# kvarq/kvarq

Measured on AMD Instinct MI355X. Metric: fastq_reads_per_sec_scanned, higher is better.
Workload: dtype u8

## Files before the change

include/kvarq_hip.h:

```cpp
#ifndef KVARQ_HIP_H
#define KVARQ_HIP_H

#include <stddef.h>
#include <stdint.h>

#ifdef __cplusplus
extern "C" {
#endif

#define KVQ_MAX_READLENGTH 1024
#define KVQ_SCANBUFSIZE    (1024*1024)
#define KVQ_MUT_CLASSES    6

enum {
    KVQ_OK          = 0,
    KVQ_ERR_FORMAT  = 1,
    KVQ_ERR_IO      = 2,
    KVQ_ERR_MEMORY  = 3,
    KVQ_ERR_RUNTIME = 4,
    KVQ_ERR_TYPE    = 5,
    KVQ_ERR_DEVICE  = 6,
    KVQ_ERR_RESCAN  = 7
};

typedef struct kvq_config {
    int32_t maxerrors;
    int32_t minoverlap;
    int32_t minreadlength;
    int32_t nthreads;
    int8_t  Amin;
    int8_t  Azero;
} kvq_config;

void kvq_config_set(const kvq_config *cfg);
void kvq_config_get(kvq_config *cfg);

int32_t kvq_last_error(char *msg, size_t cap);

typedef struct kvq_table kvq_table;

kvq_table *kvq_table_create(const uint8_t *const *seqs, const int32_t *seqlens, int32_t nseq,
                            const kvq_config *cfg);
void    kvq_table_destroy(kvq_table *t);
int32_t kvq_table_nseq(const kvq_table *t);
int64_t kvq_table_bases(const kvq_table *t);
int32_t kvq_table_seq_is_seeded(const kvq_table *t, int32_t s);
int32_t kvq_table_seed_k(const kvq_table *t);

enum { KVQ_CTR_RECORDS = 0, KVQ_CTR_LONGEST = 1, KVQ_CTR_HITS = 2, KVQ_CTR_READLENGTHS = 4 };
int64_t kvq_counters_len(const kvq_table *t);
int64_t kvq_counters_off_nseqhits(const kvq_table *t);
int64_t kvq_counters_off_nseqbasehits(const kvq_table *t);
int64_t kvq_counters_off_coverage(const kvq_table *t);
int64_t kvq_counters_off_mutations(const kvq_table *t);
int64_t kvq_table_seq_offset(const kvq_table *t, int32_t s);

typedef struct kvq_scan kvq_scan;

kvq_scan *kvq_scan_create(const kvq_table *t, void *d_counters);
void      kvq_scan_destroy(kvq_scan *s);

int64_t kvq_chunk_offsets(const uint8_t *data, int64_t nbytes, int64_t *offsets, int64_t cap);

int32_t kvq_scan_device(kvq_scan *s, const void *d_data, int64_t nbytes,
                        const int64_t *chunk_off, int64_t nchunks, int64_t fpos_base);

int32_t kvq_scan_host(kvq_scan *s, const void *h_data, int64_t nbytes,
                      const int64_t *chunk_off, int64_t nchunks, int64_t fpos_base);

int32_t kvq_scan_host_async(kvq_scan *s, const void *h_data, int64_t nbytes,
                            const int64_t *chunk_off, int64_t nchunks, int64_t fpos_base);
int32_t kvq_scan_host_copied(kvq_scan *s);
int32_t kvq_scan_host_drain(kvq_scan *s);

int32_t kvq_scan_finish(kvq_scan *s);
int32_t kvq_scan_finish_begin(kvq_scan *s);

int64_t        kvq_scan_n_hits(const kvq_scan *s);
const int32_t *kvq_scan_hit_seq_nr(const kvq_scan *s);
const int64_t *kvq_scan_hit_file_pos(const kvq_scan *s);
const int32_t *kvq_scan_hit_seq_pos(const kvq_scan *s);
const int32_t *kvq_scan_hit_length(const kvq_scan *s);
const int32_t *kvq_scan_hit_readlength(const kvq_scan *s);
const uint8_t *kvq_scan_hitseq_blob(const kvq_scan *s);
const int64_t *kvq_scan_hitseq_offsets(const kvq_scan *s);
const int64_t *kvq_scan_counters(const kvq_scan *s);
void          *kvq_scan_device_counters(const kvq_scan *s);
void          *kvq_scan_device_counters_own(const kvq_scan *s);
int64_t        kvq_scan_parsed(const kvq_scan *s);
int64_t        kvq_scan_total(const kvq_scan *s);

int32_t        kvq_scan_set_records(kvq_scan *s, int32_t on);
const uint8_t *kvq_scan_record_blob(const kvq_scan *s);
const int64_t *kvq_scan_hit_record_off(const kvq_scan *s);
const int32_t *kvq_scan_hit_record_len(const kvq_scan *s);
int64_t        kvq_scan_record_bytes(const kvq_scan *s);

double  kvq_scan_kernel_ms(const kvq_scan *s);
double  kvq_scan_main_kernel_ms(const kvq_scan *s);
double  kvq_scan_gap_ms(const kvq_scan *a, const kvq_scan *b);
int64_t kvq_scan_main_kernel_launches(const kvq_scan *s);
int32_t kvq_scan_reset(kvq_scan *s);
int32_t kvq_scan_path(const kvq_scan *s);
void    kvq_scan_force_exhaustive(kvq_scan *s, int32_t on);

#define KVQ_CELL_DENSE  0x1000
#define KVQ_CELL_DIAG   0x2000
#define KVQ_CELL_STAMPS 0x4000
int32_t kvq_scan_kernel_pick(int32_t k, int32_t stride, int32_t dense, uint32_t rec_bytes, uint32_t tile_bytes, uint32_t dbg);
int32_t kvq_scan_kernel(const kvq_scan *s);
uint32_t kvq_tile_for_text(const uint8_t *text, size_t n, uint32_t *rec_bytes_out);

typedef struct kvq_comm kvq_comm;
int32_t   kvq_comm_unique_id(void *id128);
kvq_comm *kvq_comm_create(int32_t nranks, int32_t rank, const void *id128);
void      kvq_comm_destroy(kvq_comm *c);
int32_t   kvq_comm_nranks(const kvq_comm *c);
int32_t   kvq_comm_rank(const kvq_comm *c);
int32_t   kvq_scan_set_comm(kvq_scan *s, kvq_comm *c);
int32_t   kvq_scan_gather_hits(kvq_scan *s, kvq_comm *c);
int32_t   kvq_comm_allreduce_counters(kvq_comm *c, void *d_counters, int64_t ctr_len, void *d_scratch16);
kvq_comm *kvq_comm_create_local(int32_t nranks, int32_t rank, uint64_t world_key);
int32_t   kvq_gather_plan(int32_t nranks, const uint64_t *counts, uint64_t *parts, uint64_t *blob_base, uint64_t *totals);
int32_t   kvq_gather_host(int32_t nranks, const uint64_t *counts, const uint8_t *const *rank_bufs, uint8_t *out);
void      kvq_result_layout_words(uint64_t n, uint64_t blob_bytes, uint64_t *out8);

kvq_scan *kvq_findseqs(const char *const *files, int32_t nfiles,
                       const uint8_t *const *seqs, const int32_t *seqlens, int32_t nseq);

#define KVQ_FIND_DEVICE_INFLATE 1u
#define KVQ_FIND_DEVICE_GZIP 2u
#define KVQ_FIND_RECORDS 4u
kvq_scan *kvq_findseqs_ex(const char *const *files, int32_t nfiles,
                          const uint8_t *const *seqs, const int32_t *seqlens, int32_t nseq, uint32_t flags);

void kvq_findseqs_free(kvq_scan *s);

int64_t kvq_host_chunk_plan(const char *const *files, int32_t nfiles, int64_t *chunk_fpos, int64_t *chunk_len,
                            int64_t cap, int64_t *parsed, int64_t *total, int64_t batch_bytes);

typedef struct kvq_live_stats {
    int64_t records_parsed;
    int64_t parsed;
    int64_t total;
    int64_t rls_longest;
    int32_t nseq;
    int32_t running;
    int32_t sigints;
    int32_t stop_requested;
} kvq_live_stats;

void kvq_poll_stats(kvq_live_stats *out, int64_t *readlengths ,
                    int64_t *nseqhits, int64_t *nseqbasehits, int32_t nseq_cap);
void kvq_request_stop(void);
void kvq_count_sigint(void);
int  kvq_sigint_counter_install(void);
void kvq_sigint_counter_remove(void);

int32_t kvq_device_count(void);
int32_t kvq_set_device(int32_t ordinal);
void   *kvq_device_alloc(int64_t nbytes);
void    kvq_device_free(void *p);
int32_t kvq_memcpy_h2d(void *d, const void *h, int64_t nbytes);
int32_t kvq_memcpy_d2h(void *h, const void *d, int64_t nbytes);
int32_t kvq_memset_d(void *d, int32_t value, int64_t nbytes);
int32_t kvq_device_synchronize(void);
void    kvq_release_cached(void);

int32_t kvq_synth_reads_device(void *d_out, int64_t first, int64_t n, int32_t L,
                               uint64_t seed, const void *d_genome, int64_t genome_size);
void    kvq_synth_reads_host(uint8_t *out, int64_t first, int64_t n, int32_t L,
                             uint64_t seed, const uint8_t *genome, int64_t genome_size);
void    kvq_synth_genome_host(uint8_t *out, int64_t size, uint64_t seed);

int32_t kvq_inflate_raw_host(const uint8_t *in, int64_t n, uint8_t *out, int64_t isize);

int64_t kvq_bgzf_index(const uint8_t *file_bytes, int64_t n, int64_t *block_off, uint32_t *csize, uint32_t *isize, int64_t cap);

typedef struct kvq_bgzf_block {
    int64_t  in_off;
    int64_t  out_off;
    uint32_t in_len;
    uint32_t isize;
} kvq_bgzf_block;

int32_t kvq_inflate_bgzf_device(const void *d_in, int64_t in_bytes, const kvq_bgzf_block *d_blocks, int64_t nblocks,
                                void *d_out, int64_t out_bytes, int32_t *d_status);

int64_t kvq_chunk_offsets_device(const void *d_data, int64_t nbytes, int64_t *offsets, int64_t cap);

typedef struct kvq_gzip_report {
    int64_t runs;
    int64_t chunks;
    int64_t candidates_tested;
    int64_t refuted;
    int64_t redecodes;
    int64_t slot_overflows;
    int64_t marker_symbols;
    int64_t input_retries;
    double  ms_find, ms_decode, ms_resolve, ms_replace;
} kvq_gzip_report;

int64_t kvq_inflate_gzip_host(const uint8_t *file, int64_t n, int64_t chunk_bytes, uint8_t *out, int64_t out_cap,
                              int32_t *status, int64_t *err_fpos, kvq_gzip_report *rep);
int64_t kvq_inflate_gzip_device(const void *d_file, int64_t n, int64_t chunk_bytes, void *d_out, int64_t out_cap,
                                int32_t *status, int64_t *err_fpos, kvq_gzip_report *rep);
void    kvq_gzip_last_report(kvq_gzip_report *rep);
int64_t kvq_gzip_slot_canaries(int32_t pad_symbols);
int64_t kvq_gzip_last_chunks(int64_t *cand, int64_t ncand_cap, int64_t *start_bit, int64_t *end_bit, int64_t *nsym, int64_t cap,
                             int64_t *ncand);

typedef struct kvq_bam_report {
    int64_t runs;
    int64_t segments;
    int64_t refuted;
    int64_t check_passes;
    int64_t records_seen;
    int64_t records_written;
    int64_t records_skipped;
    int64_t records_noqual;
    int64_t bam_bytes;
    int64_t text_bytes;
    double  ms_inflate, ms_find, ms_emit;
} kvq_bam_report;
void    kvq_bam_last_report(kvq_bam_report *rep);
int64_t kvq_bam_header_host(const uint8_t *inflated, int64_t n, int32_t *n_ref);
int64_t kvq_bam_to_fastq_host(const uint8_t *inflated, int64_t n, int32_t n_ref, int64_t first_record, uint8_t *out, int64_t cap,
                              int64_t *consumed);
int64_t kvq_bam_to_fastq_device(const void *d_in, int64_t n, int32_t n_ref, int64_t first_record, void *d_out, int64_t cap,
                                int64_t segment_bytes, kvq_bam_report *report);

const char *kvq_version(void);

#ifdef __cplusplus
}
#endif
#endif
```

kvarq_amd/_lib.py:

```python
import ctypes as C
import os

HERE = os.path.dirname(os.path.abspath(__file__))
PATH = os.path.join(HERE, 'libkvarq_hip.so')

MAX_READLENGTH = 1024
OK, ERR_FORMAT, ERR_IO, ERR_MEMORY, ERR_RUNTIME, ERR_TYPE, ERR_DEVICE, ERR_RESCAN = range(8)
CTR_RECORDS, CTR_LONGEST, CTR_HITS, CTR_READLENGTHS = 0, 1, 2, 4
CELL_DENSE, CELL_DIAG, CELL_STAMPS = 0x1000, 0x2000, 0x4000
FIND_RECORDS = 4


class Config(C.Structure):
    _fields_ = [('maxerrors', C.c_int32), ('minoverlap', C.c_int32), ('minreadlength', C.c_int32),
                ('nthreads', C.c_int32), ('Amin', C.c_int8), ('Azero', C.c_int8)]


class LiveStats(C.Structure):
    _fields_ = [('records_parsed', C.c_int64), ('parsed', C.c_int64), ('total', C.c_int64),
                ('rls_longest', C.c_int64), ('nseq', C.c_int32), ('running', C.c_int32),
                ('sigints', C.c_int32), ('stop_requested', C.c_int32)]


class GzipReport(C.Structure):
    _fields_ = [(n, C.c_int64) for n in ('runs', 'chunks', 'candidates_tested', 'refuted', 'redecodes',
                                         'slot_overflows', 'marker_symbols', 'input_retries')] + \
        [(n, C.c_double) for n in ('ms_find', 'ms_decode', 'ms_resolve', 'ms_replace')]

    def as_dict(self):
        return {n: getattr(self, n) for n, _ in self._fields_}


class BamReport(C.Structure):
    _fields_ = [(n, C.c_int64) for n in ('runs', 'segments', 'refuted', 'check_passes', 'records_seen', 'records_written',
                                         'records_skipped', 'records_noqual', 'bam_bytes', 'text_bytes')] + \
        [(n, C.c_double) for n in ('ms_inflate', 'ms_find', 'ms_emit')]

    def as_dict(self):
        return {n: getattr(self, n) for n, _ in self._fields_}


i32, i64, u64, vp, cp = C.c_int32, C.c_int64, C.c_uint64, C.c_void_p, C.c_char_p
P = C.POINTER

PROTOTYPES = {
    'kvq_config_set': (None, [P(Config)]),
    'kvq_config_get': (None, [P(Config)]),
    'kvq_last_error': (i32, [C.c_char_p, C.c_size_t]),
    'kvq_table_create': (vp, [P(cp), P(i32), i32, P(Config)]),
    'kvq_table_destroy': (None, [vp]),
    'kvq_table_nseq': (i32, [vp]),
    'kvq_table_bases': (i64, [vp]),
    'kvq_table_seq_is_seeded': (i32, [vp, i32]),
    'kvq_table_seed_k': (i32, [vp]),
    'kvq_counters_len': (i64, [vp]),
    'kvq_counters_off_nseqhits': (i64, [vp]),
    'kvq_counters_off_nseqbasehits': (i64, [vp]),
    'kvq_counters_off_coverage': (i64, [vp]),
    'kvq_counters_off_mutations': (i64, [vp]),
    'kvq_table_seq_offset': (i64, [vp, i32]),
    'kvq_scan_create': (vp, [vp, vp]),
    'kvq_scan_destroy': (None, [vp]),
    'kvq_chunk_offsets': (i64, [vp, i64, P(i64), i64]),
    'kvq_scan_device': (i32, [vp, vp, i64, P(i64), i64, i64]),
    'kvq_scan_host': (i32, [vp, vp, i64, P(i64), i64, i64]),
    'kvq_scan_host_async': (i32, [vp, vp, i64, P(i64), i64, i64]),
    'kvq_scan_host_copied': (i32, [vp]),
    'kvq_scan_host_drain': (i32, [vp]),
    'kvq_scan_finish': (i32, [vp]),
    'kvq_scan_finish_begin': (i32, [vp]),
    'kvq_scan_n_hits': (i64, [vp]),
    'kvq_scan_hit_seq_nr': (P(i32), [vp]),
    'kvq_scan_hit_file_pos': (P(i64), [vp]),
    'kvq_scan_hit_seq_pos': (P(i32), [vp]),
    'kvq_scan_hit_length': (P(i32), [vp]),
    'kvq_scan_hit_readlength': (P(i32), [vp]),
    'kvq_scan_hitseq_blob': (vp, [vp]),
    'kvq_scan_hitseq_offsets': (P(i64), [vp]),
    'kvq_scan_counters': (P(i64), [vp]),
    'kvq_scan_device_counters': (vp, [vp]),
    'kvq_scan_device_counters_own': (vp, [vp]),
    'kvq_scan_parsed': (i64, [vp]),
    'kvq_scan_total': (i64, [vp]),
    'kvq_scan_set_records': (i32, [vp, i32]),
    'kvq_scan_record_blob': (vp, [vp]),
    'kvq_scan_hit_record_off': (P(i64), [vp]),
    'kvq_scan_hit_record_len': (P(i32), [vp]),
    'kvq_scan_record_bytes': (i64, [vp]),
    'kvq_scan_kernel_ms': (C.c_double, [vp]),
    'kvq_scan_main_kernel_ms': (C.c_double, [vp]),
    'kvq_scan_gap_ms': (C.c_double, [vp, vp]),
    'kvq_scan_main_kernel_launches': (i64, [vp]),
    'kvq_scan_reset': (i32, [vp]),
    'kvq_scan_path': (i32, [vp]),
    'kvq_scan_force_exhaustive': (None, [vp, i32]),
    'kvq_scan_kernel_pick': (i32, [i32, i32, i32, C.c_uint32, C.c_uint32, C.c_uint32]),
    'kvq_scan_kernel': (i32, [vp]),
    'kvq_tile_for_text': (C.c_uint32, [vp, C.c_size_t, P(C.c_uint32)]),
    'kvq_comm_unique_id': (i32, [vp]),
    'kvq_comm_create': (vp, [i32, i32, vp]),
    'kvq_comm_destroy': (None, [vp]),
    'kvq_comm_nranks': (i32, [vp]),
    'kvq_comm_rank': (i32, [vp]),
    'kvq_scan_set_comm': (i32, [vp, vp]),
    'kvq_scan_gather_hits': (i32, [vp, vp]),
    'kvq_comm_allreduce_counters': (i32, [vp, vp, i64, vp]),
    'kvq_comm_create_local': (vp, [i32, i32, C.c_uint64]),
    'kvq_gather_plan': (i32, [i32, vp, vp, vp, vp]),
    'kvq_gather_host': (i32, [i32, vp, vp, vp]),
    'kvq_result_layout_words': (None, [C.c_uint64, C.c_uint64, vp]),
    'kvq_findseqs': (vp, [P(cp), i32, P(cp), P(i32), i32]),
    'kvq_findseqs_ex': (vp, [P(cp), i32, P(cp), P(i32), i32, C.c_uint32]),
    'kvq_findseqs_free': (None, [vp]),
    'kvq_host_chunk_plan': (i64, [P(cp), i32, P(i64), P(i64), i64, P(i64), P(i64), i64]),
    'kvq_poll_stats': (None, [P(LiveStats), P(i64), P(i64), P(i64), i32]),
    'kvq_request_stop': (None, []),
    'kvq_count_sigint': (None, []),
    'kvq_sigint_counter_install': (C.c_int, []),
    'kvq_sigint_counter_remove': (None, []),
    'kvq_device_count': (i32, []),
    'kvq_set_device': (i32, [i32]),
    'kvq_device_alloc': (vp, [i64]),
    'kvq_device_free': (None, [vp]),
    'kvq_memcpy_h2d': (i32, [vp, vp, i64]),
    'kvq_memcpy_d2h': (i32, [vp, vp, i64]),
    'kvq_memset_d': (i32, [vp, i32, i64]),
    'kvq_device_synchronize': (i32, []),
    'kvq_release_cached': (None, []),
    'kvq_synth_reads_device': (i32, [vp, i64, i64, i32, u64, vp, i64]),
    'kvq_synth_reads_host': (None, [vp, i64, i64, i32, u64, vp, i64]),
    'kvq_synth_genome_host': (None, [vp, i64, u64]),
    'kvq_inflate_raw_host': (i32, [vp, i64, vp, i64]),
    'kvq_bgzf_index': (i64, [vp, i64, P(i64), P(C.c_uint32), P(C.c_uint32), i64]),
    'kvq_chunk_offsets_device': (i64, [vp, i64, P(i64), i64]),
    'kvq_inflate_bgzf_device': (i32, [vp, i64, vp, i64, vp, i64, vp]),
    'kvq_inflate_gzip_host': (i64, [vp, i64, i64, vp, i64, P(i32), P(i64), P(GzipReport)]),
    'kvq_inflate_gzip_device': (i64, [vp, i64, i64, vp, i64, P(i32), P(i64), P(GzipReport)]),
    'kvq_gzip_last_report': (None, [P(GzipReport)]),
    'kvq_gzip_slot_canaries': (i64, [i32]),
    'kvq_gzip_last_chunks': (i64, [P(i64), i64, P(i64), P(i64), P(i64), i64, P(i64)]),
    'kvq_bam_last_report': (None, [P(BamReport)]),
    'kvq_bam_header_host': (i64, [vp, i64, P(i32)]),
    'kvq_bam_to_fastq_host': (i64, [vp, i64, i32, i64, vp, i64, P(i64)]),
    'kvq_bam_to_fastq_device': (i64, [vp, i64, i32, i64, vp, i64, i64, P(BamReport)]),
    'kvq_version': (cp, []),
}

_lib = None


def build():
    import subprocess
    subprocess.check_call(['make', '-s', '-C', os.path.join(HERE, 'csrc')])


def lib():
    global _lib
    if _lib is None:
        if not os.path.exists(PATH):
            raise ImportError('%s is missing: build it with `make -C kvarq_amd/csrc` '
                              '(there is no CPU fallback for the scan)' % PATH)
        L = C.CDLL(PATH)
        for name, (res, args) in PROTOTYPES.items():
            f = getattr(L, name)
            f.restype, f.argtypes = res, args
        _lib = L
    return _lib


def kernel_cell(cell):
    if cell <= 0:
        return None
    return {'k': cell & 15, 'stride': (cell >> 4) & 15, 'lg': ((cell >> 8) & 15) - 1, 'dense': bool(cell & CELL_DENSE)}


def last_error():
    buf = C.create_string_buffer(1024)
    code = lib().kvq_last_error(buf, 1024)
    return code, buf.value.decode('latin-1')
```

kvarq_amd/csrc/kernels_bp.hip:

```cpp
#include "kvq_host.h"

#ifndef KVQ_TEXT_AUX
#define KVQ_TEXT_AUX 0
#endif
#define KVQ_MARK(name) asm volatile("; KVQMARK " name)
#define BP_WIN (ST_BUF + ST_BLK)
#define BP_Q1_KIND 25
#define BP_QW 96
#define BP_Q2W 96
#define BP_NLCAP 1920
#define BP_P2_LATE 0xFFFEu
#define BP_HEAD 2048u
#define BP_QCAP (BP_QW * ST_WAVES)
#define BP_Q2CAP (BP_Q2W * ST_WAVES)

typedef unsigned int u32x4_t __attribute__((ext_vector_type(4)));

struct BpLds {
    uint32_t cdp[BP_WIN / 16 + 8];
    uint32_t gdp[BP_WIN / 32 + 8];
    uint16_t nl[BP_NLCAP];
    uint8_t  bmA[8192];
    uint32_t hist[KVQ_RL_BINS / 2];
    union {
        struct {
            uint32_t q1[BP_QCAP];
            uint32_t q2[BP_Q2CAP];
        };
        uint32_t nlp[BP_WIN / 32 + 8];
    };
    uint32_t rinfo[ST_RCAP];
    __attribute__((aligned(16))) uint8_t head[BP_HEAD];
    __attribute__((aligned(16))) uint32_t wtot[ST_WAVES];
    uint32_t longest_p1, records, fallback, n_owned, next_tile, first_tile, p2_jn;
    uint32_t sv_at[ST_WAVES], sv_end[ST_WAVES];
};
static_assert(sizeof(BpLds) <= 40 * 1024, "four workgroups per CU: at most 40 KB of LDS each");
static_assert(offsetof(BpLds, cdp) == 0, "cdp[] first");
#define BP_LDS_GDP ((uint32_t)offsetof(BpLds, gdp))
#define BP_LDS_BMA ((uint32_t)offsetof(BpLds, bmA))
#define BP_LDS_NLP ((uint32_t)offsetof(BpLds, nlp))
#define BP_LDS_HEAD ((uint32_t)offsetof(BpLds, head))
static_assert(sizeof(uint32_t) * (BP_QCAP + BP_Q2CAP) >= sizeof(uint32_t) * (BP_WIN / 32 + 8), "the newline plane fits the queues it shares LDS with");

__device__ __forceinline__ uint32_t lds_u32_at(uint32_t addr)
{
    return *reinterpret_cast<const __attribute__((address_space(3))) uint32_t *>((uintptr_t)addr);
}
__device__ __forceinline__ uint32_t cdp32(uint32_t pos)
{
    const uint32_t a = (pos >> 2) & ~3u, sh = (pos & 15u) * 2u;
    return __builtin_amdgcn_alignbit(lds_u32_at(a + 4u), lds_u32_at(a), sh);
}
template <int KK> __device__ __forceinline__ uint32_t cdp_code(uint32_t pos) { return cdp32(pos) & ((1u << (2 * KK)) - 1u); }

typedef const __attribute__((address_space(1))) uint32_t *GlbWords;
__device__ __forceinline__ uint32_t tab2_32(GlbWords tab2, uint32_t tpos)
{
    const uint32_t w = tpos >> 4, sh = (tpos & 15u) * 2u;
    return __builtin_amdgcn_alignbit(tab2[w + 1u], tab2[w], sh);
}

__device__ __forceinline__ int diff_codes(uint32_t x, uint32_t y)
{
    const uint32_t v = x ^ y;
    return __popc((v | (v >> 1)) & 0x55555555u);
}

template <int KK>
__device__ __forceinline__ bool seed_live_bp(GlbWords tab2, uint32_t roff, int rl, int rp, uint32_t toff, int seql, int sq)
{
    if (rp < 0 || rp + KK > rl || sq < 0 || sq + KK > seql) return false;
    return cdp_code<KK>(roff + (uint32_t)rp) == (tab2_32(tab2, toff + (uint32_t)sq) & ((1u << (2 * KK)) - 1u));
}

struct BpHot {
    const KvqParams *cold; GlbBytes tab; GlbWords tab2;
    int maxerrors, minoverlap, pitch;
};
template <int KK>
__device__ __forceinline__ void bp_verify_rest(const BpHot &P, GlbBytes text, bool alive, uint32_t roff, int rl, int p, uint32_t kind,
                                               uint32_t en_lo, uint32_t en_hi, int64_t tile_fpos, int stride)
{
    bool hitAB = false, hitC = false;
    int s = 0, lenAB = 0, lenC = 0, sposAB = 0, sposC = 0; uint32_t keyAB = 0, keyC = 0;
    const int64_t fpos = tile_fpos + (int64_t)roff - (int64_t)ST_PRE;
    if (alive) {
        const int q = (int)(en_lo & 4095u);
        s = (int)(en_lo >> 12);
        const uint32_t toff = en_hi & 0xFFFFFu;
        const int seql = (int)(en_hi >> 20);
        const int mo = P.minoverlap, me = P.maxerrors;
        const int d = q - p;
        const int a = d < 0 ? -d : 0;
        const int L = (rl < seql - d ? rl : seql - d) - a;
        bool canAB = false, canC = false;
        const bool guard = rl > mo && seql > mo;
        if (d < 0) {
            const int i = -d;
            if (i <= rl - seql) { canC = true; lenC = seql; sposC = -i; keyC = (2u << 30) | (uint32_t)i; }
            else if (guard && i <= rl - mo) { canAB = true; lenAB = rl - i; sposAB = -i; keyAB = (0u << 30) | (uint32_t)(rl - mo - i); }
        } else if (d == 0) {
            canC = true; lenC = rl > seql ? seql : rl; sposC = 0; keyC = 2u << 30;
        } else {
            const int i = d;
            if (guard && i <= seql - mo && i >= seql - rl) { canAB = true; lenAB = seql - i; sposAB = i; keyAB = (1u << 30) | (uint32_t)(seql - mo - i); }
            if (rl <= seql && i <= seql - rl) { canC = true; lenC = rl; sposC = i; keyC = (2u << 30) | (uint32_t)i; }
        }
        if (canAB || canC) {
            int mism = 0, j = 0;
            const GlbBytes x = text + roff + (uint32_t)a, y = P.tab + toff + (uint32_t)(a + d);
            for (; j + 8 <= L && mism <= me; j += 8) {
                typedef unsigned int u32x2_t __attribute__((ext_vector_type(2)));
                typedef u32x2_t __attribute__((aligned(1))) u32x2_any;
                const u32x2_t xv = *reinterpret_cast<const __attribute__((address_space(1))) u32x2_any *>(x + j);
                const u32x2_t yv = *reinterpret_cast<const __attribute__((address_space(1))) u32x2_any *>(y + j);
                mism += diff_bytes(xv.x, yv.x) + diff_bytes(xv.y, yv.y);
            }
            for (; j + 4 <= L && mism <= me; j += 4) mism += diff_bytes(glb_u32(x + j), glb_u32(y + j));
            for (; j < L && mism <= me; j++) mism += (x[j] != y[j]);
            if (mism <= me) {
                bool earlier = false;
                for (int jj = 0; jj <= me && !earlier; jj++) {
                    const int ph = jj * KK, pt = rl - (jj + 1) * KK;
                    if (ph + KK <= rl && (kind == 0u || ph < p)) earlier = seed_live_bp<KK>(P.tab2, roff, rl, ph, toff, seql, ph + d);
                    if (!earlier && pt >= 0 && (kind == 0u || pt < p)) earlier = seed_live_bp<KK>(P.tab2, roff, rl, pt, toff, seql, pt + d);
                }
                if (kind == 0u) {
                    for (int jj = 0; jj <= me && !earlier; jj++)
                        for (int sft = 0; sft < stride && !earlier; sft++) {
                            const int o = jj * P.pitch + sft;
                            if (o < q && ((o - d) & (stride - 1)) == 0) earlier = seed_live_bp<KK>(P.tab2, roff, rl, o - d, toff, seql, o);
                        }
                }
                if (!earlier) { hitAB = canAB; hitC = canC; }
            }
        }
    }
    emit_cold(P.cold, hitAB, fpos, s, sposAB, lenAB, rl, keyAB);
    emit_cold(P.cold, hitC, fpos, s, sposC, lenC, rl, keyC);
}

__device__ __forceinline__ void bp_vector(const uint4 v, uint32_t addk, uint32_t &nl16, uint32_t &g16, uint32_t &c32)
{
    const uint32_t x[4] = { v.x, v.y, v.z, v.w };
    uint32_t nf[4], gf[4], cc[4];
#pragma unroll
    for (int d = 0; d < 4; d++) {
        nf[d] = kvq_nl_flags(x[d]);
        gf[d] = good_flags(x[d], addk);
        cc[d] = __builtin_amdgcn_udot4(x[d] & 0x06060606u, 0x40100401u, 0u, false);
    }
#ifdef KVQ_ABL_JUNK
    {
        uint32_t junk = x[0];
#pragma unroll
        for (int i = 0; i < KVQ_ABL_JUNK; i++) {
#if KVQ_ABL_SLOW == 2
            { uint32_t sj = 0; asm volatile("s_add_u32 %0, %0, 1" : "+s"(sj)); asm volatile("" :: "s"(sj)); }
#elif KVQ_ABL_SLOW == 3
            { uint32_t lj; asm volatile("ds_read_b32 %0, %1" : "=v"(lj) : "v"(junk & 0x3FCu)); asm volatile("s_waitcnt lgkmcnt(0)" ::: "memory"); asm volatile("" :: "v"(lj)); }
#elif KVQ_ABL_SLOW
            asm volatile("v_lshl_or_b32 %0, %0, 1, %1" : "+v"(junk) : "v"(x[1]));
#else
            asm volatile("v_add_u32 %0, %0, %1" : "+v"(junk) : "v"(x[1]));
#endif
        }
        asm volatile("" :: "v"(junk));
    }
#endif
    nl16 = kvq_flags16(nf[0], nf[1], nf[2], nf[3]);
    g16 = kvq_flags16(gf[0], gf[1], gf[2], gf[3]);
    c32 = ((cc[0] | (cc[1] << 8)) >> 1) | ((cc[2] | (cc[3] << 8)) << 15);
}

struct BpArgs {
    KvqParams P;
    SeedTables X;
    const uint8_t *data; int64_t fpos_base;
    const uint4 *tiles; uint32_t *tile_report; unsigned int *tile_ctr;
    void *redo;
    unsigned int *fail;
    void *surv;
    uint32_t ntiles, tile_bytes, dbg, pad_, redo_cap;
    uint32_t surv_cap;
};
#define BP_SHARDS 64u
#define BP_SHARD_STRIDE 32u
__host__ __device__ static inline uint32_t bp_shard_begin(uint32_t sh, uint32_t ntiles) { return (uint32_t)(((uint64_t)sh * ntiles) / BP_SHARDS); }
__device__ __forceinline__ uint32_t bp_draw(unsigned int *ctr, uint32_t ntiles, uint32_t &sh, uint32_t &left)
{
    while (left) {
        const uint32_t t = atomicAdd(&ctr[sh * BP_SHARD_STRIDE], 1u);
        if (t < bp_shard_begin(sh + 1u, ntiles)) return t;
        sh = sh + 1u == BP_SHARDS ? 0u : sh + 1u; left--;
    }
    return ntiles;
}
static_assert(BP_SHARDS == 64u, "one counter per lane of the drawing wave");
__device__ __forceinline__ uint32_t bp_draw_wave(unsigned int *ctr, uint32_t ntiles, uint32_t &sh, uint32_t lane)
{
    const uint32_t m = (((uint32_t)blockIdx.x >> 6) * 2u + 37u) | 1u;
    for (;;) {
        const uint32_t mine = (sh + m * lane) & (BP_SHARDS - 1u);
        const uint32_t seen = __hip_atomic_load(&ctr[mine * BP_SHARD_STRIDE], __ATOMIC_RELAXED, __HIP_MEMORY_SCOPE_AGENT);
        const uint64_t open = __ballot(seen < bp_shard_begin(mine + 1u, ntiles));
        if (open == 0) return ntiles;
        const uint32_t pick = (sh + m * (uint32_t)(__ffsll((long long)open) - 1)) & (BP_SHARDS - 1u);
        uint32_t t = 0;
        if (lane == 0) t = atomicAdd(&ctr[pick * BP_SHARD_STRIDE], 1u);
        t = (uint32_t)__builtin_amdgcn_readfirstlane((int)t);
        sh = pick;
        if (t < bp_shard_begin(pick + 1u, ntiles)) return t;
    }
}
typedef const __attribute__((address_space(4))) BpArgs *BpArgsPtr;
__device__ __forceinline__ BpArgsPtr bp_args(const BpArgs *A)
{
    BpArgsPtr p = (BpArgsPtr)A;
    asm volatile("" : "+s"(p));
    return p;
}

#ifndef BP_OCC
#define BP_OCC 8
#endif

__device__ __forceinline__ void bp_runs64(uint64_t m, int n, uint32_t dbg, int &pre, int &suf, int &best, int &bstart)
{
    const uint64_t nmask = n < 64 ? (1ull << n) - 1ull : ~0ull;
    uint64_t zz = ~m & nmask;
    const int c = __popc((uint32_t)zz) + __popc((uint32_t)(zz >> 32));
    if (!__any(c > 3) && !(dbg & 4u)) {
        const uint32_t lo = (uint32_t)zz, hi = (uint32_t)(zz >> 32);
        auto ffbl = [](uint32_t x) -> uint32_t { uint32_t r; asm("v_ffbl_b32 %0, %1" : "=v"(r) : "v"(x)); return r; };
        auto ffbh = [](uint32_t x) -> uint32_t { uint32_t r; asm("v_ffbh_u32 %0, %1" : "=v"(r) : "v"(x)); return r; };
        auto ctz64 = [&](uint32_t l, uint32_t h) -> uint32_t {
            const uint32_t pl = ffbl(l), ph = ffbl(h) | 32u;
            const uint32_t r = pl < ph ? pl : ph; return r < (uint32_t)n ? r : (uint32_t)n;
        };
        const uint32_t p1 = ctz64(lo, hi);
        const uint64_t z2 = zz & (zz - 1ull);
        const uint32_t p2 = ctz64((uint32_t)z2, (uint32_t)(z2 >> 32));
        const uint32_t ch = ffbh(hi), cl = ffbh(lo) | 32u;
        uint32_t lz = ch < cl ? ch : cl; lz = lz < 64u ? lz : 64u;
        const uint32_t e = 64u - lz;
        const int g0 = (int)p1, g1 = (int)p2 - (int)p1 - 1, g2 = (int)e - (int)p2 - 2, g3 = n - (int)e;
        int bl = g0, bs = 0;
        if (g1 > bl) { bl = g1; bs = (int)p1 + 1; }
        if (g2 > bl) { bl = g2; bs = (int)p2 + 1; }
        if (g3 > bl) { bl = g3; bs = (int)e; }
        pre = g0; suf = g3; best = bl; bstart = bs;
    } else if (!__any(c > 8) && !(dbg & 4u)) {
        int prev = 0, first = n, p, bl = 0, bs = 0;
        do {
            const uint32_t plo = (uint32_t)(__ffs((int)(uint32_t)zz) - 1), ph = (uint32_t)(__ffs((int)(uint32_t)(zz >> 32)) - 1);
            const uint32_t phi = ph > 0xFFFFFFDFu ? 0xFFFFFFFFu : ph + 32u;
            uint32_t pm = plo < phi ? plo : phi; if (pm > (uint32_t)n) pm = (uint32_t)n;
            p = (int)pm;
            zz &= zz - 1ull;
            first = first < p ? first : p;
            const int gap = p - prev;
            if (gap > bl) { bl = gap; bs = prev; }
            prev = p < n ? p + 1 : prev;
        } while (__any(p < n));
        pre = first; suf = n - prev; best = bl; bstart = bs;
    } else {
        const uint64_t inv = ~m;
        pre = inv ? __ffsll((long long)inv) - 1 : 64; if (pre > n) pre = n;
        const uint64_t top = ~(m << (64 - n));
        suf = top ? __clzll((long long)top) : 64; if (suf > n) suf = n;
        longest_run64(m, n, best, bstart);
    }
}

template <int SS, int LG, bool STAMPS, bool DIAG = STAMPS, int KK = 8, bool DENSE = (KK < 8)>
__global__ void __launch_bounds__(ST_THREADS, DENSE ? 8 : BP_OCC)
kvq_scan_bp(const BpArgs *__restrict__ A_)
{
    __shared__ __align__(16) BpLds S;
    uint8_t *const lds_raw = reinterpret_cast<uint8_t *>(&S);
    int tid = threadIdx.x, lane = tid & 63;
    const uint32_t wave = rfl((uint32_t)tid >> 6);
    if ((uint32_t)(uintptr_t)((__attribute__((address_space(3))) uint8_t *)lds_raw) != 0u) __builtin_trap();
    unsigned long long stamp_acc[8] = { 0, 0, 0, 0, 0, 0, 0, 0 }, stamp_t = 0, wave_p34 = 0;
    unsigned long long rt_in = 0, rt_pro = 0, rt_first = 0;
    uint32_t tally[8] = { 0, 0, 0, 0, 0, 0, 0, 0 };
#ifdef KVQ_TALLY
#define BTALLY(i, cond) do { if constexpr (STAMPS) { if (cond) tally[i]++; } } while (0)
#else
#define BTALLY(i, cond) ((void)0)
#endif
    if constexpr (STAMPS) rt_in = __builtin_amdgcn_s_memrealtime();
#define BSTAMP(i) do { if constexpr (STAMPS) { const unsigned long long now_ = __builtin_amdgcn_s_memtime(); stamp_acc[i] += now_ - stamp_t; stamp_t = now_; } } while (0)

    uint32_t ntiles, tile_bytes, dbg, amin;
    {
        const BpArgsPtr A = bp_args(A_);
        ntiles = A->ntiles; tile_bytes = A->tile_bytes; dbg = DIAG ? A->dbg : 0u; amin = (uint32_t)A->P.amin;
        const GlbWords bm1 = (GlbWords)A->X.bm1;
        for (int i = tid; i < (1 << (2 * KK)) / 32; i += ST_THREADS) reinterpret_cast<uint32_t *>(S.bmA)[i] = bm1[i];
    }
    uint32_t my_shard = blockIdx.x % BP_SHARDS; bool no_more = false;
    if (wave == ST_WAVES - 1u) {
        unsigned int *const ctr = bp_args(A_)->tile_ctr;
        const uint32_t t0 = bp_draw_wave(ctr, ntiles, my_shard, (uint32_t)lane);
        const uint32_t t1 = t0 < ntiles ? bp_draw_wave(ctr, ntiles, my_shard, (uint32_t)lane) : ntiles;
        no_more = t1 >= ntiles;
        if (lane == 0) { S.first_tile = t0; S.next_tile = t1; }
    }
    for (int i = tid; i < KVQ_RL_BINS / 2; i += ST_THREADS) S.hist[i] = 0;
    if (tid == 0) { S.longest_p1 = 0; S.records = 0; S.fallback = 0; }
    if (tid < (int)ST_WAVES) { S.sv_at[tid] = 0; S.sv_end[tid] = 0; }
    if (tid < 8) { S.cdp[BP_WIN / 16 + tid] = 0; S.gdp[BP_WIN / 32 + tid] = 0; }

    static_assert(ST_ROUNDS * 16u == ST_BLK, "one scan block per thread");
    static_assert(ST_WAVES == 8, "eight wave totals");
    __syncthreads();

    if (const uint32_t stg = bp_args(A_)->pad_) { for (uint32_t i = 0; i < (blockIdx.x >> 8) * stg; i++) __builtin_amdgcn_s_sleep(127); }
    if constexpr (STAMPS) rt_pro = __builtin_amdgcn_s_memrealtime();
    unsigned long long *const ctr_stamps = bp_args(A_)->P.ctr + KVQ_CTR_RL_ + 924;
    const uint32_t addk = (0x80u - amin) * 0x01010101u;
    uint32_t tiles_done = 0;
    uint32_t g_done = 0xFFFFFFFFu;
    uint32_t my_longest = 0;
    for (uint32_t g = rfl(S.first_tile); ; ) {
        asm volatile("" : "+v"(tid));
        lane = tid & 63;
        const uint32_t blk = (uint32_t)tid * ST_BLK;
        const uint32_t wv = wave * (ST_BLK * 64u / 16u) + (uint32_t)lane;
        if constexpr (STAMPS) stamp_t = __builtin_amdgcn_s_memtime();
        uint32_t Ja = 0, Jb = 0, Jt = 0, g0 = 0; GlbBytes text = nullptr;
        uint4 pre[ST_ROUNDS];
#pragma unroll
        for (int r = 0; r < (int)ST_ROUNDS; r++) pre[r] = make_uint4(0, 0, 0, 0);
        if (g < ntiles) {
            const BpArgsPtr A = bp_args(A_);
            const u32x4_t q = ((const __attribute__((address_space(4))) u32x4_t *)A->tiles)[(dbg & 64u) ? (g & 63u) : g];
            Ja = q.x; Jb = q.y; Jt = q.z;
            g0 = (Ja & ~15u) + Jt * tile_bytes;
            const uint8_t *const data = A->data;
            text = (GlbBytes)data + g0 - ST_PRE;
            const uint32_t load_hi = g0 + ST_TILE + ST_OV < Jb ? g0 + ST_TILE + ST_OV : Jb;
            const uint32_t vo = 16u * wv - ST_PRE, vo0 = wv >= ST_PRE / 16u ? vo : ST_NO_BLOCK;
            const __amdgpu_buffer_rsrc_t rs = __builtin_amdgcn_make_buffer_rsrc((void *)(data + g0), 0, (int)(((load_hi + 15u) & ~15u) - g0), 0x00020000);
#pragma unroll
            for (int r = 0; r < (int)ST_ROUNDS; r++) {
                const u32x4_t v = __builtin_amdgcn_raw_buffer_load_b128(rs, (int)(r ? vo + 1024u * r : vo0), 0, KVQ_TEXT_AUX);
                pre[r] = make_uint4(v.x, v.y, v.z, v.w);
            }
        }
        __syncthreads();
        unsigned long long sub_t0 = 0, sub_t1 = 0;
        if constexpr (STAMPS) sub_t0 = __builtin_amdgcn_s_memtime();
        if (g_done != 0xFFFFFFFFu) {
            if (tid == 0 && S.fallback) { atomicOr(&bp_args(A_)->tile_report[g_done], TR_FLAG_FALLBACK); S.fallback = 0; }
        }
        if (g >= ntiles) break;
        const uint32_t gn = rfl(S.next_tile);
        const uint32_t own_end = g0 + tile_bytes < Jb ? g0 + tile_bytes : Jb;
        const uint32_t load_hi = g0 + ST_TILE + ST_OV < Jb ? g0 + ST_TILE + ST_OV : Jb;
        const uint32_t own_begin_l = (Jt == 0 ? Ja : g0) - g0 + ST_PRE;
        const uint32_t own_end_l = own_end - g0 + ST_PRE;
        const uint32_t end_l = load_hi - g0 + ST_PRE;

        {
            const uint32_t w_lo = wave * (ST_BLK * 64u), w_hi = w_lo + ST_BLK * 64u;
            const bool cut = ((own_begin_l & 15u) && own_begin_l > w_lo && own_begin_l < w_hi) || ((end_l & 15u) && end_l > w_lo && end_l < w_hi);
            if (cut) {
                uint32_t wv_ = wv;
                asm volatile("" : "+v"(wv_));
#pragma unroll
                for (int r = 0; r < (int)ST_ROUNDS; r++) {
                    const uint32_t o = 16u * (wv_ + 64u * r);
                    uint32_t x[4] = { pre[r].x, pre[r].y, pre[r].z, pre[r].w };
#pragma unroll
                    for (int d = 0; d < 4; d++) x[d] &= (kvq_range_flags(o + 4u * d, own_begin_l, end_l) >> 7) * 0xFFu;
                    pre[r] = make_uint4(x[0], x[1], x[2], x[3]);
                }
            }
        }
        if constexpr (STAMPS) { asm volatile("s_waitcnt vmcnt(0)" ::: "memory"); sub_t1 = __builtin_amdgcn_s_memtime(); }
        KVQ_MARK("P0 vectors");
        {
            const uint32_t pa = 2u * wv, ca = 4u * wv;
#pragma unroll
            for (int r = 0; r < (int)ST_ROUNDS; r++) {
                uint32_t n16, g16, c32;
                bp_vector(pre[r], addk, n16, g16, c32);
                *reinterpret_cast<__attribute__((address_space(3))) uint16_t *>((uintptr_t)(BP_LDS_NLP + pa + 128u * r)) = (uint16_t)n16;
                *reinterpret_cast<__attribute__((address_space(3))) uint16_t *>((uintptr_t)(BP_LDS_GDP + pa + 128u * r)) = (uint16_t)g16;
                *reinterpret_cast<__attribute__((address_space(3))) uint32_t *>((uintptr_t)(ca + 256u * r)) = c32;
            }
            if (wave == 0u) {
#pragma unroll
                for (int r = 0; r < (int)(BP_HEAD / 1024u); r++)
                    *reinterpret_cast<__attribute__((address_space(3))) u32x4_t *>((uintptr_t)(BP_LDS_HEAD + 16u * (uint32_t)lane + 1024u * r)) = u32x4_t{ pre[r].x, pre[r].y, pre[r].z, pre[r].w };
            }
        }
        KVQ_MARK("P0 vectors end");
        uint32_t m0, m1, m2;
        {
            const uint32_t a = BP_LDS_NLP + ((10u * (uint32_t)tid) & ~3u), sh = ((uint32_t)tid & 1u) * 16u;
            const uint32_t d0 = lds_u32_at(a), d1 = lds_u32_at(a + 4u), d2 = lds_u32_at(a + 8u);
            m0 = __builtin_amdgcn_alignbit(d1, d0, sh); m1 = __builtin_amdgcn_alignbit(d2, d1, sh); m2 = (d2 >> sh) & 0xFFFFu;
        }
        static_assert(ST_BLK == 80u, "five vectors per block");
        const uint32_t cnt = (uint32_t)(__popc(m0) + __popc(m1) + __popc(m2));
        const uint32_t incl = kvq_wave_incl_scan(cnt);
        if (lane == 63) S.wtot[wave] = incl;
        KVQ_MARK("P0 scan end");
        if constexpr (STAMPS) { if (tid == 0) { atomicAdd(&ctr_stamps[0], sub_t0 - stamp_t); atomicAdd(&ctr_stamps[1], sub_t1 - sub_t0); } }
        BSTAMP(0);
        __syncthreads();
        KVQ_MARK("P1b");
        BSTAMP(1);
        uint32_t n_all = 0;
        {
            uint32_t run = S.wtot[lane & 7];
            run += (uint32_t)__builtin_amdgcn_update_dpp(0, (int)run, 0x111, 0xf, 0xf, false);
            run += (uint32_t)__builtin_amdgcn_update_dpp(0, (int)run, 0x112, 0xf, 0xf, false);
            run += (uint32_t)__builtin_amdgcn_update_dpp(0, (int)run, 0x114, 0xf, 0xf, false);
            n_all = (uint32_t)__builtin_amdgcn_readlane((int)run, 7);
            const uint32_t upto = (uint32_t)__builtin_amdgcn_readlane((int)run, (int)wave);
            uint32_t n = upto - (uint32_t)__builtin_amdgcn_readlane((int)incl, 63) + incl - cnt;
            if (blk < own_end_l && blk + ST_BLK >= own_end_l) S.n_owned = n + cnt;
            if (__any(cnt != 0u)) {
                if (n_all <= BP_NLCAP && !__any(cnt > 2u)) {
                    auto low80 = [](uint32_t w0, uint32_t w1, uint32_t w2) -> uint32_t {
                        auto ffbl = [](uint32_t x) -> uint32_t { uint32_t r; asm("v_ffbl_b32 %0, %1" : "=v"(r) : "v"(x)); return r; };
                        const uint32_t f0 = ffbl(w0), f1 = ffbl(w1) | 32u, f2 = ffbl(w2) | 64u;
                        const uint32_t f01 = f0 < f1 ? f0 : f1;
                        return f01 < f2 ? f01 : f2;
                    };
                    const uint32_t p1 = low80(m0, m1, m2);
                    const uint32_t k0 = m0 & (m0 - 1u), k1 = m0 ? m1 : m1 & (m1 - 1u), k2 = (m0 | m1) ? m2 : m2 & (m2 - 1u);
                    const uint32_t p2 = low80(k0, k1, k2);
                    if (cnt) {
                        S.nl[n] = (uint16_t)(blk + p1);
                        if (cnt > 1u) S.nl[n + 1u] = (uint16_t)(blk + p2);
                    }
                    m0 = m1 = m2 = 0u;
                }
                while (__any((m0 | m1 | m2) != 0u)) {
                    const bool in0 = m0 != 0u, in1 = m1 != 0u;
                    const uint32_t w = in0 ? m0 : in1 ? m1 : m2;
                    if (w) {
                        const uint32_t pos = blk + (in0 ? 0u : in1 ? 32u : 64u) + (uint32_t)(__ffs((int)w) - 1);
                        if (n < BP_NLCAP) S.nl[n] = (uint16_t)pos;
                        n++;
                        const uint32_t w1 = w & (w - 1u);
                        if (in0) m0 = w1; else if (in1) m1 = w1; else m2 = w1;
                    }
                }
            }
        }
        if (wave == 0u) {
            const uint32_t cnt0 = (uint32_t)__builtin_amdgcn_readlane((int)incl, 63);
            uint32_t early = BP_P2_LATE;
            if (Jt != 0 && cnt0 >= 10u) {
                const uint32_t m = (uint32_t)lane;
                bool ok = false;
                if (m >= 1 && m <= 8) {
                    const uint32_t e0 = S.nl[m - 1], e2 = S.nl[m + 1];
                    const uint32_t ls0 = e0 + 1u, ls2 = e2 + 1u;
                    if (e0 < own_end_l && ls0 < end_l && ls2 < end_l) {
                        const uint32_t c0 = ls0 < BP_HEAD ? lds_byte_at(BP_LDS_HEAD + ls0) : (uint32_t)text[ls0];
                        const uint32_t c2 = ls2 < BP_HEAD ? lds_byte_at(BP_LDS_HEAD + ls2) : (uint32_t)text[ls2];
                        ok = c0 == '@' && c2 == '+';
                    }
                }
                const uint64_t mk = __ballot(ok);
                early = mk ? (uint32_t)(__ffsll((long long)mk) - 1) : TR_NONE;
            }
            if (lane == 0) S.p2_jn = early;
        }
        __syncthreads();
        KVQ_MARK("P1b end / P2");
        BSTAMP(2);

        uint32_t nrec = 0, jn = TR_NONE, drawn;
        {
            const uint32_t n_nl = n_all < BP_NLCAP ? n_all : BP_NLCAP;
            const uint32_t n_owned = rfl(S.n_owned);
            uint32_t fallback = n_all > BP_NLCAP ? 1u : 0u;
            if (Jt == 0) jn = 0;
            else if (const uint32_t early = rfl(S.p2_jn); early != BP_P2_LATE) jn = early;
            else {
                const uint32_t m = (uint32_t)lane;
                bool ok = false;
                if (m >= 1 && m <= 8 && m <= n_owned && m + 2 <= n_nl) {
                    const uint32_t ls0 = (uint32_t)S.nl[m - 1] + 1u;
                    const uint32_t ls2 = (uint32_t)S.nl[m + 1] + 1u;
                    if (ls0 < end_l && ls2 < end_l) {
                        const uint32_t c0 = ls0 < BP_HEAD ? lds_byte_at(BP_LDS_HEAD + ls0) : (uint32_t)text[ls0];
                        const uint32_t c2 = ls2 < BP_HEAD ? lds_byte_at(BP_LDS_HEAD + ls2) : (uint32_t)text[ls2];
                        ok = c0 == '@' && c2 == '+';
                    }
                }
                const uint64_t mk = __ballot(ok);
                if (mk) jn = (uint32_t)(__ffsll((long long)mk) - 1);
            }
            uint32_t left = 0u;
            if (jn != TR_NONE) {
                if (jn <= n_owned) nrec = (n_owned - jn) / 4u + 1u;
                if (nrec > 0 && jn + 4u * nrec > n_nl) {
                    const uint32_t fit = n_nl >= jn ? (n_nl - jn) / 4u : 0u;
                    if (load_hi < Jb) left = 1u;
                    if (n_all > BP_NLCAP) fallback = 1u;
                    nrec = fit;
                }
                if (nrec > ST_RCAP) { nrec = ST_RCAP; fallback = 1u; }
            }
            if (fallback) { nrec = 0; left = 1u; }
            if (tid == 0 || tid == ST_THREADS - 64) {
                const BpArgsPtr A = bp_args(A_);
                if (tid == 0) {
                    A->tile_report[g] = (n_owned & 0xFFFFu) | ((jn & 0xFFu) << 16) | (left ? TR_FLAG_SKIPPED : 0u) | (left && nrec ? TR_FLAG_PARTIAL : 0u);
                    if (left) A->tile_report[ntiles + g] = nrec ? g0 - ST_PRE + (uint32_t)S.nl[jn + 4u * nrec - 1u] + 2u : 0u;
                    S.records += nrec;
                } else if (!no_more) drawn = atomicAdd(&A->tile_ctr[my_shard * BP_SHARD_STRIDE], 1u);
            }
        }

        if (++tiles_done == ST_HIST_TILES) {
            unsigned long long *const ctr = (bp_args(A_)->P.ctr + (size_t)(blockIdx.x % KVQ_STAGE_COPIES) * KVQ_STAGE_SLOTS);
            for (int i = tid; i < KVQ_RL_BINS / 2; i += ST_THREADS) {
                const uint32_t w = atomicExch(&S.hist[i], 0u);
                if (w & 0xFFFFu) atomicAdd(&ctr[KVQ_CTR_RL_ + 2 * i], (unsigned long long)(w & 0xFFFFu));
                if (w >> 16) atomicAdd(&ctr[KVQ_CTR_RL_ + 2 * i + 1], (unsigned long long)(w >> 16));
            }
            tiles_done = 0;
        }
        if (dbg & 32u) nrec = 0;
        KVQ_MARK("P2 end / P3 setup");
        BSTAMP(3);
        if (wave >= 4u) KVQ_SETPRIO(2); else KVQ_SETPRIO(1);
        unsigned long long wave_t3 = 0;
        if constexpr (STAMPS) wave_t3 = __builtin_amdgcn_s_memtime();
        static_assert(ST_THREADS == 512, "lg = 9 - ceil(log2(nrec))");
        uint32_t lg;
        if constexpr (LG >= 0) lg = (uint32_t)LG;
        else {
            const int lg_ = 9 - (nrec > 1u ? 32 - __builtin_clz(nrec - 1u) : 0);
            lg = lg_ < 0 ? 0u : lg_ > 6 ? 6u : (uint32_t)lg_;
        }
        const uint32_t G = 1u << lg, RP = ST_THREADS >> lg;
        const uint32_t gl = (uint32_t)tid & (G - 1u), gr = (uint32_t)tid >> lg;
        for (uint32_t pass0 = 0; pass0 < nrec; pass0 += RP) {
            const uint32_t k = pass0 + gr;
            const bool have = k < nrec;
            uint32_t roff = 0; int rl = 0;
            uint32_t c0, cp;
            if (have) {
                const uint32_t m = jn + 4u * k;
                const uint32_t rstart = m == 0 ? ST_PRE + (Ja & 15u) : (uint32_t)S.nl[m - 1] + 1u;
                const uint32_t n0 = S.nl[m], n1 = S.nl[m + 1], n2 = S.nl[m + 2], n3 = S.nl[m + 3];
                const uint32_t sread = n0 + 1u, plus = n1 + 1u, sscore = n2 + 1u;
        KVQ_MARK("trim");
                if (gl == 0) { if (dbg & 8u) { c0 = '@'; cp = '+'; } else { c0 = text[rstart]; cp = text[plus]; } }
                const int Q = (int)(n3 - sscore);
                const int per = (Q + (int)G - 1) >> lg;
                Seg sg; sg.beg = (int)mul_u24(gl, (uint32_t)per); if (sg.beg > Q) sg.beg = Q;
                int s1 = sg.beg + per; if (s1 > Q) s1 = Q;
                sg.len = 0; sg.pre = 0; sg.suf = 0; sg.best = 0; sg.bstart = sg.beg;
                {
                    auto round = [&](int c0_) -> Seg {
                        const int n = s1 - c0_ < 64 ? s1 - c0_ : 64;
                        const uint32_t bit = sscore + (uint32_t)c0_;
                        const uint32_t a = BP_LDS_GDP + ((bit >> 5) << 2), sh = bit & 31u;
                        const uint32_t d0 = lds_u32_at(a), d1 = lds_u32_at(a + 4u), d2 = lds_u32_at(a + 8u);
                        const uint64_t nmask = n < 64 ? (1ull << n) - 1ull : ~0ull;
                        const uint64_t mm = (((uint64_t)__builtin_amdgcn_alignbit(d2, d1, sh) << 32) | (uint64_t)__builtin_amdgcn_alignbit(d1, d0, sh)) & nmask;
                        Seg sub; sub.beg = c0_; sub.len = n;
                        int bs;
                        bp_runs64(mm, n, dbg, sub.pre, sub.suf, sub.best, bs);
                        sub.bstart = c0_ + bs;
                        return sub;
                    };
                    if (!__any(per > 64)) sg = round(sg.beg);
                    else {
                        for (int cc = sg.beg; cc < s1; cc += 64) {
                            const Seg sub = round(cc);
                            sg = (cc == sg.beg) ? sub : seg_merge(sg, sub);
                        }
                    }
                }
                if (G == 4u) {
#define KVQ_QUAD(v, ctl) __builtin_amdgcn_update_dpp(0, (v), (ctl), 0xf, 0xf, true)
                    {
                        Seg B;
                        B.len = KVQ_QUAD(sg.len, 0xB1); B.pre = KVQ_QUAD(sg.pre, 0xB1); B.suf = KVQ_QUAD(sg.suf, 0xB1);
                        B.best = KVQ_QUAD(sg.best, 0xB1); B.bstart = KVQ_QUAD(sg.bstart, 0xB1); B.beg = 0;
                        sg = seg_merge(sg, B);
                    }
                    {
                        Seg B;
                        B.len = KVQ_QUAD(sg.len, 0x4E); B.pre = KVQ_QUAD(sg.pre, 0x4E); B.suf = KVQ_QUAD(sg.suf, 0x4E);
                        B.best = KVQ_QUAD(sg.best, 0x4E); B.bstart = KVQ_QUAD(sg.bstart, 0x4E); B.beg = 0;
                        sg = seg_merge(sg, B);
                    }
                    rl = KVQ_QUAD(sg.best, 0x00);
                    roff = sread + (uint32_t)KVQ_QUAD(sg.bstart, 0x00);
#undef KVQ_QUAD
                } else {
                    for (uint32_t d = 1; d < G; d <<= 1) {
                        Seg B;
                        B.len = __shfl_xor(sg.len, (int)d, 64); B.pre = __shfl_xor(sg.pre, (int)d, 64); B.suf = __shfl_xor(sg.suf, (int)d, 64);
                        B.best = __shfl_xor(sg.best, (int)d, 64); B.bstart = __shfl_xor(sg.bstart, (int)d, 64); B.beg = 0;
                        if ((gl & d) == 0) sg = seg_merge(sg, B);
                    }
                    rl = __shfl(sg.best, lane & ~(int)(G - 1u), 64);
                    roff = sread + (uint32_t)__shfl(sg.bstart, lane & ~(int)(G - 1u), 64);
                }
                my_longest = my_longest > (uint32_t)(rl + 1) ? my_longest : (uint32_t)(rl + 1);
                if (gl == 0) {
                    if (rl < KVQ_RL_BINS) atomicAdd(&S.hist[rl >> 1], 1u << (16 * (rl & 1)));
                    S.rinfo[k] = roff | ((uint32_t)rl << 16);
                }
            }
        KVQ_MARK("trim end / filter");
            BSTAMP(4);
            KVQ_SETPRIO(2);
            const uint32_t rpw = 64u >> lg, grw = (uint32_t)lane >> lg;
            const uint32_t wfirst = pass0 + wave * rpw;
            const uint32_t npass = wfirst < nrec ? (nrec - wfirst < rpw ? nrec - wfirst : rpw) : 0u;
            uint32_t *const q1 = S.q1 + wave * BP_QW; uint32_t *const q2 = S.q2 + wave * BP_Q2W;
            uint32_t sub = (dbg & 128u) ? npass : 0u, step = rpw;
            while (sub < npass) {
                BTALLY(6, lane == 0);
                asm volatile("" : "+v"(rl), "+v"(roff));
                int minrl, me_; const __attribute__((address_space(1))) uint8_t *bmL;
                {
                    const BpArgsPtr A = bp_args(A_);
                    minrl = A->P.minreadlength; me_ = A->P.maxerrors;
                    bmL = (const __attribute__((address_space(1))) uint8_t *)A->X.bm1 + (1 << (2 * KK)) / 8;
                }
                const bool mine = have && rl >= minrl && !(dbg & 2u) && grw >= sub && grw - sub < step;
                uint32_t qn = 0;
                int e0 = 0, e1 = 0;
                if (mine) {
                    const int NPe = (rl - KK) / SS + 1;
                    const int per = (NPe + (int)G - 1) >> lg;
                    e0 = (int)mul_u24(gl, (uint32_t)per); if (e0 > NPe) e0 = NPe;
                    e1 = e0 + per; if (e1 > NPe) e1 = NPe;
                }
                auto fixed_block = [&](int pp, bool ok) -> bool {
                    const uint32_t code = cdp_code<KK>(roff + (uint32_t)(ok ? pp : 0));
                    const uint32_t bits = bmL[code >> 3];
                    return ok & (bool)((bits >> (code & 7u)) & 1u);
                };
                auto head_ok = [&](int jj) { return mine && jj <= me_ && (jj + 1) * KK <= rl; };
                auto tail_ok = [&](int jj) { const int pp = rl - (jj + 1) * KK; return mine && jj <= me_ && pp >= 0 && !((pp % KK) == 0 && pp <= me_ * KK); };
                const bool hhit = fixed_block((int)gl * KK, head_ok((int)gl));
                const bool thit = fixed_block(rl - ((int)gl + 1) * KK, tail_ok((int)gl));
                constexpr int NR = SS == 8 ? 6 : SS == 4 ? 12 : (LG == 3 || LG == 1) ? 24 : 18;
                bool first = true;
                if constexpr (!DENSE) {
                for (int ee = e0; __any(ee < e1); ee += NR, first = false) {
                    const bool act = ee < e1;
#include "kernels_bp_lookup.inc"
                    const int nv = act ? (e1 - ee < NR ? e1 - ee : NR) : 0;
                    hA &= (1u << nv) - 1u;
                    const bool hh = first && hhit, th = first && thit;
                    const uint32_t c = (uint32_t)__popc(hA) + (hh ? 1u : 0u) + (th ? 1u : 0u);
                    const uint32_t inc = kvq_wave_incl_scan(c);
                    const uint32_t tot = (uint32_t)__builtin_amdgcn_readlane((int)inc, 63);
                    if (tot) {
                        uint32_t idx = qn + inc - c;
                        while (hA) {
                            const int j = __ffs((int)hA) - 1; hA &= hA - 1u;
                            if (idx < BP_QW) q1[idx] = k | ((uint32_t)(SS * (ee + j)) << 9);
                            idx++;
                        }
                        if (hh) { if (idx < BP_QW) q1[idx] = k | ((gl * KK) << 9) | (1u << BP_Q1_KIND); idx++; }
                        if (th && idx < BP_QW) { const uint32_t pt = (uint32_t)(rl - ((int)gl + 1) * KK); q1[idx] = k | (pt << 9) | (1u << BP_Q1_KIND); }
                        qn += tot;
                    }
                }
                for (int t = (int)G; t <= me_; t += (int)G) {
                    const int jj = t + (int)gl;
#pragma unroll
                    for (int side = 0; side < 2; side++) {
                        const int pp = side ? rl - (jj + 1) * KK : jj * KK;
                        const bool hit = fixed_block(pp, side ? tail_ok(jj) : head_ok(jj));
                        const uint64_t mm = __ballot(hit);
                        if (mm) {
                            const uint32_t idx = qn + (uint32_t)__popcll(mm & kvq_lanemask_lt());
                            if (hit && idx < BP_QW) q1[idx] = k | ((uint32_t)pp << 9) | (1u << BP_Q1_KIND);
                            qn += (uint32_t)__popcll(mm);
                        }
                    }
                }
                }
        KVQ_MARK("filter end / P4a");
                BSTAMP(5);
                KVQ_SETPRIO(3);

                if constexpr (!DENSE) {
                const bool over = qn > BP_QW;
                const uint32_t qn_ok = (over || (dbg & 1u)) ? 0u : qn;
                if (over && step > 1u) { step >>= 1; continue; }
                if (over) {
                    if (mine && gl == 0) {
                        const BpArgsPtr A = bp_args(A_);
                        const KvqRedo Rd(A->redo);
                        const uint32_t boff = g0 - ST_PRE + roff;
                        bool put = false;
                        if (A->redo) {
                            if (rl >= KVQ_LONG_READ) {
                                const unsigned int i = atomicAdd(Rd.count + 1, 1u);
                                if (i < KVQ_LONG_CAP) { Rd.read_off[KVQ_REDO_CAP - 1u - i] = boff; Rd.read_len[KVQ_REDO_CAP - 1u - i] = rl; put = true; }
                            }
                            if (!put) {
                                const unsigned int i = atomicAdd(Rd.count, 1u);
                                if (i < A->redo_cap) { Rd.rec_start[i] = KVQ_REDO_TRIMMED; Rd.read_off[i] = boff; Rd.read_len[i] = rl; }
                                put = true;
                            }
                        }
                        if (!put) S.fallback = 1u;
                        else atomicOr(A->fail, 2u);
                    }
                }
#include "kernels_bp_p4.inc"
                } else {
                    uint32_t hA = 0, hpos = 0, tpos = 0; bool hh = false, th = false;
                    int ee = e0, xt = (int)G;
                    int ee_of_hA = e0;
                    bool done = false;
                    while (!done) {
                        bool full = false;
                        while (!full) {
                            if (!__any(hA != 0u || hh || th)) {
                                ee_of_hA = ee;
                                if (__any(ee < e1)) {
                                    const bool act = ee < e1;
                                    uint32_t hA_;
                                    {
#include "kernels_bp_lookup.inc"
                                        hA_ = hA;
                                    }
                                    const int nv = act ? (e1 - ee < NR ? e1 - ee : NR) : 0;
                                    hA = hA_ & ((1u << nv) - 1u);
                                    if (first) { hh = hhit; th = thit; hpos = gl * KK; tpos = (uint32_t)(rl - ((int)gl + 1) * KK); first = false; }
                                    ee += NR;
                                } else if (xt <= me_) {
                                    const int jj = xt + (int)gl;
                                    hpos = (uint32_t)(jj * KK); tpos = (uint32_t)(rl - (jj + 1) * KK);
                                    hh = fixed_block((int)hpos, head_ok(jj)); th = fixed_block((int)tpos, tail_ok(jj));
                                    xt += (int)G;
                                } else { done = true; break; }
                                continue;
                            }
                            const uint32_t c = (uint32_t)__popc(hA) + (hh ? 1u : 0u) + (th ? 1u : 0u);
                            const uint32_t inc = kvq_wave_incl_scan(c);
                            const uint32_t tot = (uint32_t)__builtin_amdgcn_readlane((int)inc, 63);
                            uint32_t idx = qn + inc - c;
                            while (hA && idx < BP_QW) {
                                const int j = __ffs((int)hA) - 1; hA &= hA - 1u;
                                q1[idx++] = k | ((uint32_t)(SS * (ee_of_hA + j)) << 9);
                            }
                            if (hh && idx < BP_QW) { q1[idx++] = k | (hpos << 9) | (1u << BP_Q1_KIND); hh = false; }
                            if (th && idx < BP_QW) { q1[idx++] = k | (tpos << 9) | (1u << BP_Q1_KIND); th = false; }
                            full = qn + tot >= BP_QW;
                            qn = qn + tot < BP_QW ? qn + tot : BP_QW;
                        }
                        {
                            const uint32_t qn_ok = (dbg & 1u) ? 0u : qn;
#include "kernels_bp_p4.inc"
                        }
                        qn = 0;
                    }
                }
                KVQ_SETPRIO(2);
                sub += step;
            }
            KVQ_SETPRIO(0);
            if (have && gl == 0 && (c0 != '@' || cp != '+')) {
                const BpArgsPtr A = bp_args(A_);
                const uint32_t m = jn + 4u * k;
                const uint32_t rstart = m == 0 ? ST_PRE + (Ja & 15u) : (uint32_t)S.nl[m - 1] + 1u, plus = (uint32_t)S.nl[m + 1] + 1u;
                const int64_t tf = A->fpos_base + (int64_t)g0;
                if (c0 != '@') atomicMin(A->P.err, ((unsigned long long)(tf + rstart - ST_PRE) << 16) | (0ull << 8) | c0);
                else atomicMin(A->P.err, ((unsigned long long)(tf + plus - ST_PRE) << 16) | (1ull << 8) | cp);
            }
        KVQ_MARK("P4 end");
            BSTAMP(6);
        }
        if constexpr (STAMPS) wave_p34 += __builtin_amdgcn_s_memtime() - wave_t3;
        if (wave == ST_WAVES - 1u) {
            uint32_t d = no_more ? ntiles : rfl(drawn);
            if (!no_more && d >= bp_shard_begin(my_shard + 1u, ntiles)) {
                d = bp_draw_wave(bp_args(A_)->tile_ctr, ntiles, my_shard, (uint32_t)tid & 63u);
                no_more = d >= ntiles;
            }
            if ((tid & 63) == 0) S.next_tile = d;
        }
        KVQ_MARK("tile end");
        BSTAMP(7);
        if constexpr (STAMPS) { if (rt_first == 0) rt_first = __builtin_amdgcn_s_memrealtime(); }
        g_done = g; g = gn;
    }

    unsigned long long rt_loop = 0;
    if constexpr (STAMPS) rt_loop = __builtin_amdgcn_s_memrealtime();
    {
        const uint32_t at = S.sv_at[wave], end = S.sv_end[wave];
        if (at + (uint32_t)lane < end) KvqSurvivors(bp_args(A_)->surv).item[at + (uint32_t)lane].rl = 0;
    }
    atomicMax(&S.longest_p1, my_longest);
    __syncthreads();
    unsigned long long *const ctr = (bp_args(A_)->P.ctr + (size_t)(blockIdx.x % KVQ_STAGE_COPIES) * KVQ_STAGE_SLOTS);
    if constexpr (STAMPS) {
        if (tid == 0) for (int i = 0; i < 8; i++) atomicAdd(&ctr[KVQ_CTR_RL_ + 900 + i], stamp_acc[i]);
        for (int i = 0; i < 8; i++) if (tally[i]) atomicAdd(&ctr[KVQ_CTR_RL_ + 930 + i], (unsigned long long)tally[i]);
        if (lane == 0) atomicAdd(&ctr[KVQ_CTR_RL_ + 908 + wave], wave_p34);
        if (tid == 0) {
            const unsigned long long rt_out = __builtin_amdgcn_s_memrealtime();
            atomicAdd(&ctr[KVQ_CTR_RL_ + 916], rt_pro - rt_in); atomicAdd(&ctr[KVQ_CTR_RL_ + 917], rt_first ? rt_first - rt_pro : 0ull);
            atomicAdd(&ctr[KVQ_CTR_RL_ + 918], rt_loop - rt_in); atomicAdd(&ctr[KVQ_CTR_RL_ + 919], 1ull);
            atomicMax(&ctr[KVQ_CTR_RL_ + 920], rt_out); atomicMax(&ctr[KVQ_CTR_RL_ + 921], rt_in);
            atomicMax(&ctr[KVQ_CTR_RL_ + 922], ~rt_in);
            atomicAdd(&ctr[KVQ_CTR_RL_ + 923], rt_out - rt_loop);
        }
    }
    for (int i = tid; i < KVQ_RL_BINS / 2; i += ST_THREADS) {
        const uint32_t w = S.hist[i];
        if (w & 0xFFFFu) atomicAdd(&ctr[KVQ_CTR_RL_ + 2 * i], (unsigned long long)(w & 0xFFFFu));
        if (w >> 16) atomicAdd(&ctr[KVQ_CTR_RL_ + 2 * i + 1], (unsigned long long)(w >> 16));
    }
    if (tid == 0) {
        if (S.longest_p1) atomicMax(&ctr[KVQ_CTR_LONGEST_], (unsigned long long)S.longest_p1);
        if (S.records) atomicAdd(&ctr[KVQ_CTR_RECORDS_], (unsigned long long)S.records);
    }
}

__device__ __forceinline__ bool seed_same_text(GlbBytes x, GlbBytes y, int K)
{
    const uint32_t x0 = glb_u32(x), y0 = glb_u32(y), x1 = glb_u32(x + 4), y1 = glb_u32(y + 4);
    const uint32_t m0 = K >= 4 ? 0x06060606u : (0x06060606u & ((1u << (8 * K)) - 1u));
    const uint32_t m1 = K >= 8 ? 0x06060606u : K > 4 ? (0x06060606u & ((1u << (8 * (K - 4))) - 1u)) : 0u;
    return (((x0 ^ y0) & m0) | ((x1 ^ y1) & m1)) == 0u;
}
extern "C" __global__ void __launch_bounds__(1024)
kvq_verify_survivors(KvqParams P, const uint8_t *__restrict__ data, int64_t fpos_base, const void *surv_, const unsigned int *__restrict__ fail,
                     int K, int stride, int pitch)
{
    const KvqSurvivors Sv(const_cast<void *>(surv_));
    if (fail && (*fail & 1u)) return;
    const uint32_t n = Sv.count[0] < Sv.count[1] ? Sv.count[0] : Sv.count[1];
    const int me = P.maxerrors, mo = P.minoverlap;
    const uint32_t step = gridDim.x * blockDim.x;
    __shared__ uint32_t n_round, arena_at;
    const uint32_t lane = threadIdx.x & 63u;
    for (uint32_t base = blockIdx.x * blockDim.x; base < n; base += step) {
        if (threadIdx.x == 0) n_round = 0;
        __syncthreads();
        const uint32_t i = base + threadIdx.x;
        bool hitAB = false, hitC = false;
        int s = 0, rl = 0, lenAB = 0, lenC = 0, sposAB = 0, sposC = 0; uint32_t keyAB = 0, keyC = 0; int64_t fpos = 0;
        if (i < n) {
            const KvqSurvivor v = Sv.item[i];
            rl = (int)v.rl; const int p = (int)v.p; const uint32_t kind = v.kind;
            fpos = fpos_base + (int64_t)v.boff;
            const int q = (int)(v.en & 4095u);
            s = (int)((v.en >> 12) & 0xFFFFFu);
            const uint32_t toff = (uint32_t)((v.en >> 32) & 0xFFFFFu);
            const int seql = (int)(v.en >> 52);
            const GlbBytes read = (GlbBytes)data + v.boff, seq = (GlbBytes)P.tab + toff;
            const int d = q - p;
            const int a = d < 0 ? -d : 0;
            const int L = (rl < seql - d ? rl : seql - d) - a;
            bool canAB = false, canC = false;
            const bool guard = rl > mo && seql > mo;
            if (d < 0) {
                const int ii = -d;
                if (ii <= rl - seql) { canC = true; lenC = seql; sposC = -ii; keyC = (2u << 30) | (uint32_t)ii; }
                else if (guard && ii <= rl - mo) { canAB = true; lenAB = rl - ii; sposAB = -ii; keyAB = (0u << 30) | (uint32_t)(rl - mo - ii); }
            } else if (d == 0) {
                canC = true; lenC = rl > seql ? seql : rl; sposC = 0; keyC = 2u << 30;
            } else {
                const int ii = d;
                if (guard && ii <= seql - mo && ii >= seql - rl) { canAB = true; lenAB = seql - ii; sposAB = ii; keyAB = (1u << 30) | (uint32_t)(seql - mo - ii); }
                if (rl <= seql && ii <= seql - rl) { canC = true; lenC = rl; sposC = ii; keyC = (2u << 30) | (uint32_t)ii; }
            }
            if ((canAB || canC) && L > 0 && rl > 0) {
                bool earlier = false;
                auto live = [&](bool want, int rp, int sq) -> bool {
                    const bool ok = want && rp >= 0 && rp + K <= rl && sq >= 0 && sq + K <= seql;
                    return seed_same_text(read + (ok ? rp : 0), seq + (ok ? sq : 0), K) && ok;
                };
                const int sft = d & (stride - 1);
                constexpr int JJ = 4;
#pragma unroll
                for (int jj = 0; jj < JJ; jj++) {
                    const int ph = jj * K, pt = rl - (jj + 1) * K, o = jj * pitch + sft;
                    const bool in = jj <= me;
                    const bool e0 = live(in && (kind == 0u || ph < p), ph, ph + d);
                    const bool e1 = live(in && (kind == 0u || pt < p), pt, pt + d);
                    const bool e2 = live(in && kind == 0u && o < q, o - d, o);
                    earlier = earlier || e0 || e1 || e2;
                }
                for (int jj = JJ; jj <= me && !earlier; jj++) {
                    const int ph = jj * K, pt = rl - (jj + 1) * K, o = jj * pitch + sft;
                    earlier = live(kind == 0u || ph < p, ph, ph + d) || live(kind == 0u || pt < p, pt, pt + d) || live(kind == 0u && o < q, o - d, o);
                }
                if (!earlier) {
                    int mism = 0, j = 0;
                    const GlbBytes x = read + a, y = seq + (a + d);
                    typedef u32x4_t __attribute__((aligned(1))) u32x4_any;
                    typedef const __attribute__((address_space(1))) u32x4_any *GlbVec;
                    auto diff16 = [](const u32x4_t xv, const u32x4_t yv) { return diff_bytes(xv.x, yv.x) + diff_bytes(xv.y, yv.y) + diff_bytes(xv.z, yv.z) + diff_bytes(xv.w, yv.w); };
                    for (; j + 128 <= L && mism <= me; j += 128) {
                        u32x4_t xv[8], yv[8];
#pragma unroll
                        for (int t = 0; t < 8; t++) { xv[t] = *(GlbVec)(x + j + 16 * t); yv[t] = *(GlbVec)(y + j + 16 * t); }
#pragma unroll
                        for (int t = 0; t < 8; t++) mism += diff16(xv[t], yv[t]);
                    }
                    if (j + 64 <= L && mism <= me) {
                        u32x4_t xv[4], yv[4];
#pragma unroll
                        for (int t = 0; t < 4; t++) { xv[t] = *(GlbVec)(x + j + 16 * t); yv[t] = *(GlbVec)(y + j + 16 * t); }
#pragma unroll
                        for (int t = 0; t < 4; t++) mism += diff16(xv[t], yv[t]);
                        j += 64;
                    }
                    for (; j + 16 <= L && mism <= me; j += 16) mism += diff16(*(GlbVec)(x + j), *(GlbVec)(y + j));
                    if (j < L && mism <= me) {
                        if (L >= 16) {
                            const u32x4_t xv = *(GlbVec)(x + L - 16), yv = *(GlbVec)(y + L - 16);
                            const int keep = L - j;
                            uint32_t dx[4] = { xv.x ^ yv.x, xv.y ^ yv.y, xv.z ^ yv.z, xv.w ^ yv.w };
#pragma unroll
                            for (int t = 0; t < 4; t++) {
                                const int first_new = 16 - keep - 4 * t;
                                const uint32_t m = first_new <= 0 ? 0xFFFFFFFFu : first_new >= 4 ? 0u : 0xFFFFFFFFu << (8 * first_new);
                                mism += diff_bytes(dx[t] & m, 0u);
                            }
                        } else {
                            for (; j + 4 <= L && mism <= me; j += 4) mism += diff_bytes(glb_u32(x + j), glb_u32(y + j));
                            for (; j < L && mism <= me; j++) mism += (x[j] != y[j]);
                        }
                    }
                    if (mism <= me) { hitAB = canAB; hitC = canC; }
                }
            }
        }
        const uint64_t mAB = __ballot(hitAB), mC = __ballot(hitC);
        const uint32_t nAB = (uint32_t)__popcll(mAB), nC = (uint32_t)__popcll(mC);
        uint32_t at = 0;
        if (nAB + nC) {
            if (lane == 0u) at = atomicAdd(&n_round, nAB + nC);
            at = (uint32_t)__builtin_amdgcn_readfirstlane((int)at);
        }
        __syncthreads();
        const uint32_t total = n_round;
        if (total) {
            if (threadIdx.x == 0) arena_at = atomicAdd(P.arena_n, total);
            __syncthreads();
            const uint32_t o = arena_at + at;
            KvqHit h;
            h.fpos = fpos; h.seq_nr = s; h.readlength = rl; h.blob_off = 0;
            if (hitAB) {
                const uint32_t idx = o + (uint32_t)__popcll(mAB & kvq_lanemask_lt());
                h.seq_pos = sposAB; h.length = lenAB; h.key = keyAB;
                if (idx < P.arena_cap) P.arena[idx] = h;
            }
            if (hitC) {
                const uint32_t idx = o + nAB + (uint32_t)__popcll(mC & kvq_lanemask_lt());
                h.seq_pos = sposC; h.length = lenC; h.key = keyC;
                if (idx < P.arena_cap) P.arena[idx] = h;
            }
        }
    }
}

__device__ void kvq_long_line_run(const uint8_t *line, uint32_t Q, int amin, int lane, int &best, uint32_t &best_start)
{
    Seg all; all.beg = 0; all.len = 0; all.pre = 0; all.suf = 0; all.best = 0; all.bstart = 0;
    for (uint32_t r0 = 0; r0 < Q; r0 += 4096u) {
        uint32_t w[4][4];
#pragma unroll
        for (int r = 0; r < 4; r++) {
            const uint32_t o = r0 + 1024u * (uint32_t)r + 16u * (uint32_t)lane;
            const uint32_t oo = o + 16u <= Q + 1u ? o : (Q + 1u >= 16u ? Q + 1u - 16u : 0u);
#pragma unroll
            for (int d = 0; d < 4; d++) __builtin_memcpy(&w[r][d], line + oo + 4u * d, 4);
        }
#pragma unroll
        for (int r = 0; r < 4; r++) {
            const uint32_t row = r0 + 1024u * (uint32_t)r;
            if (row >= Q) break;
            const uint32_t o = row + 16u * (uint32_t)lane;
            const uint32_t oo = o + 16u <= Q + 1u ? o : (Q + 1u >= 16u ? Q + 1u - 16u : 0u);
            const int n = o < Q ? (Q - o < 16u ? (int)(Q - o) : 16) : 0;
            uint32_t m = 0;
#pragma unroll
            for (int d = 0; d < 4; d++)
#pragma unroll
                for (int b = 0; b < 4; b++) m |= (uint32_t)((int)(int8_t)(w[r][d] >> (8 * b)) >= amin) << (4 * d + b);
            const uint32_t shift = o - oo;
            m = shift < 16u ? m >> shift : 0u;
            m &= n > 0 ? (1u << n) - 1u : 0u;
            Seg sg; sg.beg = (int)o; sg.len = n;
            int bs;
            bp_runs64((uint64_t)m, n, 0u, sg.pre, sg.suf, sg.best, bs);
            sg.bstart = (int)o + bs;
            for (uint32_t d = 1; d < 64u; d <<= 1) {
                Seg B;
                B.len = __shfl_xor(sg.len, (int)d, 64); B.pre = __shfl_xor(sg.pre, (int)d, 64); B.suf = __shfl_xor(sg.suf, (int)d, 64);
                B.best = __shfl_xor(sg.best, (int)d, 64); B.bstart = __shfl_xor(sg.bstart, (int)d, 64); B.beg = 0;
                if (((uint32_t)lane & d) == 0) sg = seg_merge(sg, B);
            }
            Seg R;
            R.beg = (int)row; R.len = __shfl(sg.len, 0, 64); R.pre = __shfl(sg.pre, 0, 64); R.suf = __shfl(sg.suf, 0, 64);
            R.best = __shfl(sg.best, 0, 64); R.bstart = __shfl(sg.bstart, 0, 64);
            all = (row == 0u) ? R : seg_merge(all, R);
        }
    }
    best = all.best; best_start = (uint32_t)all.bstart;
}
```

kvarq_amd/csrc/kernels_bp_p4.inc:

```
                if (qn_ok) {
                    typedef const __attribute__((address_space(1))) u32x4_t *GlbEntries;
                    typedef unsigned int u32x2_t __attribute__((ext_vector_type(2)));
                    typedef const __attribute__((address_space(1))) u32x2_t __attribute__((aligned(4))) *GlbPairs;
                    GlbWords start; GlbEntries ent; int need;
                    {
                        const BpArgsPtr A = bp_args(A_);
                        start = (GlbWords)A->X.start; ent = (GlbEntries)A->X.ent;
                        need = (me_ + 1) * KK;
                    }
                    BTALLY(5, lane == 0);
                    for (uint32_t w0 = 0; ; w0 += BP_Q2W) {
                        uint32_t run = 0;
                        for (uint32_t q0 = 0; q0 < qn_ok; q0 += 64u) {
                            const uint32_t qi = q0 + lane;
                            uint32_t en0 = 0, ne = 0;
                            if (qi < qn_ok) {
                                const uint32_t cd = q1[qi];
                                BTALLY(0, w0 == 0u && (cd >> BP_Q1_KIND) == 0u); BTALLY(1, w0 == 0u && (cd >> BP_Q1_KIND) != 0u);
                                const uint32_t code = cdp_code<KK>((S.rinfo[cd & 511u] & 0xFFFFu) + ((cd >> 9) & 0xFFFFu));
                                const u32x2_t st = *(GlbPairs)(start + (code | ((cd >> BP_Q1_KIND) << (2 * KK))));
                                en0 = st.x; ne = st.y - st.x;
                            }
                            const uint32_t inc = kvq_wave_incl_scan(ne);
                            const uint32_t base = run + inc - ne - w0;
                            for (uint32_t j = 0; j < ne; j++)
                                if (base + j < BP_Q2W) q2[base + j] = (qi << 22) | (en0 + j);
                            run += (uint32_t)__builtin_amdgcn_readlane((int)inc, 63);
                        }
        KVQ_MARK("P4b");
                        const uint32_t n_items = run - w0 < BP_Q2W ? run - w0 : BP_Q2W;
                        for (uint32_t i0 = 0; i0 < n_items; i0 += 64u) {
                            BTALLY(4, lane == 0);
                            const uint32_t ii = i0 + lane;
                            bool alive = false;
                            uint32_t kind = 0, croff = 0, en_lo = 0, en_hi = 0; int p = 0, crl = 0;
                            BTALLY(2, ii < n_items);
                            if (ii < n_items) {
                                const uint32_t it = q2[ii];
                                const u32x4_t E = ent[it & 0x3FFFFFu];
                                const uint32_t cd = q1[it >> 22];
                                p = (int)((cd >> 9) & 0xFFFFu); kind = cd >> BP_Q1_KIND;
                                const uint32_t ri = S.rinfo[cd & 511u];
                                croff = ri & 0xFFFFu; crl = (int)(ri >> 16);
                                en_lo = E.x; en_hi = E.y;
                                const int q = (int)(E.x & 4095u), seql = (int)(E.y >> 20);
                                const int d = q - p;
                                const int a = d < 0 ? -d : 0;
                                const int L = (crl < seql - d ? crl : seql - d) - a;
                                if (L >= need) {
                                    const int wn = L < 16 ? L : 16;
                                    const int w = p < a + L - wn ? p : a + L - wn;
                                    const uint32_t sh = 2u * (uint32_t)(w - p + 16);
                                    const uint32_t seqw = (uint32_t)((((uint64_t)E.w << 32) | E.z) >> sh);
                                    const uint32_t v = cdp32(croff + (uint32_t)w) ^ seqw;
                                    uint32_t dm = (v | (v >> 1)) & 0x55555555u;
                                    if (wn < 16) dm &= (1u << (2 * wn)) - 1u;
                                    alive = __popc(dm) <= me_;
                                }
                            }
                            const bool any_alive = __any(alive);
                            BTALLY(3, alive); BTALLY(7, lane == 0 && any_alive);
                            if (any_alive) {
                                const KvqSurvivors Sv(bp_args(A_)->surv);
                                if (Sv.count) {
                                    const uint64_t am = __ballot(alive);
                                    const uint32_t na = (uint32_t)__popcll(am);
                                    uint32_t at = rfl(S.sv_at[wave]), end = rfl(S.sv_end[wave]);
                                    if (at + na > end) {
                                        if (at + lane < end) Sv.item[at + lane].rl = 0;
                                        const uint32_t want = na > KVQ_SURV_CHUNK ? na : KVQ_SURV_CHUNK;
                                        uint32_t base = 0;
                                        if (lane == 0) base = atomicAdd(Sv.count, want);
                                        base = rfl(base);
                                        const uint32_t cap = bp_args(A_)->surv_cap;
                                        if (base + want <= cap) { at = base; end = base + want; }
                                        else {
                                            if (lane < want && base + lane < cap) Sv.item[base + lane].rl = 0;
                                            at = end = 0;
                                        }
                                    }
                                    if (at + na <= end && end != 0u) {
                                        if (alive) {
                                            KvqSurvivor v;
                                            v.boff = g0 - ST_PRE + croff; v.rl = (uint16_t)crl; v.p = (uint16_t)p; v.en = ((uint64_t)en_hi << 32) | en_lo; v.kind = kind; v.pad = 0;
                                            Sv.item[at + (uint32_t)__popcll(am & kvq_lanemask_lt())] = v;
                                            alive = false;
                                        }
                                        at += na;
                                    }
                                    if (lane == 0) { S.sv_at[wave] = at; S.sv_end[wave] = end; }
                                }
                                if (__any(alive)) {
                                    BpHot H; int64_t tile_fpos;
                                    {
                                        const BpArgsPtr A = bp_args(A_);
                                        H.cold = &A_->P; H.tab = (GlbBytes)A->P.tab; H.tab2 = (GlbWords)A->X.tab2; H.maxerrors = me_; H.minoverlap = A->P.minoverlap; H.pitch = A->X.pitch;
                                        tile_fpos = A->fpos_base + (int64_t)g0;
                                    }
                                    bp_verify_rest<KK>(H, text, alive, croff, crl, p, kind, en_lo, en_hi, tile_fpos, SS);
                                }
                            }
                        }
                        if (run <= w0 + BP_Q2W) break;
                    }
                }
```

kvarq_amd/csrc/kernels_seeded.hip:

```cpp
#include "kvq_host.h"

#include <algorithm>
#include <string.h>

#ifdef KVQ_NO_PRIO
#define KVQ_SETPRIO(n) ((void)0)
#else
#define KVQ_SETPRIO(n) __builtin_amdgcn_s_setprio(n)
#endif
#define KVQ_K_MAX 8
#define ST_TILE 36640u
#define ST_TILE_MIN 30960u
#define ST_OV 4160u
#define ST_PRE 80u
#define ST_THREADS 512
#define ST_WAVES (ST_THREADS / 64)
#define ST_ROUNDS ((ST_TILE + ST_OV) / 16u / ST_THREADS + 1)
#define ST_NLCAP 2048
#define ST_RCAP 512
#define ST_QCAP 896
#define ST_Q2CAP 2048
#define ST_QW (ST_QCAP / ST_WAVES)
#define ST_Q2W (ST_Q2CAP / ST_WAVES)
#define ST_BLK 80u
#define ST_BUF (ST_PRE + ST_TILE + ST_OV)
#define ST_HIST_TILES 100u

#define TR_NONE 0xFFu
#define TR_FLAG_FALLBACK 0x2000000u
#define TR_FLAG_SKIPPED 0x4000000u
#define TR_FLAG_PARTIAL 0x8000000u
#define KVQ_SKIP_CAP 1024u

struct SeedEntry { uint64_t en, ctx; };
struct SeedTables {
    const uint32_t *bm1;
    const uint32_t *start;
    const SeedEntry *ent;
    const uint32_t *tab2;
    int32_t stride;
    int32_t pitch;
};

struct SeedIndex {
    int stride = 2;
    int k = 8;
    int pitch = 8;
    bool dense = false;
    DevBuf d_bm1, d_start, d_ent, d_tab2;
    SeedTables dev;
};

__host__ __device__ static inline uint32_t code2_of(uint8_t c) { return (c >> 1) & 3u; }

static uint32_t host_code(const uint8_t *p, int K)
{
    uint32_t c = 0;
    for (int i = 0; i < K; i++) c |= code2_of(p[i]) << (2 * i);
    return c;
}

int kvq_seed_k(const kvq_config &cfg)
{
    const int e = cfg.maxerrors;
    if (e < 0 || e > 6) return 0;
    if (cfg.Amin <= 13) return 0;
    int K = std::min(cfg.minoverlap, cfg.minreadlength) / (e + 1);
    if (K > KVQ_K_MAX) K = KVQ_K_MAX;
    if (const char *kv = getenv("KVQ_K")) { const int w = atoi(kv); if (w >= 5 && w < K) K = w; }
    return K >= 5 ? K : 0;
}

SeedIndex *kvq_seed_index_build(kvq_table *t)
{
    const kvq_config &cfg = t->cfg;
    t->seed_k = 0;
    const int e = cfg.maxerrors;
    const int K = kvq_seed_k(cfg);
    if (!K) return nullptr;
    auto pitch_of = [&](int stride) { return (K + stride - 1) / stride * stride; };
    auto span_of = [&](int stride) { return pitch_of(stride) * e + K + stride - 1; };
    int minlen = 1 << 30;
    for (int s = 0; s < t->nseq; s++) {
        const int len = t->h_off[s + 1] - t->h_off[s];
        bool ok = len >= span_of(2) && len <= 4095 && t->h_off[s] < (1 << 20) && s < (1 << 20);
        for (int i = 0; ok && i < len; i++) {
            const uint8_t c = t->h_tab[t->h_off[s] + i];
            ok = (c == 'A' || c == 'C' || c == 'G' || c == 'T');
        }
        if (ok) { t->seeded.push_back(s); t->is_seeded[s] = 1; minlen = std::min(minlen, len); }
    }
    if (t->seeded.empty()) return nullptr;
    t->seed_k = K;
    int stride = minlen >= span_of(8) ? 8 : minlen >= span_of(4) ? 4 : 2;
    if (const char *sv = getenv("KVQ_STRIDE")) { const int w = atoi(sv); if ((w == 2 || w == 4 || w == 8) && w <= stride) stride = w; }

    const int pitch = pitch_of(stride);
    struct Ent { uint32_t key; SeedEntry e; };
    std::vector<Ent> v;
    for (int s : t->seeded) {
        const uint8_t *q = &t->h_tab[t->h_off[s]];
        const int len = t->h_off[s + 1] - t->h_off[s];
        const uint64_t hi = ((uint64_t)(uint32_t)t->h_off[s] << 32) | ((uint64_t)(uint32_t)len << 52) | ((uint64_t)(uint32_t)s << 12);
        auto entry = [&](int pos, uint32_t all) -> Ent {
            uint64_t ctx = 0;
            for (int i = 0; i < 32; i++) { const int sp = pos - 16 + i; if (sp >= 0 && sp < len) ctx |= (uint64_t)code2_of(q[sp]) << (2 * i); }
            return Ent{ host_code(q + pos, K) + (all << (2 * K)), SeedEntry{ hi | (uint64_t)pos, ctx } };
        };
        for (int j = 0; j <= e; j++)
            for (int sft = 0; sft < stride; sft++) v.push_back(entry(j * pitch + sft, 0u));
        for (int p = 0; p + K <= len; p++) v.push_back(entry(p, 1u));
    }
    if (v.size() >= (1u << 22)) {
        t->seeded.clear(); std::fill(t->is_seeded.begin(), t->is_seeded.end(), 0); t->seed_k = 0;
        return nullptr;
    }
    SeedIndex *ix = new SeedIndex();
    ix->stride = stride; ix->k = K; ix->pitch = pitch;
    const uint32_t NC = 1u << (2 * K);
    std::vector<uint8_t> bm1(2 * NC / 8 < 64 ? 64 : 2 * NC / 8, 0);
    std::stable_sort(v.begin(), v.end(), [](const Ent &a, const Ent &b) { return a.key < b.key; });
    std::vector<uint32_t> start(2 * (size_t)NC + 2, 0); std::vector<SeedEntry> ent(v.size() + 1, SeedEntry{ 0, 0 });
    for (size_t i = 0; i < v.size(); i++) {
        bm1[v[i].key >> 3] |= (uint8_t)(1u << (v[i].key & 7));
        start[v[i].key + 1]++; ent[i] = v[i].e;
    }
    {
        size_t occ_anc = 0, occ_all = 0;
        for (uint32_t c = 0; c < NC; c++) { occ_anc += start[c + 1] != 0; occ_all += start[NC + c + 1] != 0; }
        const double expect = (double)occ_anc / NC * (150.0 / stride) + (double)occ_all / NC * 2 * (e + 1);
        ix->dense = expect > 5.0;
    }
    for (uint32_t c = 0; c < 2 * NC; c++) start[c + 1] += start[c];
    start[2 * (size_t)NC + 1] = start[2 * (size_t)NC];
    if (ix->d_start.ensure(start.size() * 4) != KVQ_OK || ix->d_ent.ensure(ent.size() * sizeof(SeedEntry)) != KVQ_OK ||
        hipMemcpy(ix->d_start.p, start.data(), start.size() * 4, hipMemcpyHostToDevice) != hipSuccess ||
        hipMemcpy(ix->d_ent.p, ent.data(), ent.size() * sizeof(SeedEntry), hipMemcpyHostToDevice) != hipSuccess ||
        ix->d_bm1.ensure(bm1.size()) != KVQ_OK || hipMemcpy(ix->d_bm1.p, bm1.data(), bm1.size(), hipMemcpyHostToDevice) != hipSuccess) {
        if (!kvq_error_code()) kvq_set_error(KVQ_ERR_DEVICE, "uploading the seed index failed");
        kvq_seed_index_destroy(ix);
        return nullptr;
    }
    ix->dev.bm1 = ix->d_bm1.as<uint32_t>();
    {
        const size_t nb = t->h_tab.size();
        std::vector<uint32_t> t2(nb / 16 + 3, 0);
        for (size_t i = 0; i < nb; i++) t2[i >> 4] |= code2_of(t->h_tab[i]) << (2 * (i & 15));
        if (ix->d_tab2.ensure(t2.size() * 4) != KVQ_OK || hipMemcpy(ix->d_tab2.p, t2.data(), t2.size() * 4, hipMemcpyHostToDevice) != hipSuccess) {
            if (!kvq_error_code()) kvq_set_error(KVQ_ERR_DEVICE, "uploading the seed index failed");
            kvq_seed_index_destroy(ix);
            return nullptr;
        }
        ix->dev.tab2 = ix->d_tab2.as<uint32_t>();
    }
    ix->dev.start = ix->d_start.as<uint32_t>(); ix->dev.ent = ix->d_ent.as<SeedEntry>();
    ix->dev.stride = stride; ix->dev.pitch = pitch;
    return ix;
}

void kvq_seed_index_destroy(SeedIndex *ix)
{
    if (!ix) return;
    DevBuf *b[] = { &ix->d_tab2, &ix->d_bm1, &ix->d_start, &ix->d_ent };
    for (DevBuf *x : b) x->release();
    delete ix;
}


__device__ __forceinline__ uint32_t lds_byte_at(uint32_t addr)
{
    return *reinterpret_cast<const __attribute__((address_space(3))) uint8_t *>((uintptr_t)addr);
}
__device__ __forceinline__ uint32_t rfl(uint32_t v) { return (uint32_t)__builtin_amdgcn_readfirstlane((int)v); }

typedef const __attribute__((address_space(1))) uint8_t *GlbBytes;
__device__ __forceinline__ uint32_t glb_u32(GlbBytes p)
{
    typedef uint32_t __attribute__((aligned(1))) u32_any;
    return *reinterpret_cast<const __attribute__((address_space(1))) u32_any *>(p);
}

__device__ __forceinline__ uint32_t good_flags(uint32_t x, uint32_t addk)
{
    return __builtin_amdgcn_bitop3_b32((x & 0x7F7F7F7Fu) + addk, 0x80808080u, x, 0x40);
}

__device__ __forceinline__ uint32_t mul_u24(uint32_t a, uint32_t b)
{
    uint32_t r;
    asm("v_mul_u32_u24 %0, %1, %2" : "=v"(r) : "v"(a), "v"(b));
    return r;
}

__device__ __forceinline__ void longest_run64(uint64_t m, int n, int &len, int &start)
{
    const uint64_t r1 = m & (m << 1), r2 = r1 & (r1 << 2), r3 = r2 & (r2 << 4), r4 = r3 & (r3 << 8), r5 = r4 & (r4 << 16);
    uint64_t E = n >= 64 ? ~0ull : ((1ull << n) - 1ull);
    int L = 0; uint64_t T;
    T = E & r5;        if (T) { E = T; L = 32; }
    T = E & (r4 << L); if (T) { E = T; L += 16; }
    T = E & (r3 << L); if (T) { E = T; L += 8; }
    T = E & (r2 << L); if (T) { E = T; L += 4; }
    T = E & (r1 << L); if (T) { E = T; L += 2; }
    T = E & (m << L);  if (T) { E = T; L += 1; }
    len = L;
    start = L ? (__ffsll((long long)E) - 1) - L + 1 : 0;
    if (m == ~0ull) { len = 64; start = 0; }
}

struct Seg { int len, pre, suf, best, bstart, beg; };

__device__ __forceinline__ Seg seg_merge(const Seg &A, const Seg &B)
{
    Seg R;
    R.beg = A.beg; R.len = A.len + B.len;
    R.pre = (A.pre == A.len) ? A.len + B.pre : A.pre;
    R.suf = (B.suf == B.len) ? B.len + A.suf : B.suf;
    R.best = A.best; R.bstart = A.bstart;
    const int cross = A.suf + B.pre;
    if (cross > R.best) { R.best = cross; R.bstart = A.beg + A.len - A.suf; }
    if (B.best > R.best) { R.best = B.best; R.bstart = B.bstart; }
    return R;
}

__device__ __forceinline__ int diff_bytes(uint32_t x, uint32_t y)
{
    const uint32_t v = x ^ y;
    return __popc(__builtin_amdgcn_bitop3_b32((v & 0x7F7F7F7Fu) + 0x7F7F7F7Fu, 0x80808080u, v, 0xC8));
}

__device__ __forceinline__ void emit_cold(const KvqParams *__restrict__ P, bool hit, int64_t fpos, int seq_nr,
                                          int seq_pos, int length, int rl, uint32_t key)
{
    const uint64_t m = __ballot(hit);
    if (m == 0) return;
    KvqHit *const arena = P->arena; const uint32_t cap = P->arena_cap; unsigned int *const arena_n = P->arena_n;
    const int leader = __ffsll((long long)m) - 1;
    uint32_t base = 0;
    if (kvq_lane() == leader) base = atomicAdd(arena_n, (unsigned int)__popcll(m));
    base = __shfl(base, leader, 64);
    if (hit) {
        const uint32_t idx = base + (uint32_t)__popcll(m & kvq_lanemask_lt());
        if (idx < cap) {
            KvqHit h;
            h.fpos = fpos; h.seq_nr = seq_nr; h.seq_pos = seq_pos; h.length = length;
            h.readlength = rl; h.key = key; h.blob_off = 0;
            arena[idx] = h;
        }
    }
}

#define ST_NO_BLOCK 0x7FFFFF00u
__host__ __device__ static inline bool kvq_tile_report_bad(uint32_t rep, bool first_tile, uint32_t seen, uint32_t total)
{
    const uint32_t n_owned = rep & 0xFFFFu, jn = (rep >> 16) & 0xFFu;
    if (rep & TR_FLAG_FALLBACK) return true;
    if ((rep & TR_FLAG_SKIPPED) && !(rep & TR_FLAG_PARTIAL)) return false;
    const uint32_t want = first_tile ? 0u : 4u - (seen & 3u);
    const bool expect = want <= n_owned && (first_tile || want + 2u <= total - seen);
    return expect ? jn != want : jn != TR_NONE;
}

extern "C" __global__ void __launch_bounds__(256)
kvq_validate_tiles(uint32_t nchunks, const uint32_t *__restrict__ tile_first, const uint32_t *__restrict__ tile_report,
                   unsigned int *__restrict__ spec_fail, KvqSkippedTile *__restrict__ skip_list,
                   const uint32_t *__restrict__ chunk_off, uint32_t tile_bytes)
{
    KVQ_BESIDE_SCAN();
    const uint32_t c = blockIdx.x * blockDim.x + threadIdx.x;
    if (c >= nchunks) return;
    uint32_t total = 0;
    for (uint32_t g = tile_first[c]; g < tile_first[c + 1]; g++) total += tile_report[g] & 0xFFFFu;
    uint32_t seen = 0;
    bool bad = false;
    for (uint32_t g = tile_first[c]; g < tile_first[c + 1]; g++) {
        const uint32_t rep = tile_report[g];
        if (kvq_tile_report_bad(rep, g == tile_first[c], seen, total)) bad = true;
        if ((rep & TR_FLAG_SKIPPED) && skip_list) {
            const unsigned int k = atomicAdd(spec_fail, 0x100u) >> 8;
            if (k < KVQ_SKIP_CAP) {
                const uint32_t a = chunk_off[c], e = chunk_off[c + 1], tn = g - tile_first[c];
                const uint32_t g0 = (a & ~15u) + tn * tile_bytes;
                KvqSkippedTile T;
                T.a = a; T.b = e; T.own_begin = tn == 0 ? a : g0; T.own_end = (uint64_t)g0 + tile_bytes < e ? g0 + tile_bytes : e;
                T.seen = seen; T.first = tn == 0 ? 1u : 0u;
                const uint32_t z = tile_report[tile_first[nchunks] + g];
                if (z) { T.a = T.own_begin = z - 1u; T.seen = 0; T.first = 1u; }
                skip_list[k] = T;
            } else bad = true;
        }
        seen += rep & 0xFFFFu;
    }
    if (bad) atomicOr(spec_fail, 1u);
}


extern "C" __global__ void __launch_bounds__(256)
kvq_expand_tiles(uint32_t nchunks, const uint32_t *__restrict__ chunk_off, const uint32_t *__restrict__ tile_first, uint4 *__restrict__ tile_tab, unsigned int *__restrict__ redo_count,
                 unsigned int *__restrict__ surv_count)
{
    KVQ_BESIDE_SCAN();
    const uint32_t c = blockIdx.x * blockDim.x + threadIdx.x;
    if (c == 0 && redo_count) { redo_count[0] = 0; redo_count[1] = 0; }
    if (c == 0 && surv_count) surv_count[0] = 0;
    if (c >= nchunks) return;
    const uint32_t a = chunk_off[c], b = chunk_off[c + 1], g0 = tile_first[c];
    for (uint32_t g = g0; g < tile_first[c + 1]; g++) tile_tab[g] = make_uint4(a, b, g - g0, c);
}

uint32_t kvq_choose_tile(uint32_t maxline, uint32_t rec_bytes)
{
    if (const char *e = getenv("KVQ_TILE")) { const int v = atoi(e); if (v >= 4000 && v <= (int)(ST_TILE + ST_OV - 1040u)) return (uint32_t)v / ST_BLK * ST_BLK; }
    if (maxline == 0) return ST_TILE;
    uint32_t ov = (4u * (maxline + 2u) + 160u + ST_BLK - 1u) / ST_BLK * ST_BLK;
    ov = std::max<uint32_t>(1040u, std::min<uint32_t>(ov, ST_OV));
    uint32_t tile = ST_TILE + ST_OV - ov;
    if (rec_bytes >= 40u) {
        const uint32_t n_full = tile / rec_bytes + 1u;
        uint32_t p = 1; while (2u * p <= n_full) p *= 2u;
        if (p >= 16u && p <= (uint32_t)ST_THREADS && n_full > p) {
            const uint32_t cut = (p - 1u) * rec_bytes / ST_BLK * ST_BLK;
            if (cut >= ST_TILE_MIN && (uint64_t)cut * 100u >= (uint64_t)tile * 78u) tile = cut;
        }
    }
    return tile;
}
uint32_t kvq_min_tile()
{
    if (getenv("KVQ_TILE")) return std::min<uint32_t>(ST_TILE_MIN, kvq_choose_tile(1u << 20, 0));
    return ST_TILE_MIN;
}

void kvq_probe_text(const uint8_t *text, size_t n, uint32_t &maxline, uint32_t &rec_bytes)
{
    uint32_t best = 0; size_t start = 0, lines = 0;
    for (size_t i = 0; i < n; i++)
        if (text[i] == '\n') { best = std::max<uint32_t>(best, (uint32_t)(i + 1 - start)); start = i + 1; lines++; }
    maxline = std::max<uint32_t>(best, (uint32_t)(n - start));
    rec_bytes = lines >= 16 ? (uint32_t)(start * 4 / lines) : 0u;
}
extern "C" uint32_t kvq_tile_for_text(const uint8_t *text, size_t n, uint32_t *rec_bytes_out)
{
    uint32_t maxline, rec_bytes;
    kvq_probe_text(text, n, maxline, rec_bytes);
    if (rec_bytes_out) *rec_bytes_out = rec_bytes;
    return kvq_choose_tile(maxline, rec_bytes);
}
```

kvarq_amd/csrc/kvq_launch.hip:

```cpp
#include "kvq_host.h"


int32_t kvq_scan_pick(int k, int stride, bool ix_dense, uint32_t rec_bytes, uint32_t tile_bytes, uint32_t dbg, int lg_env, int dense_env)
{
    if (k < 5 || k > 8 || (stride != 2 && stride != 4 && stride != 8)) return -1;
    const bool st = (dbg & 16u) != 0;
    int lg = -1;
    if (rec_bytes >= 40u) {
        const uint32_t n_full = tile_bytes / rec_bytes + 1u;
        if (n_full <= 128u && n_full > 64u) lg = 2;
        else if (n_full <= 64u && n_full > 32u) lg = 3;
        else if (n_full <= 256u && n_full > 128u) lg = 1;
    }
    if (lg_env >= -1) lg = lg_env >= 1 && lg_env <= 3 ? lg_env : -1;
    if ((lg == 3 || lg == 1) && st) lg = -1;
    const bool dense = k == 8 && !st && (dense_env >= 0 ? dense_env != 0 : ix_dense);
    const bool diag = ((dbg & ~16u) && !st) || k != 8 || dense;
    if (diag && lg != 2) lg = -1;
    return (int32_t)k | (int32_t)stride << 4 | (int32_t)(lg + 1) << 8 | (k < 8 || dense ? KVQ_CELL_DENSE : 0) |
           (diag ? KVQ_CELL_DIAG : 0) | (st && !diag ? KVQ_CELL_STAMPS : 0);
}

extern "C" int32_t kvq_scan_kernel_pick(int32_t k, int32_t stride, int32_t dense, uint32_t rec_bytes, uint32_t tile_bytes, uint32_t dbg)
{
    return kvq_scan_pick(k, stride, dense != 0, rec_bytes, tile_bytes, dbg, -2, -1);
}

extern "C" int32_t kvq_scan_kernel(const kvq_scan *s) { return s->kernel_cell; }

int kvq_seeded_launch(kvq_scan *s, const KvqParams &P, const uint8_t *d_data, int64_t nbytes,
                      const uint32_t *d_chunk_off, int64_t nchunks, int64_t fpos_base, uint32_t max_chunk_bytes)
{
    (void)nbytes; (void)max_chunk_bytes;
    SeedIndex *ix = s->t->index;
    const std::vector<int64_t> &co = s->cur_chunk_off;
    if (s->tile_bytes == 0) {
        const size_t n = (size_t)std::min<int64_t>(nbytes, 128 << 10);
        std::vector<uint8_t> head(n);
        KVQ_HIP(hipStreamSynchronize(s->stream));
        KVQ_HIP(hipMemcpy(head.data(), d_data, n, hipMemcpyDeviceToHost));
        s->tile_bytes = kvq_tile_for_text(head.data(), n, &s->rec_bytes);
    }
    const uint32_t TILE = s->tile_bytes;
    uint64_t nt = 0;
    for (int64_t c = 0; c < nchunks; c++) {
        const uint32_t a = (uint32_t)co[c], b = (uint32_t)co[c + 1];
        nt += b > a ? (uint32_t)(((uint64_t)b - (a & ~15u) + TILE - 1) / TILE) : 0u;
    }
    s->cur_ntiles = 0;
    if (nt == 0) {
        if (!s->ev_main.empty()) { KVQ_HIP(hipEventRecord(s->ev_main.back().first, s->stream)); KVQ_HIP(hipEventRecord(s->ev_main.back().second, s->stream)); }
        return KVQ_OK;
    }
    static const uint32_t grid_env = (uint32_t)(getenv("KVQ_GRID") ? atoi(getenv("KVQ_GRID")) : 0);
    const uint32_t cus = s->cus ? s->cus : (s->cus = kvq_device_cu_count());
    const uint32_t per_cu = 4u;
    const uint32_t grid_full = cus * per_cu, grid_shared = grid_full - cus / 4u;
    const uint32_t grid_cap = grid_env ? grid_env : (kvq_live_scans() > 1 && kvq_chain_busy(s)) ? grid_shared : grid_full;
    if (s->pool.used + ((size_t)nchunks + 1) * 4 + (size_t)nt * 24 + 24576 + KVQ_SKIP_CAP * sizeof(KvqSkippedTile) > s->pool.cap) {
        kvq_set_error(KVQ_ERR_RUNTIME, "batch tables outgrew their reservation"); return KVQ_ERR_RUNTIME;
    }
    const size_t first_b = (((size_t)nchunks + 1) * 4 + 255) & ~(size_t)255;
    const size_t ctr_b = 256 + 4 * BP_SHARDS * BP_SHARD_STRIDE;
    const size_t first_at = s->pool.take(first_b + sizeof(BpArgs) + ctr_b);
    const size_t chunk_at = s->pool.take((size_t)nt * 16), report_at = s->pool.take((size_t)nt * 8), skip_at = s->pool.take(KVQ_SKIP_CAP * sizeof(KvqSkippedTile));
    s->cur_skip_at = skip_at; s->cur_first_at = first_at; s->cur_ntiles = (uint32_t)nt;
    uint32_t *first = reinterpret_cast<uint32_t *>(s->pool.h + first_at);
    uint64_t acc = 0;
    for (int64_t c = 0; c < nchunks; c++) {
        const uint32_t a = (uint32_t)co[c], b = (uint32_t)co[c + 1];
        first[c] = (uint32_t)acc;
        acc += b > a ? (uint32_t)(((uint64_t)b - (a & ~15u) + TILE - 1) / TILE) : 0u;
    }
    first[nchunks] = (uint32_t)acc;
    static const uint32_t dbg = (uint32_t)(getenv("KVQ_DBG") ? atoi(getenv("KVQ_DBG")) : 0);
    const uint32_t grid_seeded = (uint32_t)std::min<uint64_t>(nt, grid_cap);
    uint32_t *d_first = reinterpret_cast<uint32_t *>(s->pool.d + first_at);
    const BpArgs *d_args = reinterpret_cast<const BpArgs *>(s->pool.d + first_at + first_b);
    uint32_t *d_tchunk = reinterpret_cast<uint32_t *>(s->pool.d + chunk_at);
    uint32_t *d_report = reinterpret_cast<uint32_t *>(s->pool.d + report_at);
    const size_t ctr_at = first_at + first_b + ((sizeof(BpArgs) + 127) & ~(size_t)127);
    unsigned int *d_tile_ctr = reinterpret_cast<unsigned int *>(s->pool.d + ctr_at);
    {
        BpArgs a;
        memset(&a, 0, sizeof(a));
        a.P = P; a.X = ix->dev; a.data = d_data; a.fpos_base = fpos_base;
        a.tiles = reinterpret_cast<const uint4 *>(d_tchunk); a.tile_report = d_report; a.tile_ctr = d_tile_ctr;
        static const uint32_t stagger = (uint32_t)(getenv("KVQ_STAGGER") ? atoi(getenv("KVQ_STAGGER")) : 0);
        a.ntiles = (uint32_t)nt; a.tile_bytes = TILE; a.dbg = dbg; a.pad_ = stagger;
        a.redo = s->d_redo.p; a.redo_cap = KVQ_REDO_CAP - KVQ_LONG_CAP; a.fail = s->cur_fail;
        static const bool surv_off = getenv("KVQ_SURVIVORS") && getenv("KVQ_SURVIVORS")[0] == '0';
        a.surv = surv_off ? nullptr : s->d_surv.p; a.surv_cap = s->surv_cap;
        memcpy(s->pool.h + first_at + first_b, &a, sizeof(a));
    }
    {
        unsigned int *hc = reinterpret_cast<unsigned int *>(s->pool.h + ctr_at);
        memset(hc, 0, 4 * BP_SHARDS * BP_SHARD_STRIDE);
        for (uint32_t sh = 0; sh < BP_SHARDS; sh++) hc[sh * BP_SHARD_STRIDE] = bp_shard_begin(sh, (uint32_t)nt);
    }
    KVQ_HIP(hipMemcpyAsync(s->pool.d + s->cur_co_at, s->pool.h + s->cur_co_at, ctr_at + 4 * BP_SHARDS * BP_SHARD_STRIDE - s->cur_co_at,
                           hipMemcpyHostToDevice, s->stream));
    hipLaunchKernelGGL(kvq_expand_tiles, dim3((uint32_t)((nchunks + 255) / 256)), dim3(256), 0, s->stream, (uint32_t)nchunks, d_chunk_off, d_first, reinterpret_cast<uint4 *>(d_tchunk),
                       s->d_redo.p ? KvqRedo(s->d_redo.p).count : (unsigned int *)nullptr, s->d_surv.p ? KvqSurvivors(s->d_surv.p).count : (unsigned int *)nullptr);

    bool pipelined = false;
    { const int rcw = kvq_chain_wait(s, &pipelined); if (rcw) return rcw; }
    const bool timed = !s->ev_main.empty();
    if (timed) KVQ_HIP(hipEventRecord(s->ev_main.back().first, s->stream));
    typedef void (*BpKernel)(const BpArgs *);
    {
        static const BpKernel kernels_diag[6] = { kvq_scan_bp<2, -1, false, true>, kvq_scan_bp<4, -1, false, true>, kvq_scan_bp<8, -1, false, true>,
                                                  kvq_scan_bp<2, 2, false, true>, kvq_scan_bp<4, 2, false, true>, kvq_scan_bp<8, 2, false, true> };
        static const BpKernel kernels_bp[18] = { kvq_scan_bp<2, -1, false>, kvq_scan_bp<4, -1, false>, kvq_scan_bp<8, -1, false>,
                                                 kvq_scan_bp<2, -1, true>, kvq_scan_bp<4, -1, true>, kvq_scan_bp<8, -1, true>,
                                                 kvq_scan_bp<2, 2, false>, kvq_scan_bp<4, 2, false>, kvq_scan_bp<8, 2, false>,
                                                 kvq_scan_bp<2, 2, true>, kvq_scan_bp<4, 2, true>, kvq_scan_bp<8, 2, true>,
                                                 kvq_scan_bp<2, 3, false>, kvq_scan_bp<4, 3, false>, kvq_scan_bp<8, 3, false>,
                                                 kvq_scan_bp<2, 1, false>, kvq_scan_bp<4, 1, false>, kvq_scan_bp<8, 1, false> };
        static const BpKernel kernels_k5[6] = { kvq_scan_bp<2, -1, false, true, 5>, kvq_scan_bp<4, -1, false, true, 5>, kvq_scan_bp<8, -1, false, true, 5>,
                                                kvq_scan_bp<2, 2, false, true, 5>, kvq_scan_bp<4, 2, false, true, 5>, kvq_scan_bp<8, 2, false, true, 5> };
        static const BpKernel kernels_k6[6] = { kvq_scan_bp<2, -1, false, true, 6>, kvq_scan_bp<4, -1, false, true, 6>, kvq_scan_bp<8, -1, false, true, 6>,
                                                kvq_scan_bp<2, 2, false, true, 6>, kvq_scan_bp<4, 2, false, true, 6>, kvq_scan_bp<8, 2, false, true, 6> };
        static const BpKernel kernels_k7[6] = { kvq_scan_bp<2, -1, false, true, 7>, kvq_scan_bp<4, -1, false, true, 7>, kvq_scan_bp<8, -1, false, true, 7>,
                                                kvq_scan_bp<2, 2, false, true, 7>, kvq_scan_bp<4, 2, false, true, 7>, kvq_scan_bp<8, 2, false, true, 7> };
        static const BpKernel kernels_dense[6] = { kvq_scan_bp<2, -1, false, true, 8, true>, kvq_scan_bp<4, -1, false, true, 8, true>, kvq_scan_bp<8, -1, false, true, 8, true>,
                                                   kvq_scan_bp<2, 2, false, true, 8, true>, kvq_scan_bp<4, 2, false, true, 8, true>, kvq_scan_bp<8, 2, false, true, 8, true> };
        static const int lg_env = getenv("KVQ_LG") ? atoi(getenv("KVQ_LG")) : -2;
        static const int dense_env = getenv("KVQ_DENSE") ? atoi(getenv("KVQ_DENSE")) : -1;
        const int32_t cell = kvq_scan_pick(ix->k, ix->stride, ix->dense, s->rec_bytes, TILE, dbg, lg_env, dense_env);
        if (cell < 0) { kvq_set_error(KVQ_ERR_RUNTIME, "no scan kernel for seeds of %d bases at stride %d", ix->k, ix->stride); return KVQ_ERR_RUNTIME; }
        const int si = ix->stride == 8 ? 2 : ix->stride == 4 ? 1 : 0, lg = ((cell >> 8) & 15) - 1;
        const int k = cell & 15;
        const bool dense = (cell & KVQ_CELL_DENSE) != 0, diag = (cell & KVQ_CELL_DIAG) != 0, stamps = (cell & KVQ_CELL_STAMPS) != 0;
        const BpKernel *const dk = k == 5 ? kernels_k5 : k == 6 ? kernels_k6 : k == 7 ? kernels_k7 : dense ? kernels_dense : kernels_diag;
        const BpKernel kern = diag ? dk[(lg == 2 ? 3 : 0) + si] : kernels_bp[lg == 3 ? 12 + si : lg == 1 ? 15 + si : (lg == 2 ? 6 : 0) + si + (stamps ? 3 : 0)];
        s->kernel_cell = cell;
        hipLaunchKernelGGL(kern, dim3(grid_seeded), dim3(ST_THREADS), 0, s->stream, d_args);
    }
    if (timed) KVQ_HIP(hipEventRecord(s->ev_main.back().second, s->stream));
    static const int sv_env = getenv("KVQ_SV_MODE") ? atoi(getenv("KVQ_SV_MODE")) : -1;
    const bool beside = sv_env >= 0 ? sv_env != 0 : pipelined;
    if (beside) { const int rcp = kvq_chain_publish(s); if (rcp) return rcp; }
    static const int sv_grid = getenv("KVQ_SV_GRID") ? atoi(getenv("KVQ_SV_GRID")) : 64;
    if (s->d_surv.p)
        hipLaunchKernelGGL(kvq_verify_survivors, dim3(beside ? sv_grid : 256), dim3(beside ? 256 : 1024), 0, s->stream, P, d_data, fpos_base, (const void *)s->d_surv.p,
                           (const unsigned int *)s->cur_fail, ix->k, ix->stride, ix->pitch);
    if (!beside) { const int rcp = kvq_chain_publish(s); if (rcp) return rcp; }
    if (!(dbg & 64u))
    hipLaunchKernelGGL(kvq_validate_tiles, dim3((uint32_t)((nchunks + 255) / 256)), dim3(256), 0, s->stream, (uint32_t)nchunks,
                       d_first, d_report, s->cur_fail, reinterpret_cast<KvqSkippedTile *>(s->pool.d + skip_at), d_chunk_off, TILE);
    KVQ_HIP(hipGetLastError());
    if (getenv("KVQ_DBG_REPORT")) {
        KVQ_HIP(hipStreamSynchronize(s->stream));
        std::vector<uint32_t> rep((size_t)nt);
        KVQ_HIP(hipMemcpy(rep.data(), d_report, (size_t)nt * 4, hipMemcpyDeviceToHost));
        for (int64_t c = 0; c < nchunks; c++) {
            uint32_t seen = 0, total = 0;
            for (uint32_t g = first[c]; g < first[c + 1]; g++) total += rep[g] & 0xFFFFu;
            for (uint32_t g = first[c]; g < first[c + 1]; g++) {
                if (kvq_tile_report_bad(rep[g], g == first[c], seen, total))
                    fprintf(stderr, "tile %u (chunk %lld [%lld, %lld), tile %u of it): report %08x n_owned %u jn %u seen %u of %u\n",
                            g, (long long)c, (long long)co[c], (long long)co[c + 1], g - first[c], rep[g], rep[g] & 0xFFFFu, (rep[g] >> 16) & 0xFFu, seen, total);
                seen += rep[g] & 0xFFFFu;
            }
        }
    }
    return KVQ_OK;
}
```

kvarq_amd/csrc/kvq_runtime.hip:

```cpp
#include "kvq_host.h"

#include <algorithm>
#include <atomic>
#include <mutex>
#include <stdarg.h>
#include <string.h>
#include <chrono>

static double now_ms() { return std::chrono::duration<double, std::milli>(std::chrono::steady_clock::now().time_since_epoch()).count(); }
static const bool g_timing = getenv("KVQ_TIMING") != nullptr;

#define KVQ_NEED_RESCAN (-2)


static thread_local int  tl_err_code = 0;
static thread_local char tl_err_msg[1024] = "";

void kvq_set_error(int code, const char *fmt, ...)
{
    tl_err_code = code;
    va_list ap; va_start(ap, fmt);
    vsnprintf(tl_err_msg, sizeof(tl_err_msg), fmt, ap);
    va_end(ap);
}
// ... 146 lines not shown
    for (int i = 0; i < nseq; i++) {
        if (seqlens[i] < 0) { kvq_set_error(KVQ_ERR_TYPE, "seqlist must be list of strings"); delete t; return nullptr; }
        t->h_off[i] = (int32_t)tot; tot += seqlens[i];
        if (tot > 0x7FFFFFFF) { kvq_set_error(KVQ_ERR_MEMORY, "sequence table too large"); delete t; return nullptr; }
    }
    t->h_off[nseq] = (int32_t)tot;
    t->bases = tot;
    t->h_tab.resize((size_t)tot + 64, 0);
    for (int i = 0; i < nseq; i++) if (seqlens[i]) memcpy(&t->h_tab[t->h_off[i]], seqs[i], (size_t)seqlens[i]);
    t->off_nseqhits = KVQ_CTR_RL_ + KVQ_RL_BINS;
    t->off_nseqbasehits = t->off_nseqhits + nseq;
    t->off_cov = t->off_nseqbasehits + nseq;
    t->off_mut = t->off_cov + tot;
    t->ctr_len = t->off_mut + 6 * tot;

    (void)hipGetDevice(&t->device);
    t->is_seeded.assign((size_t)nseq, 0);
    t->index = kvq_seed_index_build(t);
    if (kvq_error_code()) { kvq_table_destroy(t); return nullptr; }
    for (int i = 0; i < nseq; i++) if (!t->is_seeded[i]) t->exhaustive.push_back(i);

    std::vector<int32_t> all((size_t)nseq);
    for (int i = 0; i < nseq; i++) all[i] = i;
    bool ok = t->d_tab.ensure(t->h_tab.size()) == KVQ_OK && t->d_off.ensure((size_t)(nseq + 1) * 4) == KVQ_OK &&
              t->d_exh.ensure((size_t)(nseq + 1) * 4) == KVQ_OK && t->d_all.ensure((size_t)(nseq + 1) * 4) == KVQ_OK &&
              t->d_seeded.ensure((size_t)(nseq + 1) * 4) == KVQ_OK;
    if (ok) {
        ok = hipMemcpy(t->d_tab.p, t->h_tab.data(), t->h_tab.size(), hipMemcpyHostToDevice) == hipSuccess &&
             hipMemcpy(t->d_off.p, t->h_off.data(), (size_t)(nseq + 1) * 4, hipMemcpyHostToDevice) == hipSuccess &&
             (t->exhaustive.empty() || hipMemcpy(t->d_exh.p, t->exhaustive.data(), t->exhaustive.size() * 4, hipMemcpyHostToDevice) == hipSuccess) &&
             (t->seeded.empty() || hipMemcpy(t->d_seeded.p, t->seeded.data(), t->seeded.size() * 4, hipMemcpyHostToDevice) == hipSuccess) &&
             (nseq == 0 || hipMemcpy(t->d_all.p, all.data(), (size_t)nseq * 4, hipMemcpyHostToDevice) == hipSuccess);
        if (!ok) kvq_set_error(KVQ_ERR_DEVICE, "uploading the sequence table failed");
    }
    if (!ok) { kvq_table_destroy(t); return nullptr; }
    return t;
}

extern "C" void kvq_table_destroy(kvq_table *t)
{
    if (!t) return;
    {
        int cur = 0; (void)hipGetDevice(&cur);
        if (t->device != cur) (void)hipSetDevice(t->device);
        (void)hipDeviceSynchronize();
        if (t->device != cur) (void)hipSetDevice(cur);
    }
    if (t->index) kvq_seed_index_destroy(t->index);
    t->d_tab.release(); t->d_off.release(); t->d_exh.release(); t->d_all.release(); t->d_seeded.release();
    delete t;
}
extern "C" int32_t kvq_table_nseq(const kvq_table *t) { return t->nseq; }
extern "C" int64_t kvq_table_bases(const kvq_table *t) { return t->bases; }
extern "C" int32_t kvq_table_seq_is_seeded(const kvq_table *t, int32_t s) { return (s >= 0 && s < t->nseq) ? t->is_seeded[s] : 0; }
extern "C" int32_t kvq_table_seed_k(const kvq_table *t) { return t->seed_k; }
extern "C" int64_t kvq_counters_len(const kvq_table *t) { return t->ctr_len; }
extern "C" int64_t kvq_counters_off_nseqhits(const kvq_table *t) { return t->off_nseqhits; }
extern "C" int64_t kvq_counters_off_nseqbasehits(const kvq_table *t) { return t->off_nseqbasehits; }
extern "C" int64_t kvq_counters_off_coverage(const kvq_table *t) { return t->off_cov; }
extern "C" int64_t kvq_counters_off_mutations(const kvq_table *t) { return t->off_mut; }
extern "C" int64_t kvq_table_seq_offset(const kvq_table *t, int32_t s) { return (s >= 0 && s <= t->nseq) ? t->h_off[s] : -1; }


#define KVQ_MAX_BATCHES 65536
static const size_t SMALL_RANGE = 64, SMALL_FAIL = SMALL_RANGE + 4 * (KVQ_MAX_BATCHES + 1),
                    SMALL_STAGE = (SMALL_FAIL + 4 * KVQ_MAX_BATCHES + 255) & ~(size_t)255,
                    SMALL_BYTES = SMALL_STAGE + 8 * KVQ_STAGE_SLOTS * KVQ_STAGE_COPIES;

extern "C" __global__ void __launch_bounds__(256)
kvq_commit_batch(unsigned long long *stage, unsigned long long *ctr, unsigned long long *err_stage, unsigned long long *err,
                 const unsigned int *fail, unsigned int *arena_n, unsigned int *range)
{
    KVQ_BESIDE_SCAN();
    const bool bad = (*fail & 1u) != 0u;
    for (int i = threadIdx.x; i < KVQ_STAGE_SLOTS; i += blockDim.x) {
        unsigned long long v = 0;
        for (int c = 0; c < KVQ_STAGE_COPIES; c++) {
            const unsigned long long w = stage[(size_t)c * KVQ_STAGE_SLOTS + i];
            v = i == KVQ_CTR_LONGEST_ ? (v > w ? v : w) : v + w;
            stage[(size_t)c * KVQ_STAGE_SLOTS + i] = 0;
        }
        if (v && !bad) { if (i == KVQ_CTR_LONGEST_) atomicMax(&ctr[i], v); else atomicAdd(&ctr[i], v); }
    }
    if (threadIdx.x == 0) {
        if (bad) *arena_n = range[0];
        else if (*err_stage != ~0ull) atomicMin(err, *err_stage);
        *err_stage = ~0ull;
        range[1] = *arena_n;
    }
}

extern "C" __global__ void __launch_bounds__(256)
kvq_reset_state(unsigned long long *small, size_t small_words, unsigned long long *ctr, size_t ctr_words,
                unsigned long long *cov, size_t cov_words)
{
    KVQ_BESIDE_SCAN();
    const size_t i0 = (size_t)blockIdx.x * blockDim.x + threadIdx.x, step = (size_t)gridDim.x * blockDim.x;
    for (size_t i = i0; i < small_words; i += step) small[i] = (i == 2 || i == 3) ? ~0ull : 0ull;
    for (size_t i = i0; i < ctr_words; i += step) ctr[i] = 0ull;
    for (size_t i = i0; i < cov_words; i += step) cov[i] = 0ull;
}

extern "C" __global__ void __launch_bounds__(256)
kvq_publish_small(const unsigned int *__restrict__ small, const unsigned int *__restrict__ fail, unsigned int nbatches,
                  const unsigned int *__restrict__ state, unsigned int state_words,
                  unsigned int *host_small, unsigned int *host_fail, unsigned int *host_state)
{
    KVQ_BESIDE_SCAN();
    if (threadIdx.x < 8) host_small[threadIdx.x] = small[threadIdx.x];
    for (unsigned int i = threadIdx.x; i < nbatches; i += blockDim.x) host_fail[i] = fail[i];
    for (unsigned int i = threadIdx.x; i < state_words; i += blockDim.x) host_state[i] = state[i];
    __threadfence_system();
}

static KvqRecTable rec_table(const kvq_scan *s)
{
    KvqRecTable T;
    T.key = s->d_rkey.as<unsigned long long>(); T.off = s->d_roff.as<unsigned long long>(); T.len = s->d_rlen.as<unsigned int>();
    T.dir = s->d_rdir.as<unsigned int>(); T.ctr = s->d_rsmall.as<unsigned long long>();
    T.store = s->d_rstore.as<uint8_t>(); T.store_cap = s->rstore_cap; T.mask = s->rslots - 1u;
    return T;
}

static int records_prepare(kvq_scan *s)
{
    int rc;
    uint64_t slots = 1024; while (slots < 2ull * s->arena_cap) slots <<= 1;
    if (s->rstore_cap == 0) {
        unsigned long long cap = 32ull << 20;
        if (const char *e = getenv("KVQ_RECORD_CAP")) { const long long v = atoll(e); if (v >= 0 && (unsigned long long)v < cap) cap = (unsigned long long)v; }
        if ((rc = s->d_rstore.ensure((size_t)std::max<unsigned long long>(cap, 256) + 64))) return rc;
        s->rstore_cap = cap;
    }
    if ((rc = s->d_rsmall.ensure(256))) return rc;
    if (slots > s->rslots) {
        if ((rc = s->d_rkey.ensure((size_t)slots * 8)) || (rc = s->d_roff.ensure((size_t)slots * 8)) ||
            (rc = s->d_rlen.ensure((size_t)slots * 4)) || (rc = s->d_rdir.ensure((size_t)slots * 4))) return rc;
        KVQ_HIP(hipMemsetAsync(s->d_rkey.p, 0, (size_t)slots * 8, s->stream));
        s->rslots = (uint32_t)slots;
    } else {
        hipLaunchKernelGGL(kvq_records_clear, dim3(256), dim3(256), 0, s->stream, rec_table(s));
    }
    KVQ_HIP(hipMemsetAsync(s->d_rsmall.p, 0, 256, s->stream));
    KVQ_HIP(hipGetLastError());
    return KVQ_OK;
}

static int reset_device_state(kvq_scan *s)
{
    static_assert(SMALL_BYTES % 8 == 0, "kvq_reset_state writes 8-byte words");
    hipLaunchKernelGGL(kvq_reset_state, dim3(256), dim3(256), 0, s->stream, (unsigned long long *)s->d_small.p, SMALL_BYTES / 8,
                       s->d_ctr, (size_t)s->t->ctr_len, s->d_covdiff.as<unsigned long long>(), (size_t)s->t->bases + (size_t)s->t->nseq + 1);
    KVQ_HIP(hipGetLastError());
    if (s->records_on) return records_prepare(s);
    return KVQ_OK;
}

static int ensure_arena(kvq_scan *s, uint64_t hits, uint64_t blob)
{
    if (hits > 0xFFFFFFF0ull) { kvq_set_error(KVQ_ERR_MEMORY, "cannot allocate memory for results"); return KVQ_ERR_MEMORY; }
    if (hits > s->arena_cap) {
        int rc = s->d_arena.ensure((size_t)hits * sizeof(KvqHit)); if (rc) return rc;
        s->arena_cap = (uint32_t)hits;
    }
    if (blob > s->blob_cap) {
        if (blob > 0xFFFFFFF0ull) { kvq_set_error(KVQ_ERR_MEMORY, "cannot allocate memory for results"); return KVQ_ERR_MEMORY; }
        int rc = s->d_blob.ensure((size_t)blob); if (rc) return rc;
        s->blob_cap = blob;
    }
    return KVQ_OK;
}

static std::atomic<int> g_live_scans{0};
int kvq_live_scans() { return g_live_scans.load(); }
uint32_t kvq_device_cu_count()
{
    int dev = 0; hipDeviceProp_t pr;
    if (hipGetDevice(&dev) != hipSuccess || hipGetDeviceProperties(&pr, dev) != hipSuccess || pr.multiProcessorCount <= 0) return 256u;
    return (uint32_t)pr.multiProcessorCount;
}

extern "C" kvq_scan *kvq_scan_create(const kvq_table *t, void *d_counters)
{
    kvq_clear_error();
    kvq_scan *s = new kvq_scan();
    g_live_scans++;
    s->t = t;
    if (hipStreamCreateWithFlags(&s->stream, hipStreamNonBlocking) != hipSuccess) {
        kvq_set_error(KVQ_ERR_DEVICE, "hipStreamCreate failed"); delete s; return nullptr;
    }
    if (d_counters) { s->d_ctr = (unsigned long long *)d_counters; s->own_ctr = false; }
    else {
        if (s->d_ctr_own.ensure((size_t)t->ctr_len * 8) != KVQ_OK) { kvq_scan_destroy(s); return nullptr; }
        s->d_ctr = s->d_ctr_own.as<unsigned long long>(); s->own_ctr = true;
    }
    if (s->d_small.ensure(SMALL_BYTES) != KVQ_OK) { kvq_scan_destroy(s); return nullptr; }
    if (s->d_covdiff.ensure(((size_t)t->bases + (size_t)t->nseq + 1) * 8) != KVQ_OK) { kvq_scan_destroy(s); return nullptr; }
    s->d_arena_n = (unsigned int *)s->d_small.p;
    s->d_blob_n = (unsigned long long *)((char *)s->d_small.p + 8);
    s->d_err = (unsigned long long *)((char *)s->d_small.p + 16);
    s->d_err_stage = (unsigned long long *)((char *)s->d_small.p + 24);
    s->d_range = (unsigned int *)((char *)s->d_small.p + SMALL_RANGE);
    s->d_fail = (unsigned int *)((char *)s->d_small.p + SMALL_FAIL);
    s->d_stage_ctr = (unsigned long long *)((char *)s->d_small.p + SMALL_STAGE);
    if (ensure_arena(s, 1u << 20, 64ull << 20) != KVQ_OK) { kvq_scan_destroy(s); return nullptr; }
    if (s->d_surv.ensure(KvqSurvivors::bytes()) != KVQ_OK) { kvq_scan_destroy(s); return nullptr; }
    {
        unsigned int hdr[64] = { 0 };
        hdr[1] = KVQ_SURV_CAP;
        if (const char *e = getenv("KVQ_SURV_CAP")) { const long v = atol(e); if (v >= 0 && v < (long)KVQ_SURV_CAP) hdr[1] = (unsigned int)v; }
        s->surv_cap = hdr[1];
        if (hipMemcpyAsync(s->d_surv.p, hdr, 256, hipMemcpyHostToDevice, s->stream) != hipSuccess || hipStreamSynchronize(s->stream) != hipSuccess) { kvq_scan_destroy(s); return nullptr; }
    }
    if (s->d_redo.ensure(KvqRedo::bytes()) != KVQ_OK) { kvq_scan_destroy(s); return nullptr; }
    if (hipMemsetAsync(s->d_redo.p, 0, 256, s->stream) != hipSuccess) { kvq_scan_destroy(s); return nullptr; }
    s->pin_cap = (size_t)t->ctr_len * 8 + (4u << 20);
    {
        const size_t small_b = 64 + 4 * (size_t)KVQ_MAX_BATCHES + 512;
        size_t c = 0;
        s->pin_small = (uint8_t *)pinned_take(small_b, &c); s->pin_small_cap = c;
        s->pin = (uint8_t *)pinned_take(s->pin_cap, &c);
        if (s->pin) s->pin_cap = c;
        if (!s->pin_small || !s->pin) { kvq_set_error(KVQ_ERR_MEMORY, "cannot allocate memory for results"); kvq_scan_destroy(s); return nullptr; }
        memset(s->pin_small, 0, small_b);
    }
    memset(s->pin, 0, s->pin_cap < (1u << 20) ? s->pin_cap : (1u << 20));
    s->res = kvq_result_layout(0, 0);
    s->pin_res = s->pin + ((((size_t)t->ctr_len * 8) + 255) & ~(size_t)255);
    if (reset_device_state(s) != KVQ_OK) { kvq_scan_destroy(s); return nullptr; }
    s->h_ctr.assign((size_t)t->ctr_len, 0);
    return s;
}

static std::mutex g_chain_lock;
static hipEvent_t g_chain_done = nullptr;
static const kvq_scan *g_chain_owner = nullptr;

bool kvq_chain_busy(const kvq_scan *s)
{
    std::lock_guard<std::mutex> l(g_chain_lock);
    if (!g_chain_done || g_chain_owner == s) return false;
    const bool busy = hipEventQuery(g_chain_done) == hipErrorNotReady;
    (void)hipGetLastError();
    return busy;
}
int kvq_chain_wait(kvq_scan *s, bool *behind_a_running_scan)
{
    std::lock_guard<std::mutex> l(g_chain_lock);
    if (behind_a_running_scan) *behind_a_running_scan = false;
    if (g_chain_done && g_chain_owner != s) {
        if (behind_a_running_scan) { *behind_a_running_scan = hipEventQuery(g_chain_done) == hipErrorNotReady; (void)hipGetLastError(); }
        KVQ_HIP(hipStreamWaitEvent(s->stream, g_chain_done, 0));
    }
    return KVQ_OK;
}
int kvq_chain_publish(kvq_scan *s)
{
    if (!s->ev_chain) KVQ_HIP(hipEventCreateWithFlags(&s->ev_chain, hipEventDisableTiming));
    KVQ_HIP(hipEventRecord(s->ev_chain, s->stream));
    std::lock_guard<std::mutex> l(g_chain_lock);
    g_chain_done = s->ev_chain; g_chain_owner = s;
    return KVQ_OK;
}
static void chain_forget(const kvq_scan *s)
{
    std::lock_guard<std::mutex> l(g_chain_lock);
    if (g_chain_owner == s) { g_chain_done = nullptr; g_chain_owner = nullptr; }
}

static void drop_events(kvq_scan *s, bool destroy = false)
{
    for (auto *v : { &s->ev_all, &s->ev_main }) { s->ev_free.insert(s->ev_free.end(), v->begin(), v->end()); v->clear(); }
    if (destroy) {
        chain_forget(s);
        for (auto &e : s->ev_free) { (void)hipEventDestroy(e.first); (void)hipEventDestroy(e.second); }
        s->ev_free.clear();
    }
}

extern "C" void kvq_scan_destroy(kvq_scan *s)
{
    if (!s) return;
    g_live_scans--;
    if (s->stream) (void)hipStreamSynchronize(s->stream);
    drop_events(s, true);
    s->d_ctr_own.release();
    if (s->copy_stream) (void)hipStreamSynchronize(s->copy_stream);
    if (s->pin) pinned_give(s->pin, s->pin_cap);
    if (s->pin_small) pinned_give(s->pin_small, s->pin_small_cap);
    for (int i = 0; i < 2; i++) if (s->ev_copy[i]) (void)hipEventDestroy(s->ev_copy[i]);
    if (s->copy_stream) (void)hipStreamDestroy(s->copy_stream);
    if (s->ev_chain) (void)hipEventDestroy(s->ev_chain);
    if (s->pin_rec) pinned_give(s->pin_rec, s->pin_rec_cap);
    DevBuf *bufs[] = { &s->d_rkey, &s->d_roff, &s->d_rlen, &s->d_rdir, &s->d_rstore, &s->d_rsmall, &s->d_rres, &s->d_surv, &s->d_redo, &s->d_ctr_all, &s->d_gather_cnt, &s->d_gather_res, &s->d_sort_tmp, &s->d_sorted, &s->d_result, &s->d_order, &s->d_finish, &s->d_covdiff, &s->d_skipped, &s->d_chunk_off, &s->d_seg_base, &s->d_seg_cnt, &s->d_chunk_nrec, &s->d_rec_base, &s->d_nl4,
                       &s->d_rec_start, &s->d_read_off, &s->d_read_len, &s->d_arena, &s->d_blob, &s->d_small, &s->d_stage, &s->d_stage_b };
    for (DevBuf *b : bufs) b->release();
    s->pool.release();
    if (s->stream) (void)hipStreamDestroy(s->stream);
    delete s;
}

extern "C" int32_t kvq_scan_path(const kvq_scan *s) { return s->path_bits; }
extern "C" void kvq_scan_force_exhaustive(kvq_scan *s, int32_t on) { s->force_exhaustive = on != 0; }

extern "C" int32_t kvq_scan_set_records(kvq_scan *s, int32_t on)
{
    kvq_clear_error();
    if (!s->batches.empty() || s->copied_pending || s->host_pending >= 0) {
        kvq_set_error(KVQ_ERR_RUNTIME, "kvq_scan_set_records: only before the first batch or after kvq_scan_reset");
        return KVQ_ERR_RUNTIME;
    }
    if (on && s->comm) {
        kvq_set_error(KVQ_ERR_RUNTIME, "records are not gathered across ranks: a scan with a communicator cannot keep them");
        return KVQ_ERR_RUNTIME;
    }
    const bool was = s->records_on;
    s->records_on = on != 0;
    s->rec_store_bytes = 0;
    return s->records_on && !was ? records_prepare(s) : KVQ_OK;
}
extern "C" const uint8_t *kvq_scan_record_blob(const kvq_scan *s)
{
    return s->records_on && s->finished ? s->pin_rec + 256 + ((s->rec_hcap * 8 + 255) & ~255ull) + ((s->rec_hcap * 4 + 255) & ~255ull) : nullptr;
}
extern "C" const int64_t *kvq_scan_hit_record_off(const kvq_scan *s) { return s->records_on && s->finished ? reinterpret_cast<const int64_t *>(s->pin_rec + 256) : nullptr; }
extern "C" const int32_t *kvq_scan_hit_record_len(const kvq_scan *s)
{
    return s->records_on && s->finished ? reinterpret_cast<const int32_t *>(s->pin_rec + 256 + ((s->rec_hcap * 8 + 255) & ~255ull)) : nullptr;
}
extern "C" int64_t kvq_scan_record_bytes(const kvq_scan *s) { return s->records_on && s->finished ? s->rec_store_bytes : 0; }

extern "C" int32_t kvq_scan_reset(kvq_scan *s)
{
    kvq_clear_error();
    const double tr0 = now_ms();
    KVQ_HIP(hipStreamSynchronize(s->stream));
    drop_events(s);
    if (s->copy_stream) (void)hipStreamSynchronize(s->copy_stream);
    s->batches.clear(); s->host_batches = false; s->host_pending = -1; s->copied_pending = false; s->records = 0; s->parsed = 0; s->total = 0;
    s->ms_all = s->ms_main = 0; s->main_launches = 0; s->finished = false; s->reduced = false; s->gathered = false; s->path_bits = 0; s->kernel_cell = 0; s->n_hits = 0;
    s->tail_pending = false;
    s->pool.used = 0;
    const int rr = reset_device_state(s);
    if (g_timing) fprintf(stderr, "reset host %.3f ms\n", now_ms() - tr0);
    return rr;
}

static KvqParams make_params(const kvq_scan *s)
{
    const kvq_table *t = s->t;
    KvqParams P;
    P.maxerrors = t->cfg.maxerrors; P.minoverlap = t->cfg.minoverlap; P.minreadlength = t->cfg.minreadlength;
    P.amin = (int32_t)t->cfg.Amin; P.nseq = t->nseq;
    P.tab = t->d_tab.as<uint8_t>(); P.tab_off = t->d_off.as<int32_t>();
    P.ctr = s->d_ctr; P.covdiff = s->d_covdiff.as<unsigned long long>();
    P.off_nseqhits = t->off_nseqhits; P.off_nseqbasehits = t->off_nseqbasehits; P.off_cov = t->off_cov; P.off_mut = t->off_mut;
    P.arena = s->d_arena.as<KvqHit>(); P.arena_cap = s->arena_cap; P.arena_n = s->d_arena_n;
    P.blob = s->d_blob.as<uint8_t>(); P.blob_cap = s->blob_cap; P.blob_n = s->d_blob_n;
    P.err = s->d_err;
    return P;
}

static int new_event_pair(kvq_scan *s, std::vector<std::pair<hipEvent_t, hipEvent_t>> &v)
{
    if (!s->ev_free.empty()) { v.push_back(s->ev_free.back()); s->ev_free.pop_back(); return KVQ_OK; }
    hipEvent_t a, b;
    KVQ_HIP(hipEventCreate(&a)); KVQ_HIP(hipEventCreate(&b));
    v.emplace_back(a, b);
    return KVQ_OK;
}

static int run_batch(kvq_scan *s, const uint8_t *d_data, int64_t nbytes, const int64_t *chunk_off, int64_t nchunks,
                     int64_t fpos_base, size_t batch_no, bool exhaustive_only)
{
    const kvq_table *t = s->t;
    const double tb0 = now_ms();
    if (nbytes <= 0 || nchunks <= 0) return KVQ_OK;
    if (nbytes > 0xFFF00000ll) { kvq_set_error(KVQ_ERR_RUNTIME, "batch of %lld bytes is too large (< 4 GiB - 1 MiB)", (long long)nbytes); return KVQ_ERR_RUNTIME; }
    if (batch_no >= KVQ_MAX_BATCHES) { kvq_set_error(KVQ_ERR_RUNTIME, "too many batches in one scan"); return KVQ_ERR_RUNTIME; }
    if (((uintptr_t)d_data & 15u) != 0) { kvq_set_error(KVQ_ERR_RUNTIME, "device buffer must be 16-byte aligned"); return KVQ_ERR_RUNTIME; }

    KvqParams P = make_params(s);
    const bool use_seeded = t->index && !t->seeded.empty() && !s->force_exhaustive && !exhaustive_only;
    s->cur_chunk_off.assign(chunk_off, chunk_off + nchunks + 1);
    const std::vector<int32_t> *exh = &t->exhaustive;
    const int32_t *d_exh = t->d_exh.as<int32_t>();
    std::vector<int32_t> all;
    if (!use_seeded) { d_exh = t->d_all.as<int32_t>(); }
    const int32_t n_exh = use_seeded ? (int32_t)exh->size() : t->nseq;

    int rc;
    const size_t tiles_bound = (size_t)(nbytes / kvq_min_tile()) + (size_t)nchunks + 2;
    if ((rc = s->pool.reserve(((size_t)nchunks + 1) * 8 + tiles_bound * 24 + 65536, s->stream))) return rc;
    const size_t co_at = s->pool.take(((size_t)nchunks + 1) * 4);
    s->cur_co_at = co_at;
    uint32_t *co = reinterpret_cast<uint32_t *>(s->pool.h + co_at);
    const uint32_t *d_co = reinterpret_cast<const uint32_t *>(s->pool.d + co_at);
    std::vector<uint32_t> sb((size_t)nchunks + 1);
    uint32_t maxseg = 0, maxchunk = 0; uint64_t segs = 0;
    for (int64_t c = 0; c <= nchunks; c++) {
        if (chunk_off[c] < 0 || chunk_off[c] > nbytes || (c && chunk_off[c] < chunk_off[c - 1])) {
            kvq_set_error(KVQ_ERR_RUNTIME, "bad chunk offsets"); return KVQ_ERR_RUNTIME;
        }
        co[c] = (uint32_t)chunk_off[c];
    }
    for (int64_t c = 0; c < nchunks; c++) {
        const uint32_t a = co[c], b = co[c + 1];
        const uint32_t n = b > a ? (uint32_t)(((uint64_t)b - (a & ~15u) + KVQ_SEG_BYTES - 1) / KVQ_SEG_BYTES) : 0u;
        sb[c] = (uint32_t)segs; segs += n;
        maxseg = std::max(maxseg, n); maxchunk = std::max(maxchunk, b - a);
    }
    sb[nchunks] = (uint32_t)segs;
    if (!use_seeded) KVQ_HIP(hipMemcpyAsync(s->pool.d + co_at, co, ((size_t)nchunks + 1) * 4, hipMemcpyHostToDevice, s->stream));

    if ((rc = new_event_pair(s, s->ev_all))) return rc;
    KVQ_HIP(hipEventRecord(s->ev_all.back().first, s->stream));

    bool hist_done = false;
    if (use_seeded) {
        if ((rc = new_event_pair(s, s->ev_main))) return rc;
        KvqParams PS = P;
        PS.ctr = s->d_stage_ctr; PS.err = s->d_err_stage;
        s->cur_fail = s->d_fail + batch_no;
        if ((rc = kvq_seeded_launch(s, PS, d_data, nbytes, d_co, nchunks, fpos_base, maxchunk))) return rc;
        s->batches[batch_no].skip_at = s->cur_skip_at; s->batches[batch_no].tile_bytes = s->tile_bytes;
        s->main_launches++; s->path_bits |= 1;
        hist_done = true;
    }

    if (!hist_done || n_exh > 0) {
        if (n_exh > 0) s->path_bits |= 2;
        if ((rc = s->d_seg_base.ensure(sb.size() * 4))) return rc;
        if ((rc = s->d_seg_cnt.ensure((size_t)(segs + 1) * 4))) return rc;
        if ((rc = s->d_chunk_nrec.ensure((size_t)(nchunks + 1) * 4))) return rc;
        if ((rc = s->d_rec_base.ensure((size_t)(nchunks + 1) * 4))) return rc;
        KVQ_HIP(hipMemcpyAsync(s->d_seg_base.p, sb.data(), sb.size() * 4, hipMemcpyHostToDevice, s->stream));
        const uint32_t gx = std::max(1u, std::min(65u, (maxseg + 3) / 4));
        for (int64_t c0 = 0; c0 < nchunks; c0 += 32768) {
            const uint32_t ny = (uint32_t)std::min<int64_t>(32768, nchunks - c0);
            hipLaunchKernelGGL(kvq_count_lines, dim3(gx, ny), dim3(256), 0, s->stream, d_data,
                               d_co + c0, s->d_seg_base.as<uint32_t>() + c0, s->d_seg_cnt.as<uint32_t>());
        }
        hipLaunchKernelGGL(kvq_scan_segments, dim3((uint32_t)((nchunks + 3) / 4)), dim3(256), 0, s->stream, (uint32_t)nchunks,
                           s->d_seg_base.as<uint32_t>(), s->d_seg_cnt.as<uint32_t>(), s->d_chunk_nrec.as<uint32_t>());
        std::vector<uint32_t> nrec((size_t)nchunks), rbase((size_t)nchunks + 1);
        KVQ_HIP(hipMemcpyAsync(nrec.data(), s->d_chunk_nrec.p, (size_t)nchunks * 4, hipMemcpyDeviceToHost, s->stream));
        KVQ_HIP(hipStreamSynchronize(s->stream));
        uint64_t R = 0;
        for (int64_t c = 0; c < nchunks; c++) { rbase[c] = (uint32_t)R; R += nrec[c]; }
        rbase[nchunks] = (uint32_t)R;
        if (R > 0) {
            if ((rc = s->d_nl4.ensure((size_t)R * 16))) return rc;
            if ((rc = s->d_rec_start.ensure((size_t)R * 4))) return rc;
            if ((rc = s->d_read_off.ensure((size_t)R * 4))) return rc;
            if ((rc = s->d_read_len.ensure((size_t)R * 4))) return rc;
            KVQ_HIP(hipMemcpyAsync(s->d_rec_base.p, rbase.data(), rbase.size() * 4, hipMemcpyHostToDevice, s->stream));
            KVQ_HIP(hipStreamSynchronize(s->stream));
            for (int64_t c0 = 0; c0 < nchunks; c0 += 32768) {
                const uint32_t ny = (uint32_t)std::min<int64_t>(32768, nchunks - c0);
                hipLaunchKernelGGL(kvq_index_records, dim3(gx, ny), dim3(256), 0, s->stream, d_data,
                                   d_co + c0, s->d_seg_base.as<uint32_t>() + c0, s->d_seg_cnt.as<uint32_t>(),
                                   s->d_chunk_nrec.as<uint32_t>() + c0, s->d_rec_base.as<uint32_t>() + c0,
                                   s->d_nl4.as<uint32_t>(), s->d_rec_start.as<uint32_t>());
            }
            const uint32_t per_block = 4 * 16;
            hipLaunchKernelGGL(kvq_trim_records, dim3((uint32_t)((R + per_block - 1) / per_block)), dim3(256), 0, s->stream, P, d_data,
                               fpos_base, (uint32_t)R, KvqDevCount{ nullptr, 0, 0, nullptr }, s->d_nl4.as<uint32_t>(), s->d_rec_start.as<uint32_t>(),
                               s->d_read_off.as<uint32_t>(), s->d_read_len.as<int32_t>(), hist_done ? 0 : 1, 16u, (unsigned int *)nullptr, 0u);
            if (n_exh > 0) {
                const bool main_here = !use_seeded;
                if (main_here) { if ((rc = new_event_pair(s, s->ev_main))) return rc; KVQ_HIP(hipEventRecord(s->ev_main.back().first, s->stream)); }
                hipLaunchKernelGGL(kvq_match_all, dim3((uint32_t)((R + 3) / 4)), dim3(256), 0, s->stream, P, d_data, fpos_base, (uint32_t)R, KvqDevCount{ nullptr, 0, 0, nullptr },
                                   s->d_read_off.as<uint32_t>(), s->d_read_len.as<int32_t>(), d_exh, n_exh);
                if (main_here) { KVQ_HIP(hipEventRecord(s->ev_main.back().second, s->stream)); s->main_launches++; }
            }
        }
    }
    if (use_seeded && s->cur_ntiles) {
        const KvqRedo Rd(s->d_redo.p);
        unsigned int *const failw = s->d_fail + batch_no;
        const KvqSkippedTile *tiles = reinterpret_cast<const KvqSkippedTile *>(s->pool.d + s->cur_skip_at);
        const KvqDevCount ntile{ failw, 8, KVQ_SKIP_CAP, failw }, nrec{ Rd.count, 0, KVQ_REDO_CAP - KVQ_LONG_CAP, failw }, nlong{ Rd.count + 1, 0, 0xFFFFFFFFu, failw };
        hipLaunchKernelGGL(kvq_collect_skipped, dim3(16), dim3(256), 0, s->stream, d_data, tiles, 0u, ntile, Rd.nl4, Rd.rec_start, Rd.count, KVQ_REDO_CAP - KVQ_LONG_CAP);
        hipLaunchKernelGGL(kvq_trim_records, dim3(32), dim3(256), 0, s->stream, P, d_data, fpos_base, 0u, nrec, Rd.nl4, Rd.rec_start, Rd.read_off, Rd.read_len, 1, 1u, Rd.count + 1, KVQ_REDO_CAP - 1u);
        static const char *mg = getenv("KVQ_MGRID");
        const uint32_t lgrid = mg && atoi(mg) > 0 ? (uint32_t)atoi(mg) : 1536u;
        const dim3 ogrid = s->seen_skips ? dim3(128, (uint32_t)std::min<size_t>(s->t->seeded.size(), 4), 1) : dim3(16, (uint32_t)std::min<size_t>(s->t->seeded.size(), 4), 1);
        if (!s->t->seeded.empty()) {
            hipLaunchKernelGGL(kvq_match_all, ogrid, dim3(256), 0, s->stream, P, d_data, fpos_base, 0u, nrec,
                               Rd.read_off, Rd.read_len, s->t->d_seeded.as<int32_t>(), (int32_t)s->t->seeded.size());
            hipLaunchKernelGGL(kvq_match_long, dim3(s->seen_skips ? lgrid : 256u), dim3(256), 0, s->stream, P, d_data, fpos_base, nlong,
                               Rd.read_off, Rd.read_len, s->t->d_seeded.as<int32_t>(), (int32_t)s->t->seeded.size(), KVQ_REDO_CAP - 1u);
        }
    }
    if (use_seeded)
        hipLaunchKernelGGL(kvq_commit_batch, dim3(1), dim3(256), 0, s->stream, s->d_stage_ctr, s->d_ctr, s->d_err_stage, s->d_err,
                           (const unsigned int *)(s->d_fail + batch_no), s->d_arena_n, s->d_range + batch_no);
    else
        KVQ_HIP(hipMemcpyAsync(s->d_range + batch_no + 1, s->d_arena_n, 4, hipMemcpyDeviceToDevice, s->stream));
    hipLaunchKernelGGL(kvq_fold_batch, dim3(512), dim3(256), 0, s->stream, P, d_data, fpos_base,
                       (const unsigned int *)(s->d_range + batch_no), (const unsigned int *)(s->d_range + batch_no + 1));
    if (s->records_on)
        hipLaunchKernelGGL(kvq_gather_records, dim3(512), dim3(256), 0, s->stream, rec_table(s), (const KvqHit *)P.arena, P.arena_cap, d_data,
                           nbytes, fpos_base, d_co, (uint32_t)nchunks, (const unsigned int *)(s->d_range + batch_no), (const unsigned int *)(s->d_range + batch_no + 1));
    KVQ_HIP(hipEventRecord(s->ev_all.back().second, s->stream));
    KVQ_HIP(hipGetLastError());
    if (g_timing) fprintf(stderr, "run_batch host %.3f ms\n", now_ms() - tb0);
    return KVQ_OK;
}

static int check_batch(const void *data, int64_t nbytes, const int64_t *chunk_off, int64_t nchunks, size_t batch_no, bool device)
{
    if (nbytes > 0xFFF00000ll) { kvq_set_error(KVQ_ERR_RUNTIME, "batch of %lld bytes is too large (< 4 GiB - 1 MiB)", (long long)nbytes); return KVQ_ERR_RUNTIME; }
    if (batch_no >= KVQ_MAX_BATCHES) { kvq_set_error(KVQ_ERR_RUNTIME, "too many batches in one scan"); return KVQ_ERR_RUNTIME; }
    if (device && ((uintptr_t)data & 15u) != 0) { kvq_set_error(KVQ_ERR_RUNTIME, "device buffer must be 16-byte aligned"); return KVQ_ERR_RUNTIME; }
    for (int64_t c = 0; c <= nchunks; c++)
        if (chunk_off[c] < 0 || chunk_off[c] > nbytes || (c && chunk_off[c] < chunk_off[c - 1])) {
            kvq_set_error(KVQ_ERR_RUNTIME, "bad chunk offsets"); return KVQ_ERR_RUNTIME;
        }
    return KVQ_OK;
}

extern "C" int32_t kvq_scan_device(kvq_scan *s, const void *d_data, int64_t nbytes, const int64_t *chunk_off, int64_t nchunks, int64_t fpos_base)
{
    kvq_clear_error();
    if (nbytes <= 0 || nchunks <= 0) return KVQ_OK;
    int rc = check_batch(d_data, nbytes, chunk_off, nchunks, s->batches.size(), true); if (rc) return rc;
    Batch b; b.d_data = (const uint8_t *)d_data; b.nbytes = nbytes; b.fpos_base = fpos_base;
    b.chunk_off.assign(chunk_off, chunk_off + nchunks + 1);
    s->batches.push_back(b);
    s->parsed += nbytes; s->total += nbytes;
    return run_batch(s, (const uint8_t *)d_data, nbytes, chunk_off, nchunks, fpos_base, s->batches.size() - 1, false);
}

static DevBuf &stage_of(kvq_scan *s, int slot) { return slot == 0 ? s->d_stage : s->d_stage_b; }

static int settle_in_flight(kvq_scan *s)
{
    KVQ_HIP(hipStreamSynchronize(s->stream));
    if (s->host_pending < 0) return KVQ_OK;
    const size_t b = (size_t)s->host_pending;
    s->host_pending = -1;
    if (!(s->path_bits & 1)) return KVQ_OK;
    const unsigned int fail = *reinterpret_cast<const unsigned int *>(s->pin_small + 40);
    if (!fail) return KVQ_OK;
    if (!(fail & 1u)) { s->path_bits |= 8 | 2; s->seen_skips = true; return KVQ_OK; }
    s->batches[b].redone = true;
    s->tile_bytes = kvq_choose_tile(1u << 20, 0); s->rec_bytes = 0;
    Batch again = s->batches[b]; again.is_redo = true;
    s->batches.push_back(again);
    s->path_bits |= 4;
    int rc = run_batch(s, again.staged ? again.staged : stage_of(s, s->run_slot).as<uint8_t>(), again.nbytes, again.chunk_off.data(), (int64_t)again.chunk_off.size() - 1,
                       again.fpos_base, s->batches.size() - 1, true);
    if (rc) return rc;
    KVQ_HIP(hipStreamSynchronize(s->stream));
    return KVQ_OK;
}

static int launch_copied(kvq_scan *s)
{
    if (!s->copied_pending) return KVQ_OK;
    s->copied_pending = false;
    const int slot = s->copied_slot;
    DevBuf &stage = stage_of(s, slot);
    s->pool.used = 0;
    *reinterpret_cast<unsigned int *>(s->pin_small + 40) = 0;
    KVQ_HIP(hipStreamWaitEvent(s->stream, s->ev_copy[slot], 0));
    s->batches.push_back(s->copied);
    const Batch &b = s->batches.back();
    s->run_slot = slot;
    int rc = run_batch(s, stage.as<uint8_t>(), b.nbytes, b.chunk_off.data(), (int64_t)b.chunk_off.size() - 1, b.fpos_base, s->batches.size() - 1, false);
    if (rc) return rc;
    if (s->path_bits & 1)
        KVQ_HIP(hipMemcpyAsync(s->pin_small + 40, s->d_fail + (s->batches.size() - 1), 4, hipMemcpyDeviceToHost, s->stream));
    s->host_pending = (int64_t)s->batches.size() - 1;
    return KVQ_OK;
}

extern "C" int32_t kvq_scan_host_drain(kvq_scan *s)
{
    int rc;
    if ((rc = settle_in_flight(s))) return rc;
    if ((rc = launch_copied(s))) return rc;
    return settle_in_flight(s);
}

extern "C" int32_t kvq_scan_host_async(kvq_scan *s, const void *h_data, int64_t nbytes, const int64_t *chunk_off, int64_t nchunks, int64_t fpos_base)
{
    kvq_clear_error();
    if (nbytes <= 0 || nchunks <= 0) return KVQ_OK;
    int rc;
    if ((rc = check_batch(h_data, nbytes, chunk_off, nchunks, s->batches.size() + (s->copied_pending ? 1u : 0u), false))) return rc;
    if ((rc = settle_in_flight(s))) return rc;
    if ((rc = launch_copied(s))) return rc;
    const int slot = s->run_slot == 0 ? 1 : 0;
    DevBuf &stage = stage_of(s, slot);
    if ((rc = stage.ensure((size_t)nbytes + 64))) return rc;
    if (!s->copy_stream) KVQ_HIP(hipStreamCreateWithFlags(&s->copy_stream, hipStreamNonBlocking));
    for (int i = 0; i < 2; i++) if (!s->ev_copy[i]) KVQ_HIP(hipEventCreateWithFlags(&s->ev_copy[i], hipEventDisableTiming));
    if (s->tile_bytes == 0)
        s->tile_bytes = kvq_tile_for_text((const uint8_t *)h_data, (size_t)std::min<int64_t>(nbytes, 128 << 10), &s->rec_bytes);
    KVQ_HIP(hipMemcpyAsync(stage.p, h_data, (size_t)nbytes, hipMemcpyHostToDevice, s->copy_stream));
    KVQ_HIP(hipEventRecord(s->ev_copy[slot], s->copy_stream));
    s->copied = Batch(); s->copied.d_data = nullptr; s->copied.nbytes = nbytes; s->copied.fpos_base = fpos_base;
    s->copied.chunk_off.assign(chunk_off, chunk_off + nchunks + 1);
    s->copied_pending = true; s->copied_slot = slot;
    s->host_batches = true;
    s->parsed += nbytes; s->total += nbytes;
    if (s->host_pending >= 0) KVQ_HIP(hipEventSynchronize(s->ev_copy[s->run_slot]));
    return KVQ_OK;
}

int kvq_scan_staged(kvq_scan *s, const uint8_t *d_text, int64_t nbytes, const int64_t *chunk_off, int64_t nchunks, int64_t fpos_base)
{
    kvq_clear_error();
    if (nbytes <= 0 || nchunks <= 0) return KVQ_OK;
    int rc;
    if ((rc = check_batch(d_text, nbytes, chunk_off, nchunks, s->batches.size() + (s->copied_pending ? 1u : 0u), true))) return rc;
    if ((rc = settle_in_flight(s))) return rc;
    if ((rc = launch_copied(s))) return rc;
    if (s->tile_bytes == 0) {
        std::vector<uint8_t> head((size_t)std::min<int64_t>(nbytes, 128 << 10));
        KVQ_HIP(hipMemcpyAsync(head.data(), d_text, head.size(), hipMemcpyDeviceToHost, s->stream));
        KVQ_HIP(hipStreamSynchronize(s->stream));
        s->tile_bytes = kvq_tile_for_text(head.data(), head.size(), &s->rec_bytes);
    }
    s->pool.used = 0;
    *reinterpret_cast<unsigned int *>(s->pin_small + 40) = 0;
    Batch b; b.d_data = nullptr; b.staged = d_text; b.nbytes = nbytes; b.fpos_base = fpos_base;
    b.chunk_off.assign(chunk_off, chunk_off + nchunks + 1);
    s->batches.push_back(b);
    s->host_batches = true;
    s->parsed += nbytes; s->total += nbytes;
    rc = run_batch(s, d_text, nbytes, chunk_off, nchunks, fpos_base, s->batches.size() - 1, false);
    if (rc) return rc;
    if (s->path_bits & 1)
        KVQ_HIP(hipMemcpyAsync(s->pin_small + 40, s->d_fail + (s->batches.size() - 1), 4, hipMemcpyDeviceToHost, s->stream));
    s->host_pending = (int64_t)s->batches.size() - 1;
    return KVQ_OK;
}

extern "C" int32_t kvq_scan_host_copied(kvq_scan *s)
{
    if (s->copied_pending && s->ev_copy[s->copied_slot]) KVQ_HIP(hipEventSynchronize(s->ev_copy[s->copied_slot]));
    return KVQ_OK;
}

extern "C" int32_t kvq_scan_host(kvq_scan *s, const void *h_data, int64_t nbytes, const int64_t *chunk_off, int64_t nchunks, int64_t fpos_base)
{
    const int rc = kvq_scan_host_async(s, h_data, nbytes, chunk_off, nchunks, fpos_base);
    return rc ? rc : kvq_scan_host_copied(s);
}

static int records_tail(kvq_scan *s, const KvqFinishState *d_st)
{
    int rc;
    const size_t hoff = ((size_t)s->arena_cap * 8 + 255) & ~(size_t)255;
    if ((rc = s->d_rres.ensure(hoff + (size_t)s->arena_cap * 4 + 256))) return rc;
    long long *d_off = s->d_rres.as<long long>();
    int32_t *d_len = reinterpret_cast<int32_t *>(s->d_rres.as<uint8_t>() + hoff);
    hipLaunchKernelGGL(kvq_record_lookup, dim3(256), dim3(256), 0, s->stream, rec_table(s), d_st, (const uint8_t *)s->d_result.p, d_off, d_len);
    KVQ_HIP(hipGetLastError());
    s->rec_tail_n = s->rec_tail_b = 0;
    if (!s->pin_rec) return KVQ_OK;
    const uint64_t n = std::min<uint64_t>(std::min<uint64_t>(s->rec_spec_n, s->rec_hcap), s->arena_cap);
    const uint64_t b = std::min<uint64_t>(std::min<uint64_t>(s->rec_spec_b, s->rec_scap), s->rstore_cap);
    uint8_t *h_len = s->pin_rec + 256 + ((s->rec_hcap * 8 + 255) & ~255ull), *h_blob = h_len + ((s->rec_hcap * 4 + 255) & ~255ull);
    if (n) {
        KVQ_HIP(hipMemcpyAsync(s->pin_rec + 256, d_off, n * 8, hipMemcpyDeviceToHost, s->stream));
        KVQ_HIP(hipMemcpyAsync(h_len, d_len, n * 4, hipMemcpyDeviceToHost, s->stream));
    }
    if (b) KVQ_HIP(hipMemcpyAsync(h_blob, s->d_rstore.p, b, hipMemcpyDeviceToHost, s->stream));
    s->rec_tail_n = n; s->rec_tail_b = b;
    return KVQ_OK;
}

static int records_check(kvq_scan *s, uint64_t n_hits, unsigned long long *used, bool *grow)
{
    *grow = false;
    unsigned long long w[4] = { 0, 0, 0, 0 };
    KVQ_HIP(hipMemcpyAsync(w, s->d_rsmall.p, 32, hipMemcpyDeviceToHost, s->stream));
    KVQ_HIP(hipStreamSynchronize(s->stream));
    *used = w[0];
    if (w[0] <= s->rstore_cap && !w[2]) return KVQ_OK;
    unsigned long long want = w[0];
    if (n_hits > s->arena_cap && s->arena_cap) want = (unsigned long long)((double)w[0] * ((double)n_hits / s->arena_cap) * 1.25) + (1 << 20);
    want = std::max<unsigned long long>(want + want / 8, s->rstore_cap);
    if (want > 0xFFFFFFF0ull) { kvq_set_error(KVQ_ERR_MEMORY, "cannot allocate memory for results"); return KVQ_ERR_MEMORY; }
    int rc; if ((rc = s->d_rstore.ensure((size_t)want + 64))) return rc;
    s->rstore_cap = want;
    *grow = true;
    return KVQ_OK;
}

static int records_fetch(kvq_scan *s, uint64_t n_hits, unsigned long long used)
{
// ... 303 lines not shown
```

Measured before the change: 9.563 billion.

## Precompute per-tile geometry into 32-byte records and reload instead of keeping in registers

The tile table grows from a 16-byte (a,b,tn,chunk) entry to a 32-byte record that also holds g0, load_hi and packed local own/end bounds plus first/cut flags, computed once in the expand kernel. The scan kernel stops carrying Ja/Jb/Jt/g0/text/ntiles/amin and similar values across phases. It re-reads them from the constant-address tile record where needed and uses opaque asm to keep the wave index scalar. The aim is to reduce live register pressure and per-tile arithmetic, at the cost of extra scalar loads and doubled tile-table memory. A survivors query API and a host-side tile-record helper are added as well.

```diff
diff --git a/include/kvarq_hip.h b/include/kvarq_hip.h
--- a/include/kvarq_hip.h
+++ b/include/kvarq_hip.h
@@ -103,6 +103,7 @@
 int32_t kvq_scan_reset(kvq_scan *s);
 int32_t kvq_scan_path(const kvq_scan *s);
 void    kvq_scan_force_exhaustive(kvq_scan *s, int32_t on);
+int32_t kvq_scan_survivors(kvq_scan *s, uint32_t *asked, uint32_t *cap);
 
 #define KVQ_CELL_DENSE  0x1000
 #define KVQ_CELL_DIAG   0x2000
@@ -110,6 +111,7 @@
 int32_t kvq_scan_kernel_pick(int32_t k, int32_t stride, int32_t dense, uint32_t rec_bytes, uint32_t tile_bytes, uint32_t dbg);
 int32_t kvq_scan_kernel(const kvq_scan *s);
 uint32_t kvq_tile_for_text(const uint8_t *text, size_t n, uint32_t *rec_bytes_out);
+void    kvq_tile_record(uint32_t a, uint32_t b, uint32_t tn, uint32_t chunk, uint32_t tile_bytes, uint32_t *out);
 
 typedef struct kvq_comm kvq_comm;
 int32_t   kvq_comm_unique_id(void *id128);
diff --git a/kvarq_amd/_lib.py b/kvarq_amd/_lib.py
--- a/kvarq_amd/_lib.py
+++ b/kvarq_amd/_lib.py
@@ -94,9 +94,11 @@
     'kvq_scan_reset': (i32, [vp]),
     'kvq_scan_path': (i32, [vp]),
     'kvq_scan_force_exhaustive': (None, [vp, i32]),
+    'kvq_scan_survivors': (i32, [vp, P(C.c_uint32), P(C.c_uint32)]),
     'kvq_scan_kernel_pick': (i32, [i32, i32, i32, C.c_uint32, C.c_uint32, C.c_uint32]),
     'kvq_scan_kernel': (i32, [vp]),
     'kvq_tile_for_text': (C.c_uint32, [vp, C.c_size_t, P(C.c_uint32)]),
+    'kvq_tile_record': (None, [C.c_uint32, C.c_uint32, C.c_uint32, C.c_uint32, C.c_uint32, P(C.c_uint32)]),
     'kvq_comm_unique_id': (i32, [vp]),
     'kvq_comm_create': (vp, [i32, i32, vp]),
     'kvq_comm_destroy': (None, [vp]),
diff --git a/kvarq_amd/csrc/kernels_bp.hip b/kvarq_amd/csrc/kernels_bp.hip
--- a/kvarq_amd/csrc/kernels_bp.hip
+++ b/kvarq_amd/csrc/kernels_bp.hip
@@ -33,6 +33,7 @@
     __attribute__((aligned(16))) uint8_t head[BP_HEAD];
     __attribute__((aligned(16))) uint32_t wtot[ST_WAVES];
     uint32_t longest_p1, records, fallback, n_owned, next_tile, first_tile, p2_jn;
+    uint32_t wjn[ST_WAVES];
     uint32_t sv_at[ST_WAVES], sv_end[ST_WAVES];
 };
 static_assert(sizeof(BpLds) <= 40 * 1024, "four workgroups per CU: at most 40 KB of LDS each");
@@ -178,7 +179,7 @@
     KvqParams P;
     SeedTables X;
     const uint8_t *data; int64_t fpos_base;
-    const uint4 *tiles; uint32_t *tile_report; unsigned int *tile_ctr;
+    const KvqTileRec *tiles; uint32_t *tile_report; unsigned int *tile_ctr;
     void *redo;
     unsigned int *fail;
     void *surv;
@@ -214,6 +215,7 @@
         if (t < bp_shard_begin(pick + 1u, ntiles)) return t;
     }
 }
+__device__ __forceinline__ uint32_t bp_opaque(uint32_t v) { asm volatile("" : "+s"(v)); return v; }
 typedef const __attribute__((address_space(4))) BpArgs *BpArgsPtr;
 __device__ __forceinline__ BpArgsPtr bp_args(const BpArgs *A)
 {
@@ -221,6 +223,19 @@
     asm volatile("" : "+s"(p));
     return p;
 }
+typedef const __attribute__((address_space(4))) uint32_t *BpTilePtr;
+#define BP_T_G0 4
+#define BP_T_LOAD_HI 5
+#define BP_T_OWN 6
+#define BP_T_END 7
+__device__ __forceinline__ BpTilePtr bp_tile(BpArgsPtr A, uint32_t g)
+{
+    asm volatile("" : "+s"(g));
+    return (BpTilePtr)A->tiles + (size_t)g * (sizeof(KvqTileRec) / 4u);
+}
+__device__ __forceinline__ GlbBytes bp_text(BpArgsPtr A, BpTilePtr T) { return (GlbBytes)A->data + T[BP_T_G0] - ST_PRE; }
+static_assert(offsetof(KvqTileRec, g0) == 4 * BP_T_G0 && offsetof(KvqTileRec, load_hi) == 4 * BP_T_LOAD_HI && offsetof(KvqTileRec, own) == 4 * BP_T_OWN &&
+              offsetof(KvqTileRec, end) == 4 * BP_T_END, "the words of a tile's record");
 
 #ifndef BP_OCC
 #define BP_OCC 8
@@ -281,7 +296,7 @@
     __shared__ __align__(16) BpLds S;
     uint8_t *const lds_raw = reinterpret_cast<uint8_t *>(&S);
     int tid = threadIdx.x, lane = tid & 63;
-    const uint32_t wave = rfl((uint32_t)tid >> 6);
+    const uint32_t wave_k = rfl((uint32_t)tid >> 6);
     if ((uint32_t)(uintptr_t)((__attribute__((address_space(3))) uint8_t *)lds_raw) != 0u) __builtin_trap();
     unsigned long long stamp_acc[8] = { 0, 0, 0, 0, 0, 0, 0, 0 }, stamp_t = 0, wave_p34 = 0;
     unsigned long long rt_in = 0, rt_pro = 0, rt_first = 0;
@@ -294,20 +309,23 @@
     if constexpr (STAMPS) rt_in = __builtin_amdgcn_s_memrealtime();
 #define BSTAMP(i) do { if constexpr (STAMPS) { const unsigned long long now_ = __builtin_amdgcn_s_memtime(); stamp_acc[i] += now_ - stamp_t; stamp_t = now_; } } while (0)
 
-    uint32_t ntiles, tile_bytes, dbg, amin;
+    uint32_t dbg;
     {
         const BpArgsPtr A = bp_args(A_);
-        ntiles = A->ntiles; tile_bytes = A->tile_bytes; dbg = DIAG ? A->dbg : 0u; amin = (uint32_t)A->P.amin;
+        dbg = DIAG ? A->dbg : 0u;
         const GlbWords bm1 = (GlbWords)A->X.bm1;
         for (int i = tid; i < (1 << (2 * KK)) / 32; i += ST_THREADS) reinterpret_cast<uint32_t *>(S.bmA)[i] = bm1[i];
     }
-    uint32_t my_shard = blockIdx.x % BP_SHARDS; bool no_more = false;
-    if (wave == ST_WAVES - 1u) {
-        unsigned int *const ctr = bp_args(A_)->tile_ctr;
+#define BP_NO_MORE 0x80000000u
+    uint32_t my_shard = blockIdx.x % BP_SHARDS;
+    if (wave_k == ST_WAVES - 1u) {
+        const BpArgsPtr A = bp_args(A_);
+        unsigned int *const ctr = A->tile_ctr;
+        const uint32_t ntiles = A->ntiles;
         const uint32_t t0 = bp_draw_wave(ctr, ntiles, my_shard, (uint32_t)lane);
         const uint32_t t1 = t0 < ntiles ? bp_draw_wave(ctr, ntiles, my_shard, (uint32_t)lane) : ntiles;
-        no_more = t1 >= ntiles;
         if (lane == 0) { S.first_tile = t0; S.next_tile = t1; }
+        if (t1 >= ntiles) my_shard |= BP_NO_MORE;
     }
     for (int i = tid; i < KVQ_RL_BINS / 2; i += ST_THREADS) S.hist[i] = 0;
     if (tid == 0) { S.longest_p1 = 0; S.records = 0; S.fallback = 0; }
@@ -321,7 +339,6 @@
     if (const uint32_t stg = bp_args(A_)->pad_) { for (uint32_t i = 0; i < (blockIdx.x >> 8) * stg; i++) __builtin_amdgcn_s_sleep(127); }
     if constexpr (STAMPS) rt_pro = __builtin_amdgcn_s_memrealtime();
     unsigned long long *const ctr_stamps = bp_args(A_)->P.ctr + KVQ_CTR_RL_ + 924;
-    const uint32_t addk = (0x80u - amin) * 0x01010101u;
     uint32_t tiles_done = 0;
     uint32_t g_done = 0xFFFFFFFFu;
     uint32_t my_longest = 0;
@@ -329,27 +346,31 @@
         asm volatile("" : "+v"(tid));
         lane = tid & 63;
         const uint32_t blk = (uint32_t)tid * ST_BLK;
+        uint32_t wave = bp_opaque(wave_k);
         const uint32_t wv = wave * (ST_BLK * 64u / 16u) + (uint32_t)lane;
         if constexpr (STAMPS) stamp_t = __builtin_amdgcn_s_memtime();
-        uint32_t Ja = 0, Jb = 0, Jt = 0, g0 = 0; GlbBytes text = nullptr;
+#define BP_TILE(A, g, dbg) bp_tile((A), ((dbg) & 64u) ? ((g) & 63u) : (g))
+#define BP_TEXT(A_, g, dbg) bp_text(bp_args(A_), BP_TILE(bp_args(A_), g, dbg))
+        bool live; uint32_t own_w = 0, end_w = 0;
         uint4 pre[ST_ROUNDS];
 #pragma unroll
         for (int r = 0; r < (int)ST_ROUNDS; r++) pre[r] = make_uint4(0, 0, 0, 0);
-        if (g < ntiles) {
-            const BpArgsPtr A = bp_args(A_);
-            const u32x4_t q = ((const __attribute__((address_space(4))) u32x4_t *)A->tiles)[(dbg & 64u) ? (g & 63u) : g];
-            Ja = q.x; Jb = q.y; Jt = q.z;
-            g0 = (Ja & ~15u) + Jt * tile_bytes;
+        {
+        const BpArgsPtr A = bp_args(A_);
+        live = g < A->ntiles;
+        if (live) {
+            const BpTilePtr T = BP_TILE(A, g, dbg);
+            const uint32_t g0 = T[BP_T_G0], load_hi = T[BP_T_LOAD_HI];
+            own_w = T[BP_T_OWN]; end_w = T[BP_T_END];
             const uint8_t *const data = A->data;
-            text = (GlbBytes)data + g0 - ST_PRE;
-            const uint32_t load_hi = g0 + ST_TILE + ST_OV < Jb ? g0 + ST_TILE + ST_OV : Jb;
             const uint32_t vo = 16u * wv - ST_PRE, vo0 = wv >= ST_PRE / 16u ? vo : ST_NO_BLOCK;
-            const __amdgpu_buffer_rsrc_t rs = __builtin_amdgcn_make_buffer_rsrc((void *)(data + g0), 0, (int)(((load_hi + 15u) & ~15u) - g0), 0x00020000);
+            const __amdgpu_buffer_rsrc_t rs = __builtin_amdgcn_make_buffer_rsrc((void *)(data + g0), 0, (int)(((load_hi + 15u) & ~15u) - g0), (int)bp_opaque(0x00020000u));
 #pragma unroll
             for (int r = 0; r < (int)ST_ROUNDS; r++) {
                 const u32x4_t v = __builtin_amdgcn_raw_buffer_load_b128(rs, (int)(r ? vo + 1024u * r : vo0), 0, KVQ_TEXT_AUX);
                 pre[r] = make_uint4(v.x, v.y, v.z, v.w);
             }
+        }
         }
         __syncthreads();
         unsigned long long sub_t0 = 0, sub_t1 = 0;
@@ -357,17 +378,16 @@
         if (g_done != 0xFFFFFFFFu) {
             if (tid == 0 && S.fallback) { atomicOr(&bp_args(A_)->tile_report[g_done], TR_FLAG_FALLBACK); S.fallback = 0; }
         }
-        if (g >= ntiles) break;
+        if (!live) break;
         const uint32_t gn = rfl(S.next_tile);
-        const uint32_t own_end = g0 + tile_bytes < Jb ? g0 + tile_bytes : Jb;
-        const uint32_t load_hi = g0 + ST_TILE + ST_OV < Jb ? g0 + ST_TILE + ST_OV : Jb;
-        const uint32_t own_begin_l = (Jt == 0 ? Ja : g0) - g0 + ST_PRE;
-        const uint32_t own_end_l = own_end - g0 + ST_PRE;
-        const uint32_t end_l = load_hi - g0 + ST_PRE;
 
         {
-            const uint32_t w_lo = wave * (ST_BLK * 64u), w_hi = w_lo + ST_BLK * 64u;
-            const bool cut = ((own_begin_l & 15u) && own_begin_l > w_lo && own_begin_l < w_hi) || ((end_l & 15u) && end_l > w_lo && end_l < w_hi);
+            const uint32_t own_begin_l = own_w & 0xFFFFu, end_l = end_w & 0xFFFFu;
+            bool cut = false;
+            if ((own_begin_l | end_l) & 15u) {
+                const uint32_t w_lo = bp_opaque(wave_k) * (ST_BLK * 64u), w_hi = w_lo + ST_BLK * 64u;
+                cut = ((own_begin_l & 15u) && own_begin_l > w_lo && own_begin_l < w_hi) || ((end_l & 15u) && end_l > w_lo && end_l < w_hi);
+            }
             if (cut) {
                 uint32_t wv_ = wv;
                 asm volatile("" : "+v"(wv_));
@@ -385,6 +405,7 @@
         KVQ_MARK("P0 vectors");
         {
             const uint32_t pa = 2u * wv, ca = 4u * wv;
+            const uint32_t addk = (0x80u - (uint32_t)bp_args(A_)->P.amin) * 0x01010101u;
 #pragma unroll
             for (int r = 0; r < (int)ST_ROUNDS; r++) {
                 uint32_t n16, g16, c32;
@@ -393,7 +414,7 @@
                 *reinterpret_cast<__attribute__((address_space(3))) uint16_t *>((uintptr_t)(BP_LDS_GDP + pa + 128u * r)) = (uint16_t)g16;
                 *reinterpret_cast<__attribute__((address_space(3))) uint32_t *>((uintptr_t)(ca + 256u * r)) = c32;
             }
-            if (wave == 0u) {
+            if (bp_opaque(wave_k) == 0u) {
 #pragma unroll
                 for (int r = 0; r < (int)(BP_HEAD / 1024u); r++)
                     *reinterpret_cast<__attribute__((address_space(3))) u32x4_t *>((uintptr_t)(BP_LDS_HEAD + 16u * (uint32_t)lane + 1024u * r)) = u32x4_t{ pre[r].x, pre[r].y, pre[r].z, pre[r].w };
@@ -409,6 +430,7 @@
         static_assert(ST_BLK == 80u, "five vectors per block");
         const uint32_t cnt = (uint32_t)(__popc(m0) + __popc(m1) + __popc(m2));
         const uint32_t incl = kvq_wave_incl_scan(cnt);
+        wave = bp_opaque(wave_k);
         if (lane == 63) S.wtot[wave] = incl;
         KVQ_MARK("P0 scan end");
         if constexpr (STAMPS) { if (tid == 0) { atomicAdd(&ctr_stamps[0], sub_t0 - stamp_t); atomicAdd(&ctr_stamps[1], sub_t1 - sub_t0); } }
@@ -417,6 +439,7 @@
         KVQ_MARK("P1b");
         BSTAMP(1);
         uint32_t n_all = 0;
+        wave = bp_opaque(wave_k);
         {
             uint32_t run = S.wtot[lane & 7];
             run += (uint32_t)__builtin_amdgcn_update_dpp(0, (int)run, 0x111, 0xf, 0xf, false);
@@ -425,7 +448,10 @@
             n_all = (uint32_t)__builtin_amdgcn_readlane((int)run, 7);
             const uint32_t upto = (uint32_t)__builtin_amdgcn_readlane((int)run, (int)wave);
             uint32_t n = upto - (uint32_t)__builtin_amdgcn_readlane((int)incl, 63) + incl - cnt;
-            if (blk < own_end_l && blk + ST_BLK >= own_end_l) S.n_owned = n + cnt;
+            {
+                const uint32_t own_end_l = BP_TILE(bp_args(A_), g, dbg)[BP_T_OWN] >> 16;
+                if (blk < own_end_l && blk + ST_BLK >= own_end_l) S.n_owned = n + cnt;
+            }
             if (__any(cnt != 0u)) {
                 if (n_all <= BP_NLCAP && !__any(cnt > 2u)) {
                     auto low80 = [](uint32_t w0, uint32_t w1, uint32_t w2) -> uint32_t {
@@ -459,15 +485,18 @@
         if (wave == 0u) {
             const uint32_t cnt0 = (uint32_t)__builtin_amdgcn_readlane((int)incl, 63);
             uint32_t early = BP_P2_LATE;
-            if (Jt != 0 && cnt0 >= 10u) {
+            const BpTilePtr T = BP_TILE(bp_args(A_), g, dbg);
+            const uint32_t end_w1 = T[BP_T_END];
+            if (!(end_w1 & KVQ_TILE_FIRST) && cnt0 >= 10u) {
                 const uint32_t m = (uint32_t)lane;
                 bool ok = false;
                 if (m >= 1 && m <= 8) {
                     const uint32_t e0 = S.nl[m - 1], e2 = S.nl[m + 1];
                     const uint32_t ls0 = e0 + 1u, ls2 = e2 + 1u;
+                    const uint32_t own_end_l = T[BP_T_OWN] >> 16, end_l = end_w1 & 0xFFFFu;
                     if (e0 < own_end_l && ls0 < end_l && ls2 < end_l) {
-                        const uint32_t c0 = ls0 < BP_HEAD ? lds_byte_at(BP_LDS_HEAD + ls0) : (uint32_t)text[ls0];
-                        const uint32_t c2 = ls2 < BP_HEAD ? lds_byte_at(BP_LDS_HEAD + ls2) : (uint32_t)text[ls2];
+                        const uint32_t c0 = ls0 < BP_HEAD ? lds_byte_at(BP_LDS_HEAD + ls0) : (uint32_t)BP_TEXT(A_, g, dbg)[ls0];
+                        const uint32_t c2 = ls2 < BP_HEAD ? lds_byte_at(BP_LDS_HEAD + ls2) : (uint32_t)BP_TEXT(A_, g, dbg)[ls2];
                         ok = c0 == '@' && c2 == '+';
                     }
                 }
@@ -485,7 +514,9 @@
             const uint32_t n_nl = n_all < BP_NLCAP ? n_all : BP_NLCAP;
             const uint32_t n_owned = rfl(S.n_owned);
             uint32_t fallback = n_all > BP_NLCAP ? 1u : 0u;
-            if (Jt == 0) jn = 0;
+            const BpTilePtr T = BP_TILE(bp_args(A_), g, dbg);
+            const uint32_t end_w2 = T[BP_T_END];
+            if (end_w2 & KVQ_TILE_FIRST) jn = 0;
             else if (const uint32_t early = rfl(S.p2_jn); early != BP_P2_LATE) jn = early;
             else {
                 const uint32_t m = (uint32_t)lane;
@@ -493,9 +524,10 @@
                 if (m >= 1 && m <= 8 && m <= n_owned && m + 2 <= n_nl) {
                     const uint32_t ls0 = (uint32_t)S.nl[m - 1] + 1u;
                     const uint32_t ls2 = (uint32_t)S.nl[m + 1] + 1u;
+                    const uint32_t end_l = end_w2 & 0xFFFFu;
                     if (ls0 < end_l && ls2 < end_l) {
-                        const uint32_t c0 = ls0 < BP_HEAD ? lds_byte_at(BP_LDS_HEAD + ls0) : (uint32_t)text[ls0];
-                        const uint32_t c2 = ls2 < BP_HEAD ? lds_byte_at(BP_LDS_HEAD + ls2) : (uint32_t)text[ls2];
+                        const uint32_t c0 = ls0 < BP_HEAD ? lds_byte_at(BP_LDS_HEAD + ls0) : (uint32_t)BP_TEXT(A_, g, dbg)[ls0];
+                        const uint32_t c2 = ls2 < BP_HEAD ? lds_byte_at(BP_LDS_HEAD + ls2) : (uint32_t)BP_TEXT(A_, g, dbg)[ls2];
                         ok = c0 == '@' && c2 == '+';
                     }
                 }
@@ -507,20 +539,21 @@
                 if (jn <= n_owned) nrec = (n_owned - jn) / 4u + 1u;
                 if (nrec > 0 && jn + 4u * nrec > n_nl) {
                     const uint32_t fit = n_nl >= jn ? (n_nl - jn) / 4u : 0u;
-                    if (load_hi < Jb) left = 1u;
+                    if (end_w2 & KVQ_TILE_CUT) left = 1u;
                     if (n_all > BP_NLCAP) fallback = 1u;
                     nrec = fit;
                 }
                 if (nrec > ST_RCAP) { nrec = ST_RCAP; fallback = 1u; }
             }
             if (fallback) { nrec = 0; left = 1u; }
+            S.wjn[wave] = jn;
             if (tid == 0 || tid == ST_THREADS - 64) {
                 const BpArgsPtr A = bp_args(A_);
                 if (tid == 0) {
                     A->tile_report[g] = (n_owned & 0xFFFFu) | ((jn & 0xFFu) << 16) | (left ? TR_FLAG_SKIPPED : 0u) | (left && nrec ? TR_FLAG_PARTIAL : 0u);
-                    if (left) A->tile_report[ntiles + g] = nrec ? g0 - ST_PRE + (uint32_t)S.nl[jn + 4u * nrec - 1u] + 2u : 0u;
+                    if (left) A->tile_report[A->ntiles + g] = nrec ? BP_TILE(A, g, dbg)[BP_T_G0] - ST_PRE + (uint32_t)S.nl[jn + 4u * nrec - 1u] + 2u : 0u;
                     S.records += nrec;
-                } else if (!no_more) drawn = atomicAdd(&A->tile_ctr[my_shard * BP_SHARD_STRIDE], 1u);
+                } else if (!(my_shard & BP_NO_MORE)) drawn = atomicAdd(&A->tile_ctr[my_shard * BP_SHARD_STRIDE], 1u);
             }
         }
 
@@ -536,6 +569,7 @@
         if (dbg & 32u) nrec = 0;
         KVQ_MARK("P2 end / P3 setup");
         BSTAMP(3);
+        wave = bp_opaque(wave_k);
         if (wave >= 4u) KVQ_SETPRIO(2); else KVQ_SETPRIO(1);
         unsigned long long wave_t3 = 0;
         if constexpr (STAMPS) wave_t3 = __builtin_amdgcn_s_memtime();
@@ -549,17 +583,17 @@
         const uint32_t G = 1u << lg, RP = ST_THREADS >> lg;
         const uint32_t gl = (uint32_t)tid & (G - 1u), gr = (uint32_t)tid >> lg;
         for (uint32_t pass0 = 0; pass0 < nrec; pass0 += RP) {
-            const uint32_t k = pass0 + gr;
-            const bool have = k < nrec;
+#define BP_GL0(tid, G) ({ asm volatile("" : "+v"(tid)); ((uint32_t)(tid) & ((G) - 1u)) == 0u; })
+            uint32_t k = pass0 + gr;
             uint32_t roff = 0; int rl = 0;
-            uint32_t c0, cp;
-            if (have) {
-                const uint32_t m = jn + 4u * k;
-                const uint32_t rstart = m == 0 ? ST_PRE + (Ja & 15u) : (uint32_t)S.nl[m - 1] + 1u;
+            uint32_t c0 = '@', cp = '+';
+            if (k < nrec) {
+                const uint32_t m = S.wjn[wave] + 4u * k;
+                const uint32_t rstart = m == 0 ? ST_PRE + ((BP_TILE(bp_args(A_), g, dbg)[BP_T_END] >> 16) & 15u) : (uint32_t)S.nl[m - 1] + 1u;
                 const uint32_t n0 = S.nl[m], n1 = S.nl[m + 1], n2 = S.nl[m + 2], n3 = S.nl[m + 3];
                 const uint32_t sread = n0 + 1u, plus = n1 + 1u, sscore = n2 + 1u;
         KVQ_MARK("trim");
-                if (gl == 0) { if (dbg & 8u) { c0 = '@'; cp = '+'; } else { c0 = text[rstart]; cp = text[plus]; } }
+                if (BP_GL0(tid, G)) { if (dbg & 8u) { c0 = '@'; cp = '+'; } else { const GlbBytes text = BP_TEXT(A_, g, dbg); c0 = text[rstart]; cp = text[plus]; } }
                 const int Q = (int)(n3 - sscore);
                 const int per = (Q + (int)G - 1) >> lg;
                 Seg sg; sg.beg = (int)mul_u24(gl, (uint32_t)per); if (sg.beg > Q) sg.beg = Q;
@@ -615,7 +649,7 @@
                     roff = sread + (uint32_t)__shfl(sg.bstart, lane & ~(int)(G - 1u), 64);
                 }
                 my_longest = my_longest > (uint32_t)(rl + 1) ? my_longest : (uint32_t)(rl + 1);
-                if (gl == 0) {
+                if (BP_GL0(tid, G)) {
                     if (rl < KVQ_RL_BINS) atomicAdd(&S.hist[rl >> 1], 1u << (16 * (rl & 1)));
                     S.rinfo[k] = roff | ((uint32_t)rl << 16);
                 }
@@ -624,13 +658,15 @@
             BSTAMP(4);
             KVQ_SETPRIO(2);
             const uint32_t rpw = 64u >> lg, grw = (uint32_t)lane >> lg;
+            wave = bp_opaque(wave_k);
             const uint32_t wfirst = pass0 + wave * rpw;
             const uint32_t npass = wfirst < nrec ? (nrec - wfirst < rpw ? nrec - wfirst : rpw) : 0u;
             uint32_t *const q1 = S.q1 + wave * BP_QW; uint32_t *const q2 = S.q2 + wave * BP_Q2W;
             uint32_t sub = (dbg & 128u) ? npass : 0u, step = rpw;
             while (sub < npass) {
                 BTALLY(6, lane == 0);
-                asm volatile("" : "+v"(rl), "+v"(roff));
+                asm volatile("" : "+v"(rl), "+v"(roff), "+v"(k));
+                const bool have = k < nrec;
                 int minrl, me_; const __attribute__((address_space(1))) uint8_t *bmL;
                 {
                     const BpArgsPtr A = bp_args(A_);
@@ -698,15 +734,16 @@
                 BSTAMP(5);
                 KVQ_SETPRIO(3);
 
+                if (!DENSE && qn > BP_QW && step > 1u) step >>= 1;
+                else {
                 if constexpr (!DENSE) {
                 const bool over = qn > BP_QW;
                 const uint32_t qn_ok = (over || (dbg & 1u)) ? 0u : qn;
-                if (over && step > 1u) { step >>= 1; continue; }
                 if (over) {
-                    if (mine && gl == 0) {
+                    if (mine && BP_GL0(tid, G)) {
                         const BpArgsPtr A = bp_args(A_);
                         const KvqRedo Rd(A->redo);
-                        const uint32_t boff = g0 - ST_PRE + roff;
+                        const uint32_t boff = BP_TILE(A, g, dbg)[BP_T_G0] - ST_PRE + roff;
                         bool put = false;
                         if (A->redo) {
                             if (rl >= KVQ_LONG_READ) {
@@ -775,13 +812,15 @@
                 }
                 KVQ_SETPRIO(2);
                 sub += step;
+                }
             }
             KVQ_SETPRIO(0);
-            if (have && gl == 0 && (c0 != '@' || cp != '+')) {
+            if (c0 != '@' || cp != '+') {
                 const BpArgsPtr A = bp_args(A_);
-                const uint32_t m = jn + 4u * k;
-                const uint32_t rstart = m == 0 ? ST_PRE + (Ja & 15u) : (uint32_t)S.nl[m - 1] + 1u, plus = (uint32_t)S.nl[m + 1] + 1u;
-                const int64_t tf = A->fpos_base + (int64_t)g0;
+                const uint32_t m = S.wjn[bp_opaque(wave_k)] + 4u * k;
+                const BpTilePtr T = BP_TILE(A, g, dbg);
+                const uint32_t rstart = m == 0 ? ST_PRE + ((T[BP_T_END] >> 16) & 15u) : (uint32_t)S.nl[m - 1] + 1u, plus = (uint32_t)S.nl[m + 1] + 1u;
+                const int64_t tf = A->fpos_base + (int64_t)T[BP_T_G0];
                 if (c0 != '@') atomicMin(A->P.err, ((unsigned long long)(tf + rstart - ST_PRE) << 16) | (0ull << 8) | c0);
                 else atomicMin(A->P.err, ((unsigned long long)(tf + plus - ST_PRE) << 16) | (1ull << 8) | cp);
             }
@@ -789,11 +828,14 @@
             BSTAMP(6);
         }
         if constexpr (STAMPS) wave_p34 += __builtin_amdgcn_s_memtime() - wave_t3;
-        if (wave == ST_WAVES - 1u) {
+        if (bp_opaque(wave_k) == ST_WAVES - 1u) {
+            const BpArgsPtr A = bp_args(A_);
+            const uint32_t ntiles = A->ntiles;
+            const bool no_more = (my_shard & BP_NO_MORE) != 0u;
             uint32_t d = no_more ? ntiles : rfl(drawn);
             if (!no_more && d >= bp_shard_begin(my_shard + 1u, ntiles)) {
-                d = bp_draw_wave(bp_args(A_)->tile_ctr, ntiles, my_shard, (uint32_t)tid & 63u);
-                no_more = d >= ntiles;
+                d = bp_draw_wave(A->tile_ctr, ntiles, my_shard, (uint32_t)tid & 63u);
+                if (d >= ntiles) my_shard |= BP_NO_MORE;
             }
             if ((tid & 63) == 0) S.next_tile = d;
         }
@@ -803,6 +845,7 @@
         g_done = g; g = gn;
     }
 
+    const uint32_t wave = wave_k;
     unsigned long long rt_loop = 0;
     if constexpr (STAMPS) rt_loop = __builtin_amdgcn_s_memrealtime();
     {
@@ -835,6 +878,12 @@
         if (S.records) atomicAdd(&ctr[KVQ_CTR_RECORDS_], (unsigned long long)S.records);
     }
 }
+#undef BP_NO_MORE
+#undef BP_TILE
+#undef BP_TEXT
+#undef BP_GL0
+#undef BSTAMP
+#undef BTALLY
 
 __device__ __forceinline__ bool seed_same_text(GlbBytes x, GlbBytes y, int K)
 {
diff --git a/kvarq_amd/csrc/kernels_bp_p4.inc b/kvarq_amd/csrc/kernels_bp_p4.inc
--- a/kvarq_amd/csrc/kernels_bp_p4.inc
+++ b/kvarq_amd/csrc/kernels_bp_p4.inc
@@ -80,9 +80,10 @@
                                         }
                                     }
                                     if (at + na <= end && end != 0u) {
+                                        const uint32_t sv_g0 = BP_TILE(bp_args(A_), g, dbg)[BP_T_G0];
                                         if (alive) {
                                             KvqSurvivor v;
-                                            v.boff = g0 - ST_PRE + croff; v.rl = (uint16_t)crl; v.p = (uint16_t)p; v.en = ((uint64_t)en_hi << 32) | en_lo; v.kind = kind; v.pad = 0;
+                                            v.boff = sv_g0 - ST_PRE + croff; v.rl = (uint16_t)crl; v.p = (uint16_t)p; v.en = ((uint64_t)en_hi << 32) | en_lo; v.kind = kind; v.pad = 0;
                                             Sv.item[at + (uint32_t)__popcll(am & kvq_lanemask_lt())] = v;
                                             alive = false;
                                         }
@@ -91,9 +92,12 @@
                                     if (lane == 0) { S.sv_at[wave] = at; S.sv_end[wave] = end; }
                                 }
                                 if (__any(alive)) {
-                                    BpHot H; int64_t tile_fpos;
+                                    BpHot H; int64_t tile_fpos; GlbBytes text;
                                     {
                                         const BpArgsPtr A = bp_args(A_);
+                                        const BpTilePtr T = BP_TILE(A, g, dbg);
+                                        const uint32_t g0 = T[BP_T_G0];
+                                        text = bp_text(A, T);
                                         H.cold = &A_->P; H.tab = (GlbBytes)A->P.tab; H.tab2 = (GlbWords)A->X.tab2; H.maxerrors = me_; H.minoverlap = A->P.minoverlap; H.pitch = A->X.pitch;
                                         tile_fpos = A->fpos_base + (int64_t)g0;
                                     }
diff --git a/kvarq_amd/csrc/kernels_seeded.hip b/kvarq_amd/csrc/kernels_seeded.hip
--- a/kvarq_amd/csrc/kernels_seeded.hip
+++ b/kvarq_amd/csrc/kernels_seeded.hip
@@ -295,9 +295,34 @@
 }
 
 
+struct KvqTileRec { uint32_t a, b, tn, chunk, g0, load_hi, own, end; };
+static_assert(sizeof(KvqTileRec) == 32, "two 16-byte vectors per tile");
+#define KVQ_TILE_FIRST (1u << 20)
+#define KVQ_TILE_CUT (1u << 21)
+__host__ __device__ static inline KvqTileRec kvq_tile_rec(uint32_t a, uint32_t b, uint32_t tn, uint32_t chunk, uint32_t tile_bytes)
+{
+    KvqTileRec T;
+    T.a = a; T.b = b; T.tn = tn; T.chunk = chunk;
+    const uint32_t g0 = (a & ~15u) + tn * tile_bytes;
+    const uint32_t own_end = g0 + tile_bytes < b ? g0 + tile_bytes : b;
+    const uint32_t load_hi = g0 + ST_TILE + ST_OV < b ? g0 + ST_TILE + ST_OV : b;
+    const uint32_t own_begin_l = (tn == 0 ? a : g0) - g0 + ST_PRE;
+    const uint32_t own_end_l = own_end - g0 + ST_PRE;
+    const uint32_t end_l = load_hi - g0 + ST_PRE;
+    T.g0 = g0; T.load_hi = load_hi;
+    T.own = (own_begin_l & 0xFFFFu) | (own_end_l << 16);
+    T.end = (end_l & 0xFFFFu) | ((a & 15u) << 16) | (tn == 0 ? KVQ_TILE_FIRST : 0u) | (load_hi < b ? KVQ_TILE_CUT : 0u);
+    return T;
+}
+extern "C" void kvq_tile_record(uint32_t a, uint32_t b, uint32_t tn, uint32_t chunk, uint32_t tile_bytes, uint32_t *out)
+{
+    const KvqTileRec T = kvq_tile_rec(a, b, tn, chunk, tile_bytes);
+    memcpy(out, &T, sizeof(T));
+}
+
 extern "C" __global__ void __launch_bounds__(256)
-kvq_expand_tiles(uint32_t nchunks, const uint32_t *__restrict__ chunk_off, const uint32_t *__restrict__ tile_first, uint4 *__restrict__ tile_tab, unsigned int *__restrict__ redo_count,
-                 unsigned int *__restrict__ surv_count)
+kvq_expand_tiles(uint32_t nchunks, const uint32_t *__restrict__ chunk_off, const uint32_t *__restrict__ tile_first, KvqTileRec *__restrict__ tile_tab, uint32_t tile_bytes,
+                 unsigned int *__restrict__ redo_count, unsigned int *__restrict__ surv_count)
 {
     KVQ_BESIDE_SCAN();
     const uint32_t c = blockIdx.x * blockDim.x + threadIdx.x;
@@ -305,7 +330,7 @@
     if (c == 0 && surv_count) surv_count[0] = 0;
     if (c >= nchunks) return;
     const uint32_t a = chunk_off[c], b = chunk_off[c + 1], g0 = tile_first[c];
-    for (uint32_t g = g0; g < tile_first[c + 1]; g++) tile_tab[g] = make_uint4(a, b, g - g0, c);
+    for (uint32_t g = g0; g < tile_first[c + 1]; g++) tile_tab[g] = kvq_tile_rec(a, b, g - g0, c, tile_bytes);
 }
 
 uint32_t kvq_choose_tile(uint32_t maxline, uint32_t rec_bytes)
diff --git a/kvarq_amd/csrc/kvq_launch.hip b/kvarq_amd/csrc/kvq_launch.hip
--- a/kvarq_amd/csrc/kvq_launch.hip
+++ b/kvarq_amd/csrc/kvq_launch.hip
@@ -57,13 +57,13 @@
     const uint32_t per_cu = 4u;
     const uint32_t grid_full = cus * per_cu, grid_shared = grid_full - cus / 4u;
     const uint32_t grid_cap = grid_env ? grid_env : (kvq_live_scans() > 1 && kvq_chain_busy(s)) ? grid_shared : grid_full;
-    if (s->pool.used + ((size_t)nchunks + 1) * 4 + (size_t)nt * 24 + 24576 + KVQ_SKIP_CAP * sizeof(KvqSkippedTile) > s->pool.cap) {
+    if (s->pool.used + ((size_t)nchunks + 1) * 4 + (size_t)nt * (sizeof(KvqTileRec) + 8) + 24576 + KVQ_SKIP_CAP * sizeof(KvqSkippedTile) > s->pool.cap) {
         kvq_set_error(KVQ_ERR_RUNTIME, "batch tables outgrew their reservation"); return KVQ_ERR_RUNTIME;
     }
     const size_t first_b = (((size_t)nchunks + 1) * 4 + 255) & ~(size_t)255;
     const size_t ctr_b = 256 + 4 * BP_SHARDS * BP_SHARD_STRIDE;
     const size_t first_at = s->pool.take(first_b + sizeof(BpArgs) + ctr_b);
-    const size_t chunk_at = s->pool.take((size_t)nt * 16), report_at = s->pool.take((size_t)nt * 8), skip_at = s->pool.take(KVQ_SKIP_CAP * sizeof(KvqSkippedTile));
+    const size_t chunk_at = s->pool.take((size_t)nt * sizeof(KvqTileRec)), report_at = s->pool.take((size_t)nt * 8), skip_at = s->pool.take(KVQ_SKIP_CAP * sizeof(KvqSkippedTile));
     s->cur_skip_at = skip_at; s->cur_first_at = first_at; s->cur_ntiles = (uint32_t)nt;
     uint32_t *first = reinterpret_cast<uint32_t *>(s->pool.h + first_at);
     uint64_t acc = 0;
@@ -85,7 +85,7 @@
         BpArgs a;
         memset(&a, 0, sizeof(a));
         a.P = P; a.X = ix->dev; a.data = d_data; a.fpos_base = fpos_base;
-        a.tiles = reinterpret_cast<const uint4 *>(d_tchunk); a.tile_report = d_report; a.tile_ctr = d_tile_ctr;
+        a.tiles = reinterpret_cast<const KvqTileRec *>(d_tchunk); a.tile_report = d_report; a.tile_ctr = d_tile_ctr;
         static const uint32_t stagger = (uint32_t)(getenv("KVQ_STAGGER") ? atoi(getenv("KVQ_STAGGER")) : 0);
         a.ntiles = (uint32_t)nt; a.tile_bytes = TILE; a.dbg = dbg; a.pad_ = stagger;
         a.redo = s->d_redo.p; a.redo_cap = KVQ_REDO_CAP - KVQ_LONG_CAP; a.fail = s->cur_fail;
@@ -100,7 +100,7 @@
     }
     KVQ_HIP(hipMemcpyAsync(s->pool.d + s->cur_co_at, s->pool.h + s->cur_co_at, ctr_at + 4 * BP_SHARDS * BP_SHARD_STRIDE - s->cur_co_at,
                            hipMemcpyHostToDevice, s->stream));
-    hipLaunchKernelGGL(kvq_expand_tiles, dim3((uint32_t)((nchunks + 255) / 256)), dim3(256), 0, s->stream, (uint32_t)nchunks, d_chunk_off, d_first, reinterpret_cast<uint4 *>(d_tchunk),
+    hipLaunchKernelGGL(kvq_expand_tiles, dim3((uint32_t)((nchunks + 255) / 256)), dim3(256), 0, s->stream, (uint32_t)nchunks, d_chunk_off, d_first, reinterpret_cast<KvqTileRec *>(d_tchunk), TILE,
                        s->d_redo.p ? KvqRedo(s->d_redo.p).count : (unsigned int *)nullptr, s->d_surv.p ? KvqSurvivors(s->d_surv.p).count : (unsigned int *)nullptr);
 
     bool pipelined = false;
diff --git a/kvarq_amd/csrc/kvq_runtime.hip b/kvarq_amd/csrc/kvq_runtime.hip
--- a/kvarq_amd/csrc/kvq_runtime.hip
+++ b/kvarq_amd/csrc/kvq_runtime.hip
@@ -472,6 +472,17 @@
 
 extern "C" int32_t kvq_scan_path(const kvq_scan *s) { return s->path_bits; }
 extern "C" void kvq_scan_force_exhaustive(kvq_scan *s, int32_t on) { s->force_exhaustive = on != 0; }
+extern "C" int32_t kvq_scan_survivors(kvq_scan *s, uint32_t *asked, uint32_t *cap)
+{
+    unsigned int hdr[2] = { 0, 0 };
+    if (s->d_surv.p) {
+        KVQ_HIP(hipStreamSynchronize(s->stream));
+        KVQ_HIP(hipMemcpy(hdr, s->d_surv.p, sizeof(hdr), hipMemcpyDeviceToHost));
+    }
+    if (asked) *asked = hdr[0];
+    if (cap) *cap = hdr[1];
+    return KVQ_OK;
+}
 
 extern "C" int32_t kvq_scan_set_records(kvq_scan *s, int32_t on)
 {
@@ -561,7 +572,7 @@
 
     int rc;
     const size_t tiles_bound = (size_t)(nbytes / kvq_min_tile()) + (size_t)nchunks + 2;
-    if ((rc = s->pool.reserve(((size_t)nchunks + 1) * 8 + tiles_bound * 24 + 65536, s->stream))) return rc;
+    if ((rc = s->pool.reserve(((size_t)nchunks + 1) * 8 + tiles_bound * (sizeof(KvqTileRec) + 8) + 65536, s->stream))) return rc;
     const size_t co_at = s->pool.take(((size_t)nchunks + 1) * 4);
     s->cur_co_at = co_at;
     uint32_t *co = reinterpret_cast<uint32_t *>(s->pool.h + co_at);
```

After: 10.15 billion, median of 6. +6.1%, better.
